# bjack205/altro

Measured on AMD Instinct MI355X. Metric: iLQR backward+forward sweeps/sec (N knotpoints x batch), higher is better.
Workload: dtype f64

## Files before the change

### altro_amd/__init__.py

```python
import ctypes as C
import os

import numpy as np

_HERE = os.path.dirname(os.path.abspath(__file__))
LIB_PATH = os.path.join(_HERE, "lib", "libaltro_hip.so")

F64, F32 = 0, 1
PLAN_AUTO, PLAN_GENERIC, PLAN_MFMA16, PLAN_LANE, PLAN_MFMA32 = 0, 1, 2, 3, 4
STORE_QBLOCKS = 0x1
LANE_FUSED = 0x4
F32_PURE = 0x2
TILE_USER_BLOCKS = 0x2
GENERIC_MATRIX_CORES = 0x8
TVLQR_SUCCESS = -1

C_ABI_SYMBOLS = [
    "altro_hip_version", "altro_hip_last_error", "altro_hip_device_count", "altro_hip_device_info", "altro_hip_device_pci_bus_id",
    "altro_hip_batch_create", "altro_hip_batch_create_dims", "altro_hip_batch_destroy", "altro_hip_batch_plan",
    "altro_hip_batch_device_bytes", "altro_hip_set_dynamics", "altro_hip_set_cost",
    "altro_hip_set_initial_state", "altro_hip_set_host_batch", "altro_hip_backward", "altro_hip_forward_ltv", "altro_hip_sweep",
    "altro_hip_synchronize", "altro_hip_get_K", "altro_hip_get_d", "altro_hip_get_P",
    "altro_hip_get_p", "altro_hip_get_x", "altro_hip_get_u", "altro_hip_get_y",
    "altro_hip_get_delta_V", "altro_hip_get_status", "altro_hip_get_qblocks",
    "altro_hip_stats_reduce", "altro_hip_comm_unique_id", "altro_hip_comm_create", "altro_hip_comm_create_all",
    "altro_hip_comm_destroy", "altro_hip_comm_rank", "altro_hip_comm_world", "altro_hip_comm_device", "altro_hip_stats_allreduce", "altro_hip_stats_allreduce_multi",
    "altro_hip_profile_enable", "altro_hip_profile_reset",
    "altro_hip_profile_get", "altro_hip_profile_get_range", "altro_hip_profile_dropped", "altro_hip_algorithmic_bytes",
    "altro_hip_set_model", "altro_hip_set_model_source", "altro_hip_model_row_layout", "altro_hip_set_tracking_cost", "altro_hip_set_quadratic_cost",
    "altro_hip_set_input_guess", "altro_hip_set_state_guess",
    "altro_hip_open_loop_rollout", "altro_hip_accept", "altro_hip_expand", "altro_hip_merit",
    "altro_hip_stationarity", "altro_hip_get_nominal", "altro_hip_get_expansion",
    "altro_hip_default_solve_options", "altro_hip_set_forms", "altro_hip_get_forms", "altro_hip_ilqr_solve", "altro_hip_last_solve_counts",
    "altro_hip_ilqr_solve_async", "altro_hip_ilqr_poll", "altro_hip_ilqr_wait",
    "altro_hip_linesearch_host",
    "altro_hip_add_linear_constraint", "altro_hip_add_user_constraint", "altro_hip_clear_constraints", "altro_hip_reset_duals",
    "altro_hip_get_duals", "altro_hip_feasibility",
    "altro_hip_shift_trajectory", "altro_hip_update_linear_costs", "altro_hip_get_knot",
    "altro_hip_set_pointer_mode",
]
CONE_EQUALITY, CONE_IDENTITY, CONE_INEQUALITY, CONE_SOC = 0, 1, 2, 3

FORM_NO_SPECULATION, FORM_NO_RUNAHEAD, FORM_NO_MERIT2, FORM_MERIT_LDS, FORM_MERIT_DPP_ALWAYS = 0x1, 0x2, 0x4, 0x8, 0x10
FORM_EXPAND_LDS, FORM_ALROWS_LDS, FORM_ROLLOUT_ROUNDS, FORM_SEQUENCED, FORM_MERIT_ONE_LAUNCH = 0x20, 0x40, 0x80, 0x100, 0x200
FORM_LANE_QUAD_OFF, FORM_LANE_QUAD_ON, FORM_GENERIC_LATE_Q_OFF, FORM_GENERIC_LATE_Q_ON, FORM_FUSED_CLOCK = 0x400, 0x800, 0x1000, 0x2000, 0x4000
FORM_AFFINE_EXACT = 0x8000
FORM_NO_COMPACTION = 0x10000
FORM_GENERIC_MERIT_LDS = 0x20000


def forms_from_env():
    e = os.environ
    off = lambda name: e.get(name) is not None and e[name].strip() not in ("",) and _atoi(e[name]) == 0
    f = 0
    if "ALTRO_HIP_NO_SPECULATION" in e: f |= FORM_NO_SPECULATION
    if "ALTRO_HIP_NO_RUNAHEAD" in e and not off("ALTRO_HIP_NO_RUNAHEAD"): f |= FORM_NO_RUNAHEAD
    if off("ALTRO_HIP_MERIT2"): f |= FORM_NO_MERIT2
    if off("ALTRO_HIP_MERIT_DPP"): f |= FORM_MERIT_LDS
    elif e.get("ALTRO_HIP_MERIT_DPP") is not None and _atoi(e["ALTRO_HIP_MERIT_DPP"]) == 2: f |= FORM_MERIT_DPP_ALWAYS
    if off("ALTRO_HIP_EXPAND_DPP"): f |= FORM_EXPAND_LDS
    if off("ALTRO_HIP_ALROWS_DPP"): f |= FORM_ALROWS_LDS
    if off("ALTRO_HIP_AFFINE"): f |= FORM_ROLLOUT_ROUNDS
    if off("ALTRO_HIP_FUSED") or "ALTRO_HIP_NO_FUSED" in e: f |= FORM_SEQUENCED
    if off("ALTRO_HIP_MERIT_SPLIT"): f |= FORM_MERIT_ONE_LAUNCH
    if "ALTRO_HIP_LANE_QUAD" in e: f |= FORM_LANE_QUAD_OFF if _atoi(e["ALTRO_HIP_LANE_QUAD"]) == 0 else FORM_LANE_QUAD_ON
    if "ALTRO_HIP_GENERIC_LATE_Q" in e: f |= FORM_GENERIC_LATE_Q_OFF if _atoi(e["ALTRO_HIP_GENERIC_LATE_Q"]) == 0 else FORM_GENERIC_LATE_Q_ON
    if "ALTRO_HIP_FUSED_CLOCK" in e: f |= FORM_FUSED_CLOCK
    if "ALTRO_HIP_AFFINE_EXACT" in e: f |= FORM_AFFINE_EXACT
    if "ALTRO_HIP_NO_COMPACTION" in e: f |= FORM_NO_COMPACTION
    return f


def _atoi(text):
    try:
        return int(text.strip() or 0)
    except ValueError:
        return 0

MODEL_LINEAR, MODEL_DOUBLE_INTEGRATOR, MODEL_PENDULUM, MODEL_BICYCLE, MODEL_USER, MODEL_QUADROTOR, MODEL_QUADROTOR13 = 0, 1, 2, 3, 4, 5, 6
MERIT_FN = C.CFUNCTYPE(None, C.c_double, C.POINTER(C.c_double), C.POINTER(C.c_double), C.c_void_p)


class SolveOptions(C.Structure):
    _fields_ = [("iterations_max", C.c_int), ("tol_stationarity", C.c_double),
                ("tol_primal_feasibility", C.c_double), ("tol_meritfun_gradient", C.c_double),
                ("use_backtracking_linesearch", C.c_int), ("penalty_initial", C.c_double),
                ("penalty_scaling", C.c_double), ("penalty_max", C.c_double), ("reg_initial", C.c_double),
                ("reg_retry_max", C.c_int), ("reg_scale", C.c_double), ("reg_min", C.c_double),
                ("reg_max", C.c_double), ("stop_when_running_at_most", C.c_int),
                ("forms", C.c_uint), ("fused_sweeps", C.c_int), ("decision_margin", C.c_double)]


class SolveResult(C.Structure):
    _fields_ = [("status", C.c_int), ("iterations", C.c_int), ("stationarity", C.c_double),
                ("final_alpha", C.c_double), ("final_phi", C.c_double), ("primal_feasibility", C.c_double),
                ("penalty", C.c_double), ("dual_updates", C.c_int), ("reg_retries", C.c_int)]


class PollRecord(C.Structure):
    _fields_ = [("result", SolveResult), ("u0", C.c_double * 4), ("done", C.c_int), ("reserved", C.c_int)]

# ... 62 lines not shown
        L.altro_hip_set_initial_state.argtypes = [vp, vp, i]
        L.altro_hip_set_host_batch.argtypes = [vp, i]
        L.altro_hip_backward.argtypes = [vp, d]
        L.altro_hip_forward_ltv.argtypes = [vp]
        L.altro_hip_sweep.argtypes = [vp, d]
        L.altro_hip_synchronize.argtypes = [vp]
        for g in ("K", "d", "P", "p", "x", "u", "y", "delta_V", "status", "qblocks"):
            getattr(L, "altro_hip_get_" + g).argtypes = [vp, vp]
        L.altro_hip_stats_reduce.argtypes = [vp, C.POINTER(Stats)]
        L.altro_hip_comm_unique_id.argtypes = [vp]
        L.altro_hip_comm_create.argtypes = [C.POINTER(vp), i, i, i, vp]
        L.altro_hip_comm_create_all.argtypes = [C.POINTER(vp), i, C.POINTER(i)]
        L.altro_hip_comm_destroy.argtypes = [vp]
        L.altro_hip_comm_destroy.restype = None
        for fn in ("rank", "world", "device"):
            getattr(L, "altro_hip_comm_" + fn).argtypes = [vp]
        L.altro_hip_stats_allreduce.argtypes = [vp, vp, C.POINTER(Stats)]
        L.altro_hip_stats_allreduce_multi.argtypes = [C.POINTER(vp), C.POINTER(vp), i, C.POINTER(Stats)]
        L.altro_hip_profile_enable.argtypes = [vp, i]
        L.altro_hip_profile_reset.argtypes = [vp]
        L.altro_hip_profile_get.argtypes = [vp, i, C.POINTER(i), C.POINTER(d), C.POINTER(C.c_char_p)]
        L.altro_hip_profile_get_range.argtypes = [vp, i, C.POINTER(d), C.POINTER(d)]
        L.altro_hip_profile_dropped.argtypes = [vp, i]
        L.altro_hip_algorithmic_bytes.argtypes = [vp, i]
        L.altro_hip_algorithmic_bytes.restype = d
        L.altro_hip_set_model.argtypes = [vp, i, C.c_float, i, d, d]
        L.altro_hip_set_model_source.argtypes = [vp, C.c_char_p, C.c_float]
        L.altro_hip_model_row_layout.argtypes = [vp]
        L.altro_hip_set_tracking_cost.argtypes = [vp, vp, vp, vp, vp, i, i]
        L.altro_hip_set_quadratic_cost.argtypes = [vp, vp, vp, vp, vp, vp, vp, i, i]
        L.altro_hip_set_input_guess.argtypes = [vp, vp, i, i]
        L.altro_hip_set_state_guess.argtypes = [vp, vp, i, i]
        for fn in ("open_loop_rollout", "accept", "expand"):
            getattr(L, "altro_hip_" + fn).argtypes = [vp]
        L.altro_hip_merit.argtypes = [vp, vp, i, i, vp, vp]
        L.altro_hip_stationarity.argtypes = [vp, vp]
        L.altro_hip_get_nominal.argtypes = [vp, vp, vp]
        L.altro_hip_get_expansion.argtypes = [vp, vp, vp, vp, vp]
        L.altro_hip_add_linear_constraint.argtypes = [vp, i, i, i, i, vp, vp, i]
        L.altro_hip_add_user_constraint.argtypes = [vp, i, i, i, i, i]
        L.altro_hip_clear_constraints.argtypes = [vp]
        L.altro_hip_reset_duals.argtypes = [vp, d]
        L.altro_hip_get_duals.argtypes = [vp, i, i, vp]
        L.altro_hip_feasibility.argtypes = [vp, vp]
        L.altro_hip_set_pointer_mode.argtypes = [vp, i]
        L.altro_hip_shift_trajectory.argtypes = [vp]
        L.altro_hip_update_linear_costs.argtypes = [vp, vp, vp, vp, i, i, i, i]
        L.altro_hip_get_knot.argtypes = [vp, i, vp, vp]
        L.altro_hip_default_solve_options.argtypes = [C.POINTER(SolveOptions)]
        L.altro_hip_default_solve_options.restype = None
        L.altro_hip_set_forms.argtypes = [vp, C.c_uint]
        L.altro_hip_get_forms.argtypes = [vp]
        L.altro_hip_get_forms.restype = C.c_uint
        L.altro_hip_ilqr_solve.argtypes = [vp, C.POINTER(SolveOptions), vp]
        L.altro_hip_last_solve_counts.argtypes = [vp, C.POINTER(i), C.POINTER(i)]
        L.altro_hip_ilqr_solve_async.argtypes = [vp, C.POINTER(SolveOptions)]
        L.altro_hip_ilqr_poll.argtypes = [vp, C.POINTER(i), C.POINTER(C.POINTER(PollRecord))]
        L.altro_hip_ilqr_wait.argtypes = [vp, vp]
        L.altro_hip_linesearch_host.argtypes = [MERIT_FN, vp, d, d, d, i, i, d, d, C.POINTER(i), C.POINTER(i),
                                                C.POINTER(d), C.POINTER(d)]
        L.altro_hip_linesearch_host.restype = d
        L.altro_hip_selftest_mfma_f64.argtypes = [i]
        L.altro_hip_selftest_mfma_f64.restype = d
        L.altro_hip_selftest_mfma_f32_4b.argtypes = [i]
        L.altro_hip_selftest_mfma_f32_4b.restype = d
        L.altro_hip_selftest_sincos.argtypes = [i, vp, i, vp, vp]
        L.altro_hip_selftest_sincos.restype = i
        _lib = L
    return _lib


def _check(rc):
    if rc != 0:
        raise AltroHipError("altro_hip error %d: %s" % (rc, lib().altro_hip_last_error().decode()))


def device_info(device=0):
    L = lib()
    name, pci = C.create_string_buffer(256), C.create_string_buffer(64)
    cus, ws = C.c_int(), C.c_int()
    _check(L.altro_hip_device_info(int(device), name, 256, C.byref(cus), C.byref(ws)))
    _check(L.altro_hip_device_pci_bus_id(int(device), pci, 64))
    return name.value.decode(), cus.value, pci.value.decode()


def _in(a):
    if a is None:
        return None, None
    a = np.ascontiguousarray(a, dtype=np.float64)
    return a, a.ctypes.data_as(C.c_void_p)


class Batch:

    def __init__(self, N, n, m, batch, dtype=F64, plan=PLAN_AUTO, flags=0, device=0, stream=None):
        self.L = lib()
        self.N, self.n, self.m, self.batch = N, n, m, batch
        self.h = C.c_void_p()
        _check(self.L.altro_hip_batch_create(C.byref(self.h), N, n, m, batch, dtype, plan, flags,
                                             device, stream))

    @property
    def plan(self):
        return self.L.altro_hip_batch_plan(self.h)

    @classmethod
# ... 202 lines not shown
        if rc < 0:
            _check(rc)
        return rc

    def add_user_constraint(self, k_first, k_last, cone, p, cid):
        rc = self.L.altro_hip_add_user_constraint(self.h, int(k_first), int(k_last), int(cone), int(p), int(cid))
        if rc < 0:
            _check(rc)
        return rc

    def clear_constraints(self):
        _check(self.L.altro_hip_clear_constraints(self.h))

    def reset_duals(self, penalty=1.0):
        _check(self.L.altro_hip_reset_duals(self.h, float(penalty)))

    def get_duals(self, k, slot, p):
        out = np.zeros((self.batch, p))
        _check(self.L.altro_hip_get_duals(self.h, int(k), int(slot), out.ctypes.data_as(C.c_void_p)))
        return out

    def feasibility(self):
        self._sync_forms()
        out = np.zeros(self.batch)
        _check(self.L.altro_hip_feasibility(self.h, out.ctypes.data_as(C.c_void_p)))
        return out

    def _solve_options(self, iterations_max=200, tol_stationarity=1e-4, tol_meritfun_gradient=1e-8,
                       use_backtracking=False, tol_primal_feasibility=1e-4, penalty_initial=1.0, penalty_scaling=10.0,
                       penalty_max=1e8, reg_initial=0.0, reg_retry_max=0, reg_scale=10.0, reg_min=1e-6, reg_max=1e8,
                       stop_when_running_at_most=0, forms=0, fused_sweeps=None, decision_margin=None):
        self._sync_forms()
        o = SolveOptions()
        self.L.altro_hip_default_solve_options(C.byref(o))
        o.forms = int(forms)
        if fused_sweeps is None and "ALTRO_HIP_FUSED_SWEEPS" in os.environ:
            fused_sweeps = _atoi(os.environ["ALTRO_HIP_FUSED_SWEEPS"]) or 1
        o.fused_sweeps = int(fused_sweeps or 0)
        if decision_margin is not None:
            o.decision_margin = float(decision_margin)
        o.tol_primal_feasibility = tol_primal_feasibility
        o.penalty_initial, o.penalty_scaling, o.penalty_max = penalty_initial, penalty_scaling, penalty_max
        o.reg_initial, o.reg_retry_max, o.reg_scale = reg_initial, reg_retry_max, reg_scale
        o.reg_min, o.reg_max = reg_min, reg_max
        o.stop_when_running_at_most = int(stop_when_running_at_most)
        o.iterations_max, o.tol_stationarity = iterations_max, tol_stationarity
        o.tol_meritfun_gradient, o.use_backtracking_linesearch = tol_meritfun_gradient, int(use_backtracking)
        return o

    def set_forms(self, forms):
        self._forms_user = int(forms)
        self._sync_forms()

    def _sync_forms(self):
        want = getattr(self, "_forms_user", 0) | forms_from_env()
        if want != getattr(self, "_forms_set", 0):
            _check(self.L.altro_hip_set_forms(self.h, want))
            self._forms_set = want

    @staticmethod
    def _results(rec, sweeps, merit_launches):
        return dict(status=rec["status"].copy(), iterations=rec["iterations"].copy(),
                    stationarity=rec["stationarity"].copy(), alpha=rec["final_alpha"].copy(), phi=rec["final_phi"].copy(),
                    feasibility=rec["primal_feasibility"].copy(), penalty=rec["penalty"].copy(),
                    dual_updates=rec["dual_updates"].copy(), reg_retries=rec["reg_retries"].copy(),
                    sweeps=sweeps, merit_launches=merit_launches)

    def ilqr_solve(self, **options):
        o = self._solve_options(**options)
        res = (SolveResult * self.batch)()
        _check(self.L.altro_hip_ilqr_solve(self.h, C.byref(o), res))
        sw, ml = C.c_int(), C.c_int()
        self.L.altro_hip_last_solve_counts(self.h, C.byref(sw), C.byref(ml))
        rec = np.frombuffer(res, dtype=np.dtype(SolveResult))
        return self._results(rec, sw.value, ml.value)

    def ilqr_solve_async(self, **options):
        o = self._solve_options(**options)
        _check(self.L.altro_hip_ilqr_solve_async(self.h, C.byref(o)))

    def poll(self):
        n, recs = C.c_int(), C.POINTER(PollRecord)()
        _check(self.L.altro_hip_ilqr_poll(self.h, C.byref(n), C.byref(recs)))
        buf = (PollRecord * self.batch).from_address(C.addressof(recs.contents))
        return n.value, np.frombuffer(buf, dtype=np.dtype(PollRecord))

    def wait(self):
        res = (SolveResult * self.batch)()
        _check(self.L.altro_hip_ilqr_wait(self.h, res))
        sw, ml = C.c_int(), C.c_int()
        self.L.altro_hip_last_solve_counts(self.h, C.byref(sw), C.byref(ml))
        return self._results(np.frombuffer(res, dtype=np.dtype(SolveResult)), sw.value, ml.value)


class Comm:

    @staticmethod
    def unique_id():
        buf = (C.c_char * COMM_ID_BYTES)()
        _check(lib().altro_hip_comm_unique_id(C.cast(buf, C.c_void_p)))
        return bytes(buf)

    def __init__(self, device, rank, world, uid):
        self.L = lib()
        self.c = C.c_void_p()
        assert len(uid) == COMM_ID_BYTES
# ... 36 lines not shown
```

### altro_amd/csrc/capi_core.hip

```cpp
#include "capi_internal.h"

namespace altro_hip {
namespace capi {

thread_local std::string g_last_error;

int fail(int code, const char* fmt, ...) {
  char buf[512];
  va_list ap;
  va_start(ap, fmt);
  vsnprintf(buf, sizeof(buf), fmt, ap);
  va_end(ap);
  g_last_error = buf;
  return code;
}

}
}

using namespace altro_hip;
using namespace altro_hip::capi;

namespace {

// ... 166 lines not shown
    }
    ALLOC(h->g_off, off.size() * sizeof(int64_t));
    ALLOC(h->g_nx, (size_t)(N + 1) * sizeof(int));
    ALLOC(h->g_nu, (size_t)(N + 1) * sizeof(int));
    if (!rc) {
      if (hipMemcpy(h->g_off, off.data(), off.size() * sizeof(int64_t), hipMemcpyHostToDevice) != hipSuccess ||
          hipMemcpy(h->g_nx, nx.data(), nx.size() * sizeof(int), hipMemcpyHostToDevice) != hipSuccess ||
          hipMemcpy(h->g_nu, nu.data(), nu.size() * sizeof(int), hipMemcpyHostToDevice) != hipSuccess)
        rc = fail(ALTRO_HIP_ERR_HIP, "table upload failed");
    }
  }
  {
    if (!rc) h->al_knots.assign((size_t)N + 1, AlKnotBig{});
    ALLOC(h->i_prob, B * sizeof(IlqrProb));
    ALLOC(h->i_alpha, B * 8);
    ALLOC(h->i_phi, B * 8 * ILQR_SPEC_TRIALS);
    ALLOC(h->i_spec_sel, B * sizeof(int));
    ALLOC(h->i_spec_refresh, B * sizeof(int));
    ALLOC(h->i_guard, B * sizeof(int));
    ALLOC(h->i_active_exact, B * sizeof(int));
    if (!rc && (hipMemsetAsync(h->i_guard, 0, B * sizeof(int), h->stream) != hipSuccess || hipMemsetAsync(h->i_active_exact, 0, B * sizeof(int), h->stream) != hipSuccess)) rc = fail(ALTRO_HIP_ERR_HIP, "memset failed");
    ALLOC(h->i_stat_done, B * sizeof(int));
    ALLOC(h->i_dphi, B * 8 * 2);
    ALLOC(h->i_active, B * sizeof(int));
    ALLOC(h->i_counters, (size_t)kCounterSlots * 8 * sizeof(int));
    if (!rc && hipMemsetAsync(h->i_counters, 0, (size_t)kCounterSlots * 8 * sizeof(int), h->stream) != hipSuccess) rc = fail(ALTRO_HIP_ERR_HIP, "memset failed");
    ALLOC(h->i_reg, B * 8);
    if (!rc) {
      std::vector<IlqrProb> pr((size_t)B);
      std::memset(pr.data(), 0, pr.size() * sizeof(IlqrProb));
      for (auto& q : pr) { q.rho = 1.0; q.rho_est = 1.0; q.status = 1; }
      if (hipMemcpy(h->i_prob, pr.data(), pr.size() * sizeof(IlqrProb), hipMemcpyHostToDevice) != hipSuccess)
        rc = fail(ALTRO_HIP_ERR_HIP, "control block upload failed");
    }
  }
#undef ALLOC
  if (!rc && (hipEventCreate(&h->ev0) != hipSuccess || hipEventCreate(&h->ev1) != hipSuccess))
    rc = fail(ALTRO_HIP_ERR_HIP, "hipEventCreate failed");
  if (rc) {
    altro_hip_batch_destroy(h);
    return rc;
  }
  *out = h;
  return 0;
}

int altro_hip_batch_create(altro_hip_batch** out, int N, int n, int m, int batch, int dtype, int plan,
                           unsigned flags, int device, void* stream) {
  return batch_create_impl(out, N, n, m, batch, dtype, plan, flags, device, stream, nullptr, nullptr);
}

extern "C++" {
namespace altro_hip { namespace capi {
int replan_empty_handle(altro_hip_batch* h, int plan) {
  if (!h->auto_plan || h->dyn_set || h->cost_set || h->model_set || h->lqr_cost_set || h->guess_set || !h->al_defs.empty() ||
      (h->x0_set && h->x0_host.empty()))
    return fail(ALTRO_HIP_ERR_UNSUPPORTED, "this handle runs plan %d; create it with plan %d (or call altro_hip_set_model before the dynamics, the cost, "
                                           "a guess or a constraint block reach a handle created with ALTRO_HIP_PLAN_AUTO)", h->plan, plan);
  altro_hip_batch* fresh = nullptr;
  int rc = batch_create_impl(&fresh, h->N, h->n, h->m, h->batch, h->dtype, plan, h->flags, h->device, h->user_stream ? (void*)h->stream : nullptr,
                             nullptr, nullptr);
  if (rc) return rc;
  fresh->dev_ptrs = h->dev_ptrs; fresh->host_batch = h->host_batch; fresh->forms = h->forms;
  const int prof = h->prof;
  std::vector<double> x0 = std::move(h->x0_host);
  const int x0_bz = h->x0_host_bz;
  std::swap(*h, *fresh);
  h->auto_plan = false;
  altro_hip_batch_destroy(fresh);
  if (prof && (rc = altro_hip_profile_enable(h, prof))) return rc;
  if (!x0.empty()) {
    const bool dp = h->dev_ptrs;
    h->dev_ptrs = false;
    rc = altro_hip_set_initial_state(h, x0.data(), x0_bz);
    h->dev_ptrs = dp;
  }
  return rc;
}
} }
}

int altro_hip_batch_create_dims(altro_hip_batch** out, int N, const int* nx, const int* nu, int batch, int dtype,
                                unsigned flags, int device, void* stream) {
  if (!out) return fail(ALTRO_HIP_ERR_BAD_ARGUMENT, "out == NULL");
  *out = nullptr;
  if (N <= 0 || !nx || !nu) return fail(ALTRO_HIP_ERR_BAD_ARGUMENT, "N must be positive, nx and nu non-null");
  int nmax = 0, mmax = 0;
  for (int k = 0; k <= N; ++k) {
    if (nx[k] <= 0 || nx[k] > kGenericMaxDim) return fail(ALTRO_HIP_ERR_UNSUPPORTED, "nx[%d] = %d outside [1, %d]", k, nx[k], kGenericMaxDim);
    nmax = std::max(nmax, nx[k]);
    if (k < N) {
      if (nu[k] <= 0 || nu[k] > kGenericMaxDim) return fail(ALTRO_HIP_ERR_UNSUPPORTED, "nu[%d] = %d outside [1, %d]", k, nu[k], kGenericMaxDim);
      mmax = std::max(mmax, nu[k]);
    }
  }
  return batch_create_impl(out, N, nmax, mmax, batch, dtype, ALTRO_HIP_PLAN_GENERIC, flags, device, stream, nx, nu);
}

void altro_hip_batch_destroy(altro_hip_batch* h) {
  if (!h) return;
  (void)hipSetDevice(h->device);
  if (h->stream) (void)hipStreamSynchronize(h->stream);
  void* ptrs[] = {h->x0, h->delta_V, h->status, h->m_in, h->m_cin, h->m_term, h->m_out, h->m_outn, h->m_xuy,
                  h->m_qblk, h->m_trash, h->g_off, h->g_nx, h->g_nu, h->stage,
                  h->l_in, h->l_term, h->l_out, h->l_outn, h->l_xuy, h->l_x0,
                  h->l_nom, h->l_cost, h->g_ws, h->i_prob, h->i_alpha, h->i_phi, h->i_dphi, h->i_active, h->i_counters,
                  h->al_d_knots, h->al_d_big, h->al_d_gsel, h->al_d_guser, h->g_stat_part, h->al_d_G, h->al_d_Gpad, h->al_d_g, h->al_d_z, h->i_reg, h->m_nom, h->m_costp,
                  h->i_cand_spec, h->i_spec_sel, h->i_spec_refresh, h->i_fused_list, h->i_guard, h->i_active_exact, h->i_stat_done, h->st_partial, h->st_red, h->i_merit_jk, h->i_spec_jac, h->i_results,
                  h->m_costd, h->m_costd_term, h->l_costq, h->i_sens, h->i_sens_alpha, h->i_aff_part, h->i_aff_on, h->g_xn, h->g_un, h->g_cQ, h->g_cR, h->g_cH, h->g_cq, h->g_cr, h->g_cc};
  for (void* p : ptrs) if (p) (void)hipFree(p);
  if (h->i_results_host) (void)hipHostFree(h->i_results_host);
  if (h->poll_host) (void)hipHostFree(h->poll_host);
  if (h->poll_count_host) (void)hipHostFree(h->poll_count_host);
  if (h->cnt_host) (void)hipHostFree(h->cnt_host);
  for (hipEvent_t e : h->cnt_ev) if (e) (void)hipEventDestroy(e);
  for (int a = 0; a < G_NUM; ++a) if (h->g_arr[a]) (void)hipFree(h->g_arr[a]);
  if (h->ev0) (void)hipEventDestroy(h->ev0);
  if (h->ev1) (void)hipEventDestroy(h->ev1);
  for (hipEvent_t e : h->prof_ev) if (e) (void)hipEventDestroy(e);
  if (h->own_stream && h->stream) (void)hipStreamDestroy(h->stream);
  delete h;
}

int altro_hip_batch_plan(const altro_hip_batch* h) { return h ? (h->g_tile ? (int)ALTRO_HIP_PLAN_MFMA32 : h->plan) : ALTRO_HIP_ERR_BAD_ARGUMENT; }
size_t altro_hip_batch_device_bytes(const altro_hip_batch* h) { return h ? h->device_bytes : 0; }

int altro_hip_set_dynamics(altro_hip_batch* h, const double* A, const double* B, const double* f,
                           int kz, int bz) {
  int rc = check(h);
  if (rc) return rc;
  h->expansion_current = false;
  if (!A || !B) return fail(ALTRO_HIP_ERR_BAD_ARGUMENT, "A and B are required");
  const int n = h->n, m = h->m, N = h->N;
  h->has_f = f ? 1 : 0;
  if (h->plan == ALTRO_HIP_PLAN_MFMA16) {
    DevSrc dA, dB, df;
    const int nkh = kz ? 1 : N;
    rc = put_src(h, A, n * n, nkh, kz, bz, &dA);
    if (!rc) rc = put_src(h, B, n * m, nkh, kz, bz, &dB);
    if (!rc) rc = put_src(h, f, n, nkh, kz, bz, &df);
    if (!rc) rc = mfma16_pack_launch(h, MSEG_Z, dA.s, dB.s);
    if (!rc) rc = mfma16_pack_launch(h, MSEG_F, df.s, SrcArr{nullptr, 0, 0, 0});
    if (!rc) HIP_TRY(hipStreamSynchronize(h->stream));
  } else if (h->plan == ALTRO_HIP_PLAN_LANE) {
    const LaneSizes z = lane_sizes(n, m);
    const int nkh = kz ? 1 : N;
    auto pk = [&](const double* src, int len, int off) -> int { return lane_pack(h, h->l_in, 0, z.e_in, src, len, off, 0, N, 0, nkh, kz, bz); };
    rc = pk(A, n * n, 0);
    if (!rc) rc = pk(B, n * m, n * n);
    if (!rc) rc = pk(f, n, n * n + n * m);
  } else {
    if (h->ragged && kz) return fail(ALTRO_HIP_ERR_BAD_ARGUMENT, "k_stride_zero needs uniform dimensions");
    auto set = [&](int arr, const double* src, int blk) -> int {
      return h->ragged ? generic_set(h, arr, src, (int)h->g_bstride[arr], 1, 0, bz) : generic_set(h, arr, src, blk, N, kz, bz);
    };
    rc = set(G_A, A, n * n);
    if (!rc) rc = set(G_B, B, n * m);
    if (!rc) {
      if (f) rc = set(G_f, f, n);
      else HIP_TRY(hipMemsetAsync(h->g_arr[G_f], 0, (size_t)h->batch * h->g_bstride[G_f] * h->esz, h->stream));
    }
  }
  if (!rc) { HIP_TRY(hipStreamSynchronize(h->stream)); h->dyn_set = true; }
  return rc;
}

int altro_hip_set_cost(altro_hip_batch* h, const double* Q, const double* R, const double* H,
                       const double* q, const double* r, int is_diag, int kz, int bz) {
  int rc = check(h);
  if (rc) return rc;
  h->expansion_current = false;
  if (!Q || !R || !q || !r) return fail(ALTRO_HIP_ERR_BAD_ARGUMENT, "Q, R, q, r are required");
  if (!is_diag && !H) return fail(ALTRO_HIP_ERR_BAD_ARGUMENT, "H is required for a dense cost");
  h->ilqr_linear = false;
  const int n = h->n, m = h->m, N = h->N;
  Dims d{n, m};
  h->is_diag = is_diag ? 1 : 0;
  const int nkQ = kz ? 2 : N + 1;
  const int nkR = kz ? 1 : N;
  if (h->plan == ALTRO_HIP_PLAN_MFMA16) {
    DevSrc dQ, dR, dH, dq, dr;
    rc = put_src(h, Q, d.Q(is_diag), nkQ, kz, bz, &dQ);
    if (!rc) rc = put_src(h, R, d.R(is_diag), nkR, kz, bz, &dR);
    if (!rc && !is_diag) rc = put_src(h, H, d.H(), nkR, kz, bz, &dH);
    if (!rc) rc = put_src(h, q, n, nkQ, kz, bz, &dq);
    if (!rc) rc = put_src(h, r, m, nkR, kz, bz, &dr);
    SrcArr none{nullptr, 0, 0, 0};
    SrcArr tQ = dQ.s, tq = dq.s;
    if (kz) { tQ.p += d.Q(is_diag); tq.p += n; }
    if (!rc) rc = mfma16_pack_launch(h, MSEG_Q, dQ.s, none);
    if (!rc) rc = mfma16_pack_launch(h, MSEG_TERM_Q, tQ, none);
    if (!rc) rc = mfma16_pack_launch(h, MSEG_HR, dH.s, dR.s);
    if (!rc) rc = mfma16_pack_launch(h, MSEG_QR, dq.s, dr.s);
    if (!rc) rc = mfma16_pack_launch(h, MSEG_TERM_q, tq, none);
    if (!rc) HIP_TRY(hipStreamSynchronize(h->stream));
  } else if (h->plan == ALTRO_HIP_PLAN_LANE) {
    const LaneSizes z = lane_sizes(n, m);
    const int oQ = n * n + n * m + n, oR = oQ + n * n, oH = oR + m * m, oq = oH + m * n, or_ = oq + n;
    auto pk = [&](void* dst, int E, const double* src, int len, int off, int diag, int nk, int k_src0,
                  int nk_host, int src_off = 0) -> int {
      return lane_pack(h, dst, 0, E, src, len, off, diag, nk, k_src0, nk_host, kz, bz, src_off);
    };
    const int kt = kz ? 0 : N;
    rc = pk(h->l_in, z.e_in, Q, d.Q(is_diag), oQ, is_diag ? n : 0, N, 0, nkQ);
    if (!rc) rc = pk(h->l_in, z.e_in, R, d.R(is_diag), oR, is_diag ? m : 0, N, 0, nkR);
    if (!rc) rc = pk(h->l_in, z.e_in, is_diag ? nullptr : H, d.H(), oH, 0, N, 0, nkR);
    if (!rc) rc = pk(h->l_in, z.e_in, q, n, oq, 0, N, 0, nkQ);
    if (!rc) rc = pk(h->l_in, z.e_in, r, m, or_, 0, N, 0, nkR);
    if (!rc) rc = pk(h->l_term, z.e_term, Q, d.Q(is_diag), 0, is_diag ? n : 0, 1, kt, nkQ, kz ? d.Q(is_diag) : 0);
    if (!rc) rc = pk(h->l_term, z.e_term, q, n, n * n, 0, 1, kt, nkQ, kz ? n : 0);
  } else if (h->ragged) {
    if (kz) return fail(ALTRO_HIP_ERR_BAD_ARGUMENT, "k_stride_zero needs uniform dimensions");
    {
      std::vector<int64_t> off((size_t)(N + 1) * G_NUM);
      HIP_TRY(hipStreamSynchronize(h->stream));
      HIP_TRY(hipMemcpy(off.data(), h->g_off, off.size() * sizeof(int64_t), hipMemcpyDeviceToHost));
      int64_t aq = 0, ar = 0;
      for (int k = 0; k <= N; ++k) {
        off[(size_t)k * G_NUM + G_Q] = aq; off[(size_t)k * G_NUM + G_R] = ar;
        aq += is_diag ? h->nxv[k] : h->nxv[k] * h->nxv[k];
        if (k < N) ar += is_diag ? h->nuv[k] : h->nuv[k] * h->nuv[k];
      }
      h->g_bstride[G_Q] = aq; h->g_bstride[G_R] = ar;
      HIP_TRY(hipMemcpy(h->g_off, off.data(), off.size() * sizeof(int64_t), hipMemcpyHostToDevice));
    }
    auto whole = [&](int arr, const double* src) -> int {
      if (!src) { HIP_TRY(hipMemsetAsync(h->g_arr[arr], 0, (size_t)h->batch * h->g_bstride[arr] * h->esz, h->stream)); return 0; }
      return generic_set(h, arr, src, (int)h->g_bstride[arr], 1, 0, bz);
    };
    rc = whole(G_Q, Q);
// ... 248 lines not shown
```

### altro_amd/csrc/capi_ilqr.hip

```cpp
#include "capi_internal.h"

#include <cstring>

using namespace altro_hip;
using namespace altro_hip::capi;

namespace altro_hip {
namespace capi {

static AlInput al_input(const altro_hip_batch* h) {
  return AlInput{h->plan, h->n, h->m, h->N, h->batch, h->dtype == ALTRO_HIP_F64 ? sizeof(double) : sizeof(float), h->ragged, h->nxv, h->nuv,
                 h->al_defs, h->al_knots, h->al_G, h->al_g};
}
static int al_copy(altro_hip_batch* h, void** dst, const void* src, size_t bytes) {
  if (const int rc = dmalloc(h, dst, bytes)) return rc;
  HIP_TRY(hipMemcpy(*dst, src, bytes, hipMemcpyHostToDevice));
  return 0;
}
static int al_copy_pool(altro_hip_batch* h, void** dst, const std::vector<double>& pool) {
  if (h->dtype == ALTRO_HIP_F64) return al_copy(h, dst, pool.data(), pool.size() * sizeof(double));
  const std::vector<float> f = al_pool_as<float>(pool);
  return al_copy(h, dst, f.data(), f.size() * sizeof(float));
}
static int al_upload_tables(altro_hip_batch* h) {
// ... 69 lines not shown
bool ensure_spares(altro_hip_batch* h, int count, size_t bytes_each) {
  if (h->spare_count >= count) return true;
  if (h->spare_failed > 0 && count >= h->spare_failed) return false;
  void* fresh = nullptr;
  if (hipMalloc(&fresh, (size_t)count * bytes_each) != hipSuccess) { (void)hipGetLastError(); h->spare_failed = count; return false; }
  if (h->i_cand_spec) { (void)hipStreamSynchronize(h->stream); (void)hipFree(h->i_cand_spec); h->device_bytes -= (size_t)h->spare_count * bytes_each; }
  h->i_cand_spec = fresh;
  h->spare_count = count;
  h->device_bytes += (size_t)count * bytes_each;
  return true;
}
void merit_split_prepare(altro_hip_batch* h) {
  if (h->merit_split >= 0) return;
  h->merit_split = form(h, ALTRO_HIP_FORM_MERIT_ONE_LAUNCH) ? 0 : 1;
  if (!h->merit_split) return;
  const size_t jk = (size_t)spec_trials_cap(h) * (h->N + 1) * h->batch * h->esz;
  const size_t jac = ((size_t)h->N * (h->n * h->n + h->n * h->m + h->n + h->m) + h->n) * h->batch * h->esz;
  if (dmalloc(h, &h->i_merit_jk, jk) || dmalloc(h, &h->i_spec_jac, jac)) {
    (void)hipGetLastError();
    if (h->i_merit_jk) { (void)hipFree(h->i_merit_jk); h->i_merit_jk = nullptr; }
    h->merit_split = 0;
  }
}

template <typename T>
int ilqr_launch(altro_hip_batch* h, int which, IlqrArgs<T> a) {
  if (h->model.kind == MODEL_USER) return rtc_launch<T>(h, which, a);
  const int rc = ilqr_launch_kernel<T>(h->stream, which, h->model.kind, h->n, h->m, a);
  if (rc == 1) return fail(ALTRO_HIP_ERR_UNSUPPORTED, "no device model for (kind, n, m) = (%d, %d, %d)", h->model.kind, h->n, h->m);
  if (rc) return fail(ALTRO_HIP_ERR_HIP, "iLQR kernel launch failed");
  return 0;
}
template <typename S>
int wave_run(altro_hip_batch* h, int which, bool use_alpha, bool use_active, int want_deriv, double alpha_const, int mode) {
  IlqrWaveArgs<S> a;
  a.al = al_table<S>(h);
  a.mode = mode;
  const bool user_al = a.al.enabled && h->al_sum.has_user;
  if (user_al && (h->forms & (ALTRO_HIP_FORM_MERIT_LDS | ALTRO_HIP_FORM_ALROWS_LDS | ALTRO_HIP_FORM_EXPAND_LDS)))
    return fail(ALTRO_HIP_ERR_UNSUPPORTED, "constraint blocks from source on plan MFMA16 run in the row-layout kernels only: the LDS comparison forms "
                                           "(ALTRO_HIP_FORM_MERIT_LDS, _ALROWS_LDS, _EXPAND_LDS) do not evaluate them");
  a.penalty_scaling = h->expand_penalty_scaling; a.penalty_max = h->expand_penalty_max;
  if (which == IK_STATIONARITY || which == IK_DUAL)
    a.mode = form(h, ALTRO_HIP_FORM_ALROWS_LDS) ? 0 : STAT_NO_FEAS;
  if (which == IK_EXPAND && form(h, ALTRO_HIP_FORM_EXPAND_LDS) && !h->cost_dense) a.mode |= EXPAND_LDS;
  a.costd = (const S*)h->m_costd; a.costd_term = (const S*)h->m_costd_term; a.cost_dense = h->cost_dense ? 1 : 0;
  if (h->model_set) {
    a.mp = h->model;
    if (which == IK_EXPAND && (a.mode & EXPAND_GRADIENT) && !(a.mode & EXPAND_NEXT)) a.mode |= EXPAND_DYN;
  }
  if (which == IK_MERIT)
    a.mode = form(h, ALTRO_HIP_FORM_MERIT_LDS) ? 0 : form(h, ALTRO_HIP_FORM_MERIT_DPP_ALWAYS) ? 3 : 2;
  a.dyn = (const S*)h->m_in; a.dyn_bs = h->m_st.in_bs; a.dyn_ks = h->m_st.in_ks;
  a.cin = (S*)h->m_cin; a.cin_bs = h->m_st.cin_bs; a.cin_ks = h->m_st.cin_ks;
  a.term = (S*)h->m_term; a.out = (const S*)h->m_out; a.out_bs = h->m_st.out_bs; a.out_ks = h->m_st.out_ks;
  a.outn = (const S*)h->m_outn; a.nom = (S*)h->m_nom; a.cand = (S*)h->m_xuy; a.xuy_bs = h->m_st.xuy_bs;
  a.xuy_ks = h->m_st.xuy_ks; a.costp = (const S*)h->m_costp; a.x0 = (const S*)h->x0;
  a.alpha = use_alpha ? h->i_alpha : nullptr; a.active = use_active ? h->i_active : nullptr;
  a.phi = h->i_phi; a.dphi = h->i_dphi; a.prob = h->i_prob; a.N = h->N; a.batch = h->batch;
  a.want_derivative = want_deriv; a.alpha_const = alpha_const;
  a.cand_spec = (S*)h->i_cand_spec; a.spec_trials = h->i_cand_spec ? h->spec_trials : 1; a.spec_sel = h->i_spec_sel;
  a.spec_pre = h->i_cand_spec ? h->spec_pre : 0;
  a.spec_stride = (int64_t)h->batch * (h->N + 1) * MF_XUY;
  a.ls_beta = h->spec_beta; a.ls_max_iters = h->spec_max_iters;
  a.skip = which == IK_STATIONARITY ? h->stat_skip : nullptr;
  if constexpr (sizeof(S) == 8) {
    if (h->aff_enabled && !h->model_set) {
      if (h->aff_store && (which == IK_MERIT2 || which == IK_MERIT)) {
        a.sens = (double*)h->i_sens; a.sens_alpha = (double*)h->i_sens_alpha;
      } else if (which == IK_MERIT && h->aff_round && a.mode >= 2 && !a.spec_pre) {
        a.sens = (double*)h->i_sens; a.sens_alpha = (double*)h->i_sens_alpha;
        a.aff = 1; a.aff_part = (double*)h->i_aff_part; a.aff_on = (int*)h->i_aff_on;
      }
    }
  }
  if (h->model_set && h->model.kind == MODEL_USER) {
    if constexpr (sizeof(S) == 8) {
      if (which == IK_ROLLOUT || which == IK_MERIT || which == IK_MERIT2) return rtc_tile_launch(h, which, a);
      if (which == IK_EXPAND && (a.mode & EXPAND_DYN)) {
        const int rcm = rtc_tile_launch(h, IK_EXPAND, a);
        if (rcm) return rcm;
      }
      if (user_al && (which == IK_EXPAND || which == IK_DUAL)) return rtc_tile_al_launch(h, which, a);
      if (user_al && which == IK_STATIONARITY) {
        a.mp.kind = MODEL_LINEAR;
        a.mode |= STAT_FEAS_USER;
        const int rcs = ilqr_wave_launch_kernel<S>(h->stream, which, a);
        if (rcs) return fail(ALTRO_HIP_ERR_HIP, "iLQR kernel launch failed");
        return rtc_tile_al_launch(h, which, a);
      }
    }
    a.mp.kind = MODEL_LINEAR;
  }
  const int rc = ilqr_wave_launch_kernel<S>(h->stream, which, a);
  if (rc == 1) return fail(ALTRO_HIP_ERR_UNSUPPORTED, "operation %d is not available on plan MFMA16", which);
  if (rc) return fail(ALTRO_HIP_ERR_HIP, "iLQR kernel launch failed");
  return 0;
}
struct GenSizes { int64_t sx, su, sQ, sR, sH; };
GenSizes gen_sizes(const altro_hip_batch* h) {
  GenSizes z{0, 0, 0, 0, 0};
  for (int k = 0; k <= h->N; ++k) {
    const int64_t nk = h->ragged ? h->nxv[k] : h->n, mk = k < h->N ? (h->ragged ? h->nuv[k] : h->m) : 0;
    z.sx += nk; z.su += mk; z.sQ += nk * nk; z.sR += mk * mk; z.sH += mk * nk;
  }
  return z;
}
// ... 27 lines not shown
  a.alpha = use_alpha ? h->i_alpha : nullptr; a.active = use_active ? h->i_active : nullptr; a.alpha_const = alpha_const;
  a.phi = h->i_phi; a.dphi = h->i_dphi; a.prob = h->i_prob;
  a.N = N; a.n = n; a.m = m; a.batch = h->batch; a.want_derivative = want_deriv; a.mode = mode;
  a.off = h->g_off; a.nx = h->g_nx; a.nu = h->g_nu;
  const GenSizes gs = gen_sizes(h);
  a.sx = gs.sx; a.su = gs.su; a.sQ = gs.sQ; a.sR = gs.sR; a.sH = gs.sH;
  a.al = al_table<T>(h);
  a.row32 = (sizeof(T) == 8 && row32_eligible(h)) ? 1 : 0;
  a.row32m = (sizeof(T) == 8 && row32_model_eligible(h)) ? 1 : 0;
  if ((a.row32 || a.row32m) && which == IK_STATIONARITY && N > 32) {
    const size_t need = (size_t)((N + 31) / 32) * h->batch * 2 * sizeof(double);
    if (h->g_stat_part_bytes < need) {
      if (h->g_stat_part) { (void)hipFree(h->g_stat_part); h->g_stat_part = nullptr; h->g_stat_part_bytes = 0; }
      if (hipMalloc((void**)&h->g_stat_part, need) == hipSuccess) h->g_stat_part_bytes = need;
      else { (void)hipGetLastError(); h->g_stat_part = nullptr; }
    }
    a.stat_part = h->g_stat_part;
  }
  if (h->model_set) {
    a.mp = h->model;
    if (which == IK_EXPAND && (a.mode & EXPAND_GRADIENT)) a.mode |= EXPAND_DYN;
  }
  if constexpr (sizeof(T) == 8) {
    if (h->model_set && h->model.kind == MODEL_USER) {
      const bool user_al = a.al.enabled && a.al.guser;
      if (which == IK_ROLLOUT || which == IK_MERIT || (which == IK_MERIT2 && a.row32m)) return rtc_gen_launch(h, which, a);
      if (user_al && (which == IK_STATIONARITY || which == IK_DUAL)) return rtc_gen_al_launch(h, which, a);
      if (which == IK_EXPAND) {
        IlqrGenArgs<T> ac = a;
        ac.mp.kind = MODEL_LINEAR;
        if (user_al) {
          const int rc0 = rtc_gen_al_launch(h, which, ac);
          if (rc0) return rc0;
        } else {
          const int rc0 = ilqr_generic_launch<T>(h->stream, which, ac);
          if (rc0) return fail(ALTRO_HIP_ERR_HIP, "iLQR kernel launch failed");
        }
        return (a.mode & EXPAND_DYN) ? rtc_gen_launch(h, which, a) : 0;
      }
    }
  }
  const int rc = ilqr_generic_launch<T>(h->stream, which, a);
  if (rc == 1) return fail(ALTRO_HIP_ERR_UNSUPPORTED, "operation %d is not available on plan GENERIC", which);
  if (rc) return fail(ALTRO_HIP_ERR_HIP, "iLQR kernel launch failed");
  return 0;
}
int ilqr_run(altro_hip_batch* h, int which, bool use_alpha, bool use_active, int want_deriv, double alpha_const, int mode) {
  int rc = al_upload(h);
  if (rc) return rc;
  if (h->plan == ALTRO_HIP_PLAN_GENERIC)
    return h->dtype == ALTRO_HIP_F64 ? gen_run<double>(h, which, use_alpha, use_active, want_deriv, alpha_const, mode)
                                     : gen_run<float>(h, which, use_alpha, use_active, want_deriv, alpha_const, mode);
  if (h->plan == ALTRO_HIP_PLAN_MFMA16) {
    rc = h->dtype == ALTRO_HIP_F64 ? wave_run<double>(h, which, use_alpha, use_active, want_deriv, alpha_const, mode)
                                   : wave_run<float>(h, which, use_alpha, use_active, want_deriv, alpha_const, mode);
    if (which == IK_MERIT) h->expansion_current = !rc && want_deriv && !use_active && h->spec_trials == 1 && !h->spec_pre && h->al_defs.empty();
    else if (which == IK_ROLLOUT || which == IK_SHIFT || which == IK_SPEC_SELECT || which == IK_MERIT2 || which == IK_DUAL) h->expansion_current = false;
    return rc;
  }
  if (which == IK_MERIT) merit_split_prepare(h);
  if (h->dtype == ALTRO_HIP_F64) {
    auto a = ilqr_args<double>(h, use_alpha, use_active, want_deriv, alpha_const);
    a.mode = mode;
    return ilqr_launch<double>(h, which, a);
  }
  auto a = ilqr_args<float>(h, use_alpha, use_active, want_deriv, alpha_const);
  a.mode = mode;
  return ilqr_launch<float>(h, which, a);
}

struct CostUpload { int field; const double* src; int nk_host; };
int cost_fields_set(altro_hip_batch* h, bool dense, const CostUpload* up, int count, int kz, int bz) {
  LoopShape s = loop_shape(h);
  s.cost_dense = dense;
  const int N = h->N;
  int rc = 0;
  for (int pass = 0; pass < 2; ++pass)
    for (int i = 0; i < count && !rc; ++i) {
      const FieldRef r0 = loop_field(s, up[i].field, 0), rN = loop_field(s, up[i].field, N);
      const bool zero_array = !up[i].src && r0.kind == LK_AOS;
      if (pass == 0 && zero_array) HIP_TRY(hipMemsetAsync(loop_buffer(h, r0.buf), 0, (size_t)h->batch * r0.bs * h->esz, h->stream));
      else if (pass == 0) rc = field_set(h, s, up[i].field, 0, s.ragged && rN.buf != LB_NONE ? N + 1 : N, up[i].src, kz, bz, up[i].nk_host);
      else if (!zero_array && !s.ragged && rN.buf != LB_NONE) rc = field_set(h, s, up[i].field, N, 1, up[i].src, 1, bz, up[i].nk_host, (kz ? 1 : N) * rN.len);
    }
  return rc;
}
int generic_cost_def(altro_hip_batch* h, const double* Q, const double* R, const double* H, const double* q, const double* r,
                     const double* c, int kz, int bz) {
  const int N = h->N;
  const int nkx = kz ? 2 : N + 1, nku = kz ? 1 : N;
  const size_t B = h->batch, E = h->esz;
  const GenSizes gs = gen_sizes(h);
  int rc = 0;
  {
    struct { void** p; size_t bytes; bool zero; } want[] = {
        {&h->g_cQ, B * gs.sQ * E, false}, {&h->g_cR, B * gs.sR * E, false}, {&h->g_cH, B * gs.sH * E, false},
        {&h->g_cq, B * gs.sx * E, false}, {&h->g_cr, B * gs.su * E, false}, {&h->g_cc, B * (N + 1) * E, false},
        {&h->g_xn, B * gs.sx * E, true},  {&h->g_un, B * gs.su * E, true}};
    for (auto& w : want) {
      if (*w.p) continue;
      if ((rc = dmalloc(h, w.p, w.bytes))) return rc;
      if (w.zero) HIP_TRY(hipMemsetAsync(*w.p, 0, w.bytes, h->stream));
    }
  }
  if (h->ragged && kz) return fail(ALTRO_HIP_ERR_BAD_ARGUMENT, "k_stride_zero needs uniform dimensions");
  const CostUpload up[] = {{LF_COST_Q, Q, nkx}, {LF_COST_R, R, nku}, {LF_COST_H, H, nku}, {LF_COST_q, q, nkx}, {LF_COST_r, r, nku}, {LF_COST_c, c, nkx}};
// ... 408 lines not shown
      return fail(ALTRO_HIP_ERR_BAD_ARGUMENT, "knot points %d and %d differ in dimension: one constraint block takes one [x; u] size "
                                              "(register it per range, like ALTROSolver::SetConstraint per index)", k_first, ad.k);
    default: break;
  }
  const int w = ad.w;
  AlDef d{cone, p, g_per_problem ? 1 : 0, (int)h->al_G.size(), 0, user, w};
  h->al_G.insert(h->al_G.end(), G, G + (size_t)p * w);
  h->al_g.emplace_back(g, g + (size_t)p * (g_per_problem ? h->batch : 1));
  const int id = (int)h->al_defs.size();
  h->al_defs.push_back(d);
  for (int k = k_first; k <= k_last; ++k) {
    AlKnotBig& kn = h->al_knots[k];
    kn.def[kn.ncon++] = id;
  }
  h->al_dirty = true;
  return id;
}
int altro_hip_add_linear_constraint(altro_hip_batch* h, int k_first, int k_last, int cone, int p, const double* G,
                                    const double* g, int g_per_problem) {
  return add_block(h, k_first, k_last, cone, p, G, g, g_per_problem, 0);
}
int altro_hip_add_user_constraint(altro_hip_batch* h, int k_first, int k_last, int cone, int p, int id) {
  int rc = loop_entry(h);
  if (rc) return rc;
  const bool gen = h->plan == ALTRO_HIP_PLAN_GENERIC;
  const bool tile = h->plan == ALTRO_HIP_PLAN_MFMA16;
  if ((h->plan != ALTRO_HIP_PLAN_LANE && !gen && !tile) || h->model.kind != MODEL_USER || !h->rtc_has_constraints)
    return fail(ALTRO_HIP_ERR_NOT_SET, "altro_hip_set_model_source must come first, with a source that defines "
                                       "altro_user_constraint and altro_user_constraint_jacobian (plans LANE and GENERIC / MFMA32)");
  if (id < 0) return fail(ALTRO_HIP_ERR_BAD_ARGUMENT, "constraint id %d", id);
  const AlAdmit ad = al_admit(al_input(h), k_first, k_last, cone, p, id + 1);
  if (ad.limit == AL_LIMIT_USER_CONE) return fail(ALTRO_HIP_ERR_BAD_ARGUMENT, "unknown cone %d", cone);
  if (ad.limit == AL_LIMIT_USER_ROWS && tile)
    return fail(ALTRO_HIP_ERR_UNSUPPORTED, "a constraint block from source has 1 .. %d rows on plan MFMA16 (%s: one slot; got %d): "
                                           "ALTRO_HIP_PLAN_GENERIC takes 32", ad.pmax, cone == CONE_SOC ? "AL_MAXSOC" : "AL_MAXP", p);
  if (ad.limit == AL_LIMIT_USER_ROWS)
    return fail(ALTRO_HIP_ERR_UNSUPPORTED, "a constraint block from source has 1 .. %d rows on plan GENERIC (GEN_USER_MAXROWS; got %d)", ad.pmax, p);
  if (ad.limit == AL_LIMIT_USER_KNOT && tile)
    return fail(ALTRO_HIP_ERR_UNSUPPORTED, "at most %d constraint blocks from source per knot point on plan MFMA16 (AL_TILE_USER_MAXC; k = %d "
                                           "would have %d): ALTRO_HIP_PLAN_GENERIC takes 32 rows of them", ad.cmax, ad.k, ad.count);
  if (ad.limit == AL_LIMIT_USER_KNOT)
    return fail(ALTRO_HIP_ERR_UNSUPPORTED, "at most %d rows of constraint blocks from source per knot point on plan GENERIC "
                                           "(GEN_USER_MAXROWS; k = %d would have %d)", ad.cmax, ad.k, ad.count);
  std::vector<double> G((size_t)std::max(p, 0) * (h->n + h->m), 0.0), g((size_t)std::max(p, 0), 0.0);
  return add_block(h, k_first, k_last, cone, p, G.data(), g.data(), 0, id + 1);
}
int altro_hip_clear_constraints(altro_hip_batch* h) {
  int rc = loop_entry(h, true);
  if (rc) return rc;
  h->expansion_current = false;
  h->al_defs.clear(); h->al_G.clear(); h->al_g.clear();
  h->al_knots.assign((size_t)h->N + 1, AlKnotBig{});
  h->al_dirty = true;
  return al_upload(h);
}
int altro_hip_reset_duals(altro_hip_batch* h, double penalty) {
  int rc = loop_entry(h, true);
  if (rc) return rc;
  h->expansion_current = false;
  if (!(penalty > 0.0)) return fail(ALTRO_HIP_ERR_BAD_ARGUMENT, "penalty must be positive");
  if ((rc = al_upload(h))) return rc;
  const size_t E = h->dtype == ALTRO_HIP_F64 ? 8 : 4;
  if (h->al_d_z) HIP_TRY(hipMemsetAsync(h->al_d_z, 0, (size_t)h->al_rows * h->batch * E, h->stream));
  std::vector<IlqrProb> pr(h->batch);
  HIP_TRY(hipStreamSynchronize(h->stream));
  HIP_TRY(hipMemcpy(pr.data(), h->i_prob, pr.size() * sizeof(IlqrProb), hipMemcpyDeviceToHost));
  for (auto& q : pr) { q.rho = penalty; q.rho_est = penalty; }
  HIP_TRY(hipMemcpy(h->i_prob, pr.data(), pr.size() * sizeof(IlqrProb), hipMemcpyHostToDevice));
  return 0;
}
int altro_hip_get_duals(altro_hip_batch* h, int k, int slot, double* z) {
  int rc = loop_entry(h, true);
  if (rc) return rc;
  if ((rc = al_upload(h))) return rc;
  if (k < 0 || k > h->N || slot < 0 || slot >= h->al_knots[k].ncon || !z)
    return fail(ALTRO_HIP_ERR_BAD_ARGUMENT, "no constraint block %d at knot point %d", slot, k);
  const AlKnotBig& kn = h->al_knots[k];
  const int p = h->al_defs[kn.def[slot]].p;
  const int64_t B = h->batch;
  HIP_TRY(hipStreamSynchronize(h->stream));
  auto fetch = [&](auto t) -> int {
    std::vector<decltype(t)> v((size_t)p * B);
    HIP_TRY(hipMemcpy(v.data(), (const decltype(t)*)h->al_d_z + (size_t)kn.z_off[slot] * B, v.size() * sizeof(t), hipMemcpyDeviceToHost));
    for (int64_t b = 0; b < B; ++b)
      for (int r = 0; r < p; ++r) z[(size_t)b * p + r] = v[(size_t)r * B + b];
    return 0;
  };
  return h->dtype == ALTRO_HIP_F64 ? fetch(double{}) : fetch(float{});
}

}
int altro_hip::capi::ilqr_gather_results(altro_hip_batch* h, altro_hip_solve_result* results) {
  static_assert(sizeof(IlqrResult) == sizeof(altro_hip_solve_result), "IlqrResult mirrors altro_hip_solve_result");
  static_assert(sizeof(IlqrPollRec) == sizeof(altro_hip_poll_record), "IlqrPollRec mirrors altro_hip_poll_record");
  int rc;
  const size_t bytes = (size_t)h->batch * sizeof(IlqrResult);
  if (!h->i_results) {
    if ((rc = dmalloc(h, &h->i_results, bytes))) return rc;
    if (hipHostMalloc(&h->i_results_host, bytes, hipHostMallocDefault) != hipSuccess) { (void)hipGetLastError(); h->i_results_host = nullptr; }
  }
  if (ilqr_launch_results(h->stream, h->i_prob, (IlqrResult*)h->i_results, h->batch)) return fail(ALTRO_HIP_ERR_HIP, "results kernel launch failed");
  void* stage = h->i_results_host ? h->i_results_host : (void*)results;
  HIP_TRY(hipMemcpyAsync(stage, h->i_results, bytes, hipMemcpyDeviceToHost, h->stream));
  HIP_TRY(hipStreamSynchronize(h->stream));
  if (stage != (void*)results) std::memcpy(results, stage, bytes);
  return 0;
}
// ... 14 lines not shown
  return 0;
}
int altro_hip_ilqr_wait(altro_hip_batch* h, altro_hip_solve_result* results) {
  int rc = loop_entry(h, true);
  if (rc) return rc;
  if (!h->poll_host) return fail(ALTRO_HIP_ERR_NOT_SET, "altro_hip_ilqr_solve_async has not been called");
  HIP_TRY(hipStreamSynchronize(h->stream));
  if (h->async_pending) {
    h->async_pending = false;
    int c4[4];
    HIP_TRY(hipMemcpy(c4, h->i_counters, sizeof(c4), hipMemcpyDeviceToHost));
    h->last_sweeps = c4[3];
    h->last_merit_launches = 0;
  }
  if (results) return ilqr_gather_results(h, results);
  return 0;
}


void altro_hip_default_solve_options(altro_hip_solve_options* o) {
  if (!o) return;
  o->iterations_max = 200;
  o->tol_stationarity = 1e-4;
  o->tol_primal_feasibility = 1e-4;
  o->tol_meritfun_gradient = 1e-8;
  o->use_backtracking_linesearch = 0;
  o->penalty_initial = 1.0;
  o->penalty_scaling = 10.0;
  o->penalty_max = 1e8;
  o->reg_initial = 0.0;
  o->reg_retry_max = 0;
  o->reg_scale = 10.0;
  o->reg_min = 1e-6;
  o->reg_max = 1e8;
  o->stop_when_running_at_most = 0;
  o->forms = 0;
  o->fused_sweeps = 0;
  o->decision_margin = 0.0;
}
int altro_hip_set_forms(altro_hip_batch* h, unsigned forms) {
  int rc = check(h);
  if (rc) return rc;
  if ((forms & ALTRO_HIP_FORM_LANE_QUAD_OFF) && (forms & ALTRO_HIP_FORM_LANE_QUAD_ON))
    return fail(ALTRO_HIP_ERR_BAD_ARGUMENT, "ALTRO_HIP_FORM_LANE_QUAD_OFF and _ON exclude each other");
  if ((forms & ALTRO_HIP_FORM_GENERIC_LATE_Q_OFF) && (forms & ALTRO_HIP_FORM_GENERIC_LATE_Q_ON))
    return fail(ALTRO_HIP_ERR_BAD_ARGUMENT, "ALTRO_HIP_FORM_GENERIC_LATE_Q_OFF and _ON exclude each other");
  if (((h->forms ^ forms) & ALTRO_HIP_FORM_MERIT_ONE_LAUNCH) && h->merit_split >= 0) {
    HIP_TRY(hipStreamSynchronize(h->stream));
    if (h->i_merit_jk) { (void)hipFree(h->i_merit_jk); h->i_merit_jk = nullptr; }
    if (h->i_spec_jac) { (void)hipFree(h->i_spec_jac); h->i_spec_jac = nullptr; }
    h->merit_split = -1;
  }
  h->forms = forms;
  return 0;
}
unsigned altro_hip_get_forms(const altro_hip_batch* h) { return h ? h->forms : 0u; }
int altro_hip_last_solve_counts(const altro_hip_batch* h, int* sweeps, int* merit_launches) {
  if (!h) return fail(ALTRO_HIP_ERR_BAD_ARGUMENT, "null handle");
  if (sweeps) *sweeps = h->last_sweeps;
  if (merit_launches) *merit_launches = h->last_merit_launches;
  return 0;
}
int altro_hip_get_nominal(altro_hip_batch* h, double* x, double* u) {
  int rc = loop_entry(h, true);
  if (rc) return rc;
  if (h->plan == ALTRO_HIP_PLAN_MFMA16 && !h->m_nom) return fail(ALTRO_HIP_ERR_NOT_SET, "altro_hip_set_tracking_cost has not been called");
  if (h->plan == ALTRO_HIP_PLAN_GENERIC && !h->g_xn) return fail(ALTRO_HIP_ERR_NOT_SET, "no cost has been set for the iLQR loop");
  const LoopShape s = loop_shape(h);
  if (x && (rc = field_get(h, s, LF_NOM_X, 0, h->N + 1, x))) return rc;
  if (u) rc = field_get(h, s, LF_NOM_U, 0, h->N, u);
  return rc;
}
int altro_hip_get_expansion(altro_hip_batch* h, double* A, double* B, double* lx, double* lu) {
  int rc = loop_entry(h);
  if (rc) return rc;
  const int n = h->n, m = h->m, N = h->N;
  if (h->plan == ALTRO_HIP_PLAN_MFMA16) {
    if (h->dev_ptrs) return fail(ALTRO_HIP_ERR_UNSUPPORTED, "altro_hip_get_expansion on plan MFMA16 writes host arrays");
    const int64_t B_ = h->batch;
    std::vector<double> raw;
    auto fetch = [&](const void* src, int64_t bs, int64_t ks, int off, int block, int nk) -> int {
      raw.assign((size_t)B_ * nk * block, 0.0);
      return aos_get(h, raw.data(), src, off, bs, ks, block, nk);
    };
    if (A || B) {
      if ((rc = fetch(h->m_in, h->m_st.in_bs, h->m_st.in_ks, MF_OFF_Z, 192, N))) return rc;
      for (int64_t b = 0; b < B_; ++b)
        for (int k = 0; k < N; ++k) {
          const double* zr = raw.data() + ((size_t)b * N + k) * 192;
          if (A) for (int j = 0; j < n; ++j) for (int i = 0; i < n; ++i) A[((size_t)b * N + k) * n * n + i + (size_t)n * j] = zr[i * 16 + j];
          if (B) for (int j = 0; j < m; ++j) for (int i = 0; i < n; ++i) B[((size_t)b * N + k) * n * m + i + (size_t)n * j] = zr[i * 16 + MF_N + j];
        }
    }
    if (lx || lu) {
      if ((rc = fetch(h->m_cin, h->m_st.cin_bs, h->m_st.cin_ks, MF_OFF_QR, 16, N))) return rc;
      for (int64_t b = 0; b < B_; ++b)
        for (int k = 0; k < N; ++k) {
          const double* qr = raw.data() + ((size_t)b * N + k) * 16;
          if (lx) for (int i = 0; i < n; ++i) lx[((size_t)b * (N + 1) + k) * n + i] = qr[i];
          if (lu) for (int i = 0; i < m; ++i) lu[((size_t)b * N + k) * m + i] = qr[MF_N + i];
        }
      if (lx) {
        if ((rc = fetch(h->m_term, MF_TERM, 0, MF_TERM_q, MF_N, 1))) return rc;
        for (int64_t b = 0; b < B_; ++b)
          for (int i = 0; i < n; ++i) lx[((size_t)b * (N + 1) + N) * n + i] = raw[(size_t)b * MF_N + i];
      }
    }
    return 0;
  }
  if (h->plan == ALTRO_HIP_PLAN_GENERIC) {
    auto get = [&](double* dst, int arr, int blk, int nk) -> int { return dst ? generic_get(h, arr, dst, blk, nk) : 0; };
    rc = get(A, G_A, n * n, N);
    if (!rc) rc = get(B, G_B, n * m, N);
    if (!rc) rc = get(lx, G_q, n, N + 1);
    if (!rc) rc = get(lu, G_r, m, N);
    return rc;
  }
  const LaneSizes z = lane_sizes(n, m);
  const int oq = 2 * n * n + 2 * n * m + m * m + n, orr = oq + n;
  auto get = [&](double* dst, int off, int len, int nk, bool with_term, int off_term) -> int {
    if (!dst) return 0;
    return lane_get(h, dst, h->l_in, 0, with_term ? h->l_term : nullptr, z.e_in, off, off_term, len, nk, N);
  };
  rc = get(A, 0, n * n, N, false, 0);
  if (!rc) rc = get(B, n * n, n * m, N, false, 0);
  if (!rc) rc = get(lx, oq, n, N + 1, true, n * n);
  if (!rc) rc = get(lu, orr, m, N, false, 0);
  return rc;
}

double altro_hip_linesearch_host(altro_hip_merit_fn f, void* ctx, double alpha0, double phi0, double dphi0,
                                 int try_cubic_first, int use_backtracking, double c1, double c2,
                                 int* status, int* iters, double* phi, double* dphi) {
  LsOptions o = ls_default_options();
  o.try_cubic_first = try_cubic_first; o.use_backtracking = use_backtracking; o.c1 = c1; o.c2 = c2;
  LsState s;
  bool need = ls_begin(s, o, alpha0, phi0, dphi0);
  while (need) {
    double p = 0.0, dp = 0.0;
    f(s.alpha, &p, s.want_derivative ? &dp : nullptr, ctx);
    need = ls_feed(s, o, p, dp);
  }
  if (status) *status = s.status;
  if (iters) *iters = s.n_iters;
  if (phi) *phi = s.phi;
  if (dphi) *dphi = s.dphi;
  return s.alpha;
}
// ... 3 lines not shown
```

### altro_amd/csrc/capi_internal.h

```cpp
#pragma once
#include "altro_hip/altro_hip.h"

#include <hip/hip_runtime.h>
#include <hip/hip_ext.h>

#include <algorithm>
#include <cstdarg>
#include <cstdio>
#include <cstdlib>
#include <cstring>
#include <string>
#include <vector>

#include "kernels/pack.hip"
#include "kernels/tvlqr_generic.hip"
#include "kernels/tvlqr_lane.hip"
#include "kernels/ilqr_types.h"
#include "kernels/ilqr_generic.hip"
#include "kernels/mfma16_layout.h"
#include "linesearch_sm.h"
#include "al_tables.h"
#include "loop_fields.h"
#include "rtc_unit.h"

namespace altro_hip {
namespace capi {

int fail(int code, const char* fmt, ...);

#define HIP_TRY(expr)                                                                         \
  do {                                                                                        \
    hipError_t e_ = (expr);                                                                   \
    if (e_ != hipSuccess)                                                                     \
      return ::altro_hip::capi::fail(ALTRO_HIP_ERR_HIP, "%s failed: %s (%s:%d)", #expr, hipGetErrorString(e_), \
                  __FILE__, __LINE__);                                                        \
  } while (0)

constexpr size_t kStageBytes = size_t(256) << 20;

}
}

using namespace altro_hip;

struct altro_hip_batch {
  int N = 0, n = 0, m = 0, batch = 0, dtype = 0, plan = 0, device = 0;
  unsigned flags = 0;
  unsigned forms = 0;
  hipStream_t stream = nullptr;
  bool own_stream = false;
  size_t esz = 8;
  void* x0 = nullptr;
  void* delta_V = nullptr;
  int* status = nullptr;
  bool dyn_set = false, cost_set = false, x0_set = false, backward_done = false, forward_done = false;
  int has_f = 0, is_diag = 0;
  int host_batch = 0;
  bool dev_ptrs = false;
  void* g_arr[G_NUM] = {};
  int64_t g_bstride[G_NUM] = {};
  void *i_sens = nullptr, *i_sens_alpha = nullptr, *i_aff_part = nullptr, *i_aff_on = nullptr;
  bool aff_failed = false;
  bool aff_enabled = false, aff_round = false, aff_store = false;
  bool g_tile = false;
  bool g_mfma = false;
  bool ragged = false;
  std::vector<int> nxv, nuv;
  int64_t* g_off = nullptr;
  int* g_nx = nullptr;
  int* g_nu = nullptr;
  void *m_in = nullptr, *m_cin = nullptr, *m_term = nullptr, *m_out = nullptr, *m_outn = nullptr, *m_xuy = nullptr,
       *m_qblk = nullptr, *m_trash = nullptr;
  Mfma16Strides m_st{};
  void *l_in = nullptr, *l_term = nullptr, *l_out = nullptr, *l_outn = nullptr, *l_xuy = nullptr,
       *l_x0 = nullptr;
  void *l_nom = nullptr, *l_cost = nullptr;
  IlqrProb* i_prob = nullptr;
  double *i_alpha = nullptr, *i_phi = nullptr, *i_dphi = nullptr;
  int *i_active = nullptr, *i_counters = nullptr;
  int* cnt_host = nullptr;
  int* cnt_host_dev = nullptr;
  hipEvent_t cnt_ev[16] = {};
  void* i_cand_spec = nullptr;
  void* poll_host = nullptr; int* poll_count_host = nullptr;
  bool async_request = false, async_pending = false;
  bool rtc_row32_ok = false;
  bool rtc_has_constraints = false;
  void* rtc = nullptr;
  std::string rtc_source;
  int rtc_ck = 0;
  int x0_stride = 0;
  int spare_count = 0;
  int spare_failed = 0;
  int *i_spec_sel = nullptr, *i_spec_refresh = nullptr;
  int* i_fused_list = nullptr;
  int fused_resident = 0;
  int *i_guard = nullptr, *i_active_exact = nullptr;
  int* i_stat_done = nullptr;
  const int* stat_skip = nullptr;
  void *i_merit_jk = nullptr, *i_spec_jac = nullptr;
  int merit_split = -1;
  void *i_results = nullptr, *i_results_host = nullptr;
  void* g_ws = nullptr;
  bool fwd_quad = false;
  bool bwd_quad = false;
  int spec_trials = 1;
  int spec_pre = 0;
  bool spec_no_memory = false;
  double spec_beta = 0.5;
  int spec_max_iters = 25;
  ModelParams model{MODEL_LINEAR, 0.0f, 0, 2.7, 1.5};
  bool model_set = false, lqr_cost_set = false, guess_set = false;
  std::vector<double> x0_host;
  int x0_host_bz = 0;
  bool auto_plan = false;
  bool user_stream = false;
  std::vector<AlDef> al_defs;
  std::vector<AlKnotBig> al_knots;
  std::vector<double> al_G;
  std::vector<std::vector<double>> al_g;
  int al_rows = 0;
  capi::AlSummary al_sum;
  bool al_dirty = false;
  AlKnot* al_d_knots = nullptr;
  AlKnotBig* al_d_big = nullptr;
  void *al_d_G = nullptr, *al_d_g = nullptr, *al_d_z = nullptr;
  void* al_d_Gpad = nullptr;
  double* g_stat_part = nullptr; size_t g_stat_part_bytes = 0;
  int* al_d_gsel = nullptr;
  int* al_d_guser = nullptr;
  double expand_penalty_scaling = 10.0, expand_penalty_max = 1e8;
  const int* bwd_active = nullptr;
  const double* bwd_reg = nullptr;
  void *m_nom = nullptr, *m_costp = nullptr;
  bool ilqr_linear = false;
  void *m_costd = nullptr, *m_costd_term = nullptr, *l_costq = nullptr;
  bool cost_dense = false;
  bool expansion_current = false;
  void *g_xn = nullptr, *g_un = nullptr, *g_cQ = nullptr, *g_cR = nullptr, *g_cH = nullptr, *g_cq = nullptr, *g_cr = nullptr, *g_cc = nullptr;
  double* i_reg = nullptr;
  void* stage = nullptr;
  size_t stage_bytes = 0;
  size_t device_bytes = 0;
  double *st_partial = nullptr, *st_red = nullptr;
  bool solve_done = false;
  int prof = 0;
  std::vector<hipEvent_t> prof_ev;
  std::vector<int> prof_slot;
  int prof_n = 0;
  double prof_min[2] = {0, 0}, prof_max[2] = {0, 0};
  hipEvent_t ev0 = nullptr, ev1 = nullptr;
  hipEvent_t launch_ev0 = nullptr, launch_ev1 = nullptr;
  int last_sweeps = 0, last_merit_launches = 0;
  int prof_launches[2] = {0, 0};
  int prof_dropped[2] = {0, 0};
  double prof_ms[2] = {0, 0};
};

namespace altro_hip {
namespace capi {

inline bool form(const altro_hip_batch* h, unsigned bit) { return (h->forms & bit) != 0; }

inline int dmalloc(altro_hip_batch* h, void** p, size_t bytes) {
  hipError_t e = hipMalloc(p, bytes ? bytes : 16);
  if (e != hipSuccess) {
    *p = nullptr;
    return fail(ALTRO_HIP_ERR_OUT_OF_MEMORY, "hipMalloc(%zu bytes) failed: %s", bytes,
                hipGetErrorString(e));
  }
  h->device_bytes += bytes;
  return 0;
}

inline int check(altro_hip_batch* h) {
  if (!h) return fail(ALTRO_HIP_ERR_BAD_ARGUMENT, "null handle");
  hipError_t e = hipSetDevice(h->device);
  if (e != hipSuccess) return fail(ALTRO_HIP_ERR_HIP, "hipSetDevice(%d): %s", h->device, hipGetErrorString(e));
  return 0;
}

inline int loop_entry(altro_hip_batch* h, bool takes_varying_dims = false) {
  int rc = check(h);
  if (rc) return rc;
  if (h->ragged && !takes_varying_dims)
    return fail(ALTRO_HIP_ERR_UNSUPPORTED, "this call needs uniform dimensions; a handle with per-knot-point dimensions (altro_hip_batch_create_dims) "
                                           "takes altro_hip_set_dynamics / _set_quadratic_cost / _set_tracking_cost / _update_linear_costs / _set_initial_state / "
                                           "_set_input_guess / _set_state_guess / _add_linear_constraint, the iLQR loop calls and their getters, all with packed "
                                           "[batch][k][block_k] arrays");
  return 0;
}

inline int ensure_stage(altro_hip_batch* h, size_t bytes) {
  if (h->stage_bytes >= bytes) return 0;
  if (h->stage) (void)hipFree(h->stage);
  h->stage = nullptr;
  h->stage_bytes = 0;
  hipError_t e = hipMalloc(&h->stage, bytes);
  if (e != hipSuccess)
    return fail(ALTRO_HIP_ERR_OUT_OF_MEMORY, "staging hipMalloc(%zu) failed: %s", bytes,
                hipGetErrorString(e));
  h->stage_bytes = bytes;
  return 0;
}

inline int grid_for(int64_t total, int block = 256) {
  int64_t g = (total + block - 1) / block;
  return (int)std::min<int64_t>(std::max<int64_t>(g, 1), 256 * 32);
}

struct Dims {
  int n, m;
  int A() const { return n * n; }
  int B() const { return n * m; }
  int Q(int diag) const { return diag ? n : n * n; }
  int R(int diag) const { return diag ? m : m * m; }
// ... 125 lines not shown
  });
}

inline int aos_get(altro_hip_batch* h, double* host, const void* base, int64_t off, int64_t src_bs, int64_t src_ks, int block, int nk) {
  return h->dtype == ALTRO_HIP_F64 ? aos_get<double>(h, host, (const double*)base + off, src_bs, src_ks, block, nk)
                                   : aos_get<float>(h, host, (const float*)base + off, src_bs, src_ks, block, nk);
}
inline int generic_get(altro_hip_batch* h, int arr, double* host, int block, int nk) {
  return h->dtype == ALTRO_HIP_F64 ? generic_get<double>(h, arr, host, block, nk) : generic_get<float>(h, arr, host, block, nk);
}

inline int mfma16_get(altro_hip_batch* h, int what, double* host, int block, int nk) {
  return download_chunks(h, host, block, nk, [&](double* dst, int b0, int nb) {
    const int64_t total = (int64_t)nb * nk * block;
    if (h->dtype == ALTRO_HIP_F64)
      hipLaunchKernelGGL(mfma16_unpack_kernel<double>, dim3(grid_for(total)), dim3(256), 0, h->stream, dst, what,
                         (const double*)h->m_out, (const double*)h->m_outn, (const double*)h->m_xuy,
                         (const double*)h->m_qblk, h->m_st, h->N, b0, nb, h->n, h->m);
    else
      hipLaunchKernelGGL(mfma16_unpack_kernel<float>, dim3(grid_for(total)), dim3(256), 0, h->stream, dst, what,
                         (const float*)h->m_out, (const float*)h->m_outn, (const float*)h->m_xuy,
                         (const float*)h->m_qblk, h->m_st, h->N, b0, nb, h->n, h->m);
    hipError_t e = hipGetLastError();
    if (e != hipSuccess) return fail(ALTRO_HIP_ERR_HIP, "mfma16_unpack launch: %s", hipGetErrorString(e));
    return 0;
  });
}

struct DevSrc {
  void* dev = nullptr;
  SrcArr s{nullptr, 0, 0, 0};
  ~DevSrc() { if (dev) (void)hipFree(dev); }
};
inline int put_src(altro_hip_batch* h, const double* src, int blk, int nk_host, int k_zero, int b_zero,
            DevSrc* out) {
  if (!src) return 0;
  const size_t per_b = (size_t)nk_host * blk;
  const int tiled = (!b_zero && h->host_batch > 0 && h->host_batch < h->batch) ? h->host_batch : 0;
  const size_t bytes = (size_t)(b_zero ? 1 : (tiled ? tiled : h->batch)) * per_b * sizeof(double);
  if (h->dev_ptrs) {
    out->s = SrcArr{src, b_zero ? 0 : (int64_t)per_b, k_zero ? 0 : (int64_t)blk, tiled};
    return 0;
  }
  if (hipMalloc(&out->dev, bytes) != hipSuccess)
    return fail(ALTRO_HIP_ERR_OUT_OF_MEMORY, "hipMalloc(%zu) failed", bytes);
  if (hipMemcpyAsync(out->dev, src, bytes, hipMemcpyHostToDevice, h->stream) != hipSuccess)
    return fail(ALTRO_HIP_ERR_HIP, "H2D copy failed");
  out->s = SrcArr{(const double*)out->dev, b_zero ? 0 : (int64_t)per_b, k_zero ? 0 : (int64_t)blk, tiled};
  return 0;
}
inline int mfma16_pack_launch(altro_hip_batch* h, int seg, SrcArr s0, SrcArr s1, void* cin = nullptr, void* term = nullptr,
                              int is_diag = -1) {
  const int64_t total = (int64_t)h->batch * h->N * 192;
  if (!cin) cin = h->m_cin;
  if (!term) term = h->m_term;
  if (is_diag < 0) is_diag = h->is_diag;
  if (h->dtype == ALTRO_HIP_F64)
    hipLaunchKernelGGL(mfma16_pack_kernel<double>, dim3(grid_for(total)), dim3(256), 0, h->stream, (double*)h->m_in,
                       (double*)cin, (double*)term, h->m_st, seg, s0, s1, is_diag, h->N, 0, h->batch, h->n, h->m);
  else
    hipLaunchKernelGGL(mfma16_pack_kernel<float>, dim3(grid_for(total)), dim3(256), 0, h->stream, (float*)h->m_in,
                       (float*)cin, (float*)term, h->m_st, seg, s0, s1, is_diag, h->N, 0, h->batch, h->n, h->m);
  hipError_t e = hipGetLastError();
  if (e != hipSuccess) return fail(ALTRO_HIP_ERR_HIP, "mfma16_pack launch: %s", hipGetErrorString(e));
  return 0;
}

#define LANE_SHAPES(X)                                                                                   \
  X(1, 1) X(2, 1) X(3, 1) X(4, 1) X(5, 1) X(6, 1) X(1, 2) X(2, 2) X(3, 2) X(4, 2) X(5, 2) X(6, 2) X(1, 3) \
  X(2, 3) X(3, 3) X(4, 3) X(5, 3) X(6, 3)
inline bool lane_supported(int n, int m) {
#define X(N_, M_) if (n == N_ && m == M_) return true;
  LANE_SHAPES(X)
#undef X
  return false;
}
struct LaneSizes { int e_in, e_term, e_out, e_xuy; };
inline LaneSizes lane_sizes(int n, int m) {
  return LaneSizes{2 * n * n + 2 * n * m + m * m + 2 * n + m, n * n + n, m * n + m + n * n + n, 2 * n + m};
}
template <typename T>
inline int lane_pack(altro_hip_batch* h, T* dst_base, int E, const double* host, int len, int dst_off,
              int diag_n, int nk, int k_src0, int nk_host, int kz, int bz, int src_off = 0) {
  DevSrc d;
  int rc = put_src(h, host, len, nk_host, kz, bz, &d);
  if (rc) return rc;
  LaneSeg s{d.s.p ? d.s.p + src_off : nullptr, d.s.bs, d.s.ks, len, dst_off, diag_n, d.s.bmod};
  const int dlen = diag_n > 0 ? diag_n * diag_n : len;
  const int64_t total = (int64_t)h->batch * nk * dlen;
  hipLaunchKernelGGL(lane_pack_kernel<T>, dim3(grid_for(total)), dim3(256), 0, h->stream, dst_base, E, s,
                     nk, k_src0, h->batch);
  if (hipGetLastError() != hipSuccess) return fail(ALTRO_HIP_ERR_HIP, "lane_pack launch failed");
  HIP_TRY(hipStreamSynchronize(h->stream));
  return 0;
}
template <typename T>
inline int lane_get(altro_hip_batch* h, double* host, const void* src, const void* src_term, int E, int off,
             int off_term, int len, int nk, int nk_main) {
  return download_chunks(h, host, len, nk, [&](double* dst, int b0, int nb) {
    const int64_t total = (int64_t)nb * nk * len;
    hipLaunchKernelGGL(lane_unpack_kernel<T>, dim3(grid_for(total)), dim3(256), 0, h->stream, dst,
                       (const T*)src, (const T*)src_term, E, off, 0, off_term, len, nk, nk_main, b0, nb,
                       h->batch);
    if (hipGetLastError() != hipSuccess) return fail(ALTRO_HIP_ERR_HIP, "lane_unpack launch failed");
    return 0;
  });
}

inline int lane_pack(altro_hip_batch* h, void* base, int64_t off, int E, const double* host, int len, int dst_off, int diag_n, int nk,
                     int k_src0, int nk_host, int kz, int bz, int src_off = 0) {
  return h->dtype == ALTRO_HIP_F64 ? lane_pack<double>(h, (double*)base + off, E, host, len, dst_off, diag_n, nk, k_src0, nk_host, kz, bz, src_off)
                                   : lane_pack<float>(h, (float*)base + off, E, host, len, dst_off, diag_n, nk, k_src0, nk_host, kz, bz, src_off);
}
inline int lane_get(altro_hip_batch* h, double* host, const void* base, int64_t off, const void* src_term, int E, int rec_off, int off_term,
                    int len, int nk, int nk_main) {
// ... 73 lines not shown
```

### altro_amd/csrc/capi_tvlqr.hip

```cpp
#include "capi_internal.h"
#include "models.h"

#include "kernels/tvlqr_mfma16.hip"
#include "kernels/tvlqr_mfma16_f32.hip"
#include "kernels/tvlqr_mfma16_f32x4.hip"
#include "kernels/tvlqr_mfma16_fwd_f32x4.hip"

using namespace altro_hip;
using namespace altro_hip::capi;

#define PROF_LAUNCH(kernel, grid, block, lds, stream, ...) \
  hipExtLaunchKernelGGL(kernel, grid, block, lds, stream, h->launch_ev0, h->launch_ev1, 0, __VA_ARGS__)

namespace {

template <typename T>
int lane_launch(altro_hip_batch* h, bool backward, double reg) {
  LaneArgs<T> a{(const T*)h->l_in, (const T*)h->l_term, (T*)h->l_out, (T*)h->l_outn, (const T*)h->l_x0,
                (T*)h->l_xuy, (T*)h->delta_V, h->status, h->N, h->batch, (T)reg, backward ? h->bwd_active : nullptr,
                backward ? h->bwd_reg : nullptr};
  const dim3 grid(8 * (((h->batch + 63) / 64 + 7) / 8)), block(64);
  const bool fused = (h->flags & ALTRO_HIP_LANE_FUSED) != 0;
  const bool quad_on = form(h, ALTRO_HIP_FORM_LANE_QUAD_ON) ? true : form(h, ALTRO_HIP_FORM_LANE_QUAD_OFF) ? false : h->batch <= 12288;
  const bool q42 = h->n == 4 && h->m == 2, q21 = h->n == 2 && h->m == 1;
// ... 45 lines not shown
  a.x0_stride = h->n;
  a.delta_V = (T*)h->delta_V;
  a.status = h->status;
  a.N = h->N;
  a.batch = h->batch;
  a.nmax = h->n;
  a.mmax = h->m;
  a.reg = (T)reg;
  a.is_diag = h->is_diag;
  a.store_q = (h->flags & ALTRO_HIP_STORE_QBLOCKS) ? 1 : 0;
  a.want_y = 1;
  a.no_f = h->ilqr_linear ? 1 : 0;
  if (h->bwd_reg) { a.active = h->bwd_active; a.reg_pp = h->bwd_reg; }
  return a;
}

struct ProfScope {
  altro_hip_batch* h;
  int slot, idx = -1;
  static void add(altro_hip_batch* h, int slot, float ms) {
    h->prof_min[slot] = h->prof_launches[slot] ? std::min(h->prof_min[slot], (double)ms) : (double)ms;
    h->prof_max[slot] = std::max(h->prof_max[slot], (double)ms);
    h->prof_ms[slot] += ms;
    h->prof_launches[slot] += 1;
  }
  ProfScope(altro_hip_batch* h_, int slot_) : h(h_), slot(slot_) {
    h->launch_ev0 = nullptr; h->launch_ev1 = nullptr;
    if (h->prof == 1) { h->launch_ev0 = h->ev0; h->launch_ev1 = h->ev1; }
    else if (h->prof == 2) {
      if (2 * (h->prof_n + 1) <= (int)h->prof_ev.size()) {
        idx = h->prof_n++;
        h->prof_slot[idx] = slot;
        h->launch_ev0 = h->prof_ev[2 * idx]; h->launch_ev1 = h->prof_ev[2 * idx + 1];
      } else {
        h->prof_dropped[slot] += 1;
      }
    }
  }
  ~ProfScope() {
    if (h->prof == 1 && h->launch_ev1) {
      (void)hipEventSynchronize(h->ev1);
      float ms = 0.f;
      if (hipEventElapsedTime(&ms, h->ev0, h->ev1) == hipSuccess) add(h, slot, ms);
    }
    h->launch_ev0 = nullptr; h->launch_ev1 = nullptr;
  }
};


template <typename S>
Mfma16Args<S> mfma16_args(altro_hip_batch* h, double reg) {
  Mfma16Args<S> a;
  a.in = (const S*)h->m_in;
  a.cin = (const S*)h->m_cin;
  a.cin_bs = h->m_st.cin_bs; a.cin_ks = h->m_st.cin_ks;
  a.in_bs = h->m_st.in_bs; a.in_ks = h->m_st.in_ks; a.out_bs = h->m_st.out_bs; a.out_ks = h->m_st.out_ks;
  a.xuy_bs = h->m_st.xuy_bs; a.xuy_ks = h->m_st.xuy_ks;
  a.term = (const S*)h->m_term; a.out = (S*)h->m_out; a.outn = (S*)h->m_outn; a.qblk = (S*)h->m_qblk;
  a.trash = (S*)h->m_trash; a.x0 = (const S*)h->x0; a.xuy = (S*)h->m_xuy; a.delta_V = (S*)h->delta_V;
  a.status = h->status; a.N = h->N; a.batch = h->batch; a.reg = reg; a.has_f = h->has_f && !h->ilqr_linear;
  a.active = h->bwd_active; a.reg_pp = h->bwd_reg;
  return a;
}
template <typename S>
void mfma16_launch_backward(altro_hip_batch* h, double reg, bool sq) {
  auto a = mfma16_args<S>(h, reg);
  const dim3 grid(mf_grid(h->batch)), block(64);
  if (sq && a.has_f) PROF_LAUNCH((mfma16_backward_kernel<true, true, S>), grid, block, 0, h->stream, a);
  else if (sq) PROF_LAUNCH((mfma16_backward_kernel<true, false, S>), grid, block, 0, h->stream, a);
  else if (a.has_f) PROF_LAUNCH((mfma16_backward_kernel<false, true, S>), grid, block, 0, h->stream, a);
  else PROF_LAUNCH((mfma16_backward_kernel<false, false, S>), grid, block, 0, h->stream, a);
}

template <typename S>
void mfma16_launch_forward(altro_hip_batch* h, const Mfma16Args<S>& a) {
  PROF_LAUNCH((mfma16_forward_kernel<S, 3>), dim3(mf_grid(h->batch)), dim3(64), 0, h->stream, a);
}

}

namespace altro_hip {
namespace capi {

int launch_backward(altro_hip_batch* h, double reg) {
  ProfScope ps(h, 0);
  if (h->plan == ALTRO_HIP_PLAN_MFMA16) {
    const bool sq = (h->flags & ALTRO_HIP_STORE_QBLOCKS) != 0;
    if (h->dtype == ALTRO_HIP_F64) mfma16_launch_backward<double>(h, reg, sq);
    else if (sq || !(h->flags & ALTRO_HIP_F32_PURE)) mfma16_launch_backward<float>(h, reg, sq);
    else {
      auto a = mfma16_args<float>(h, reg);
      if (h->batch % 4 == 0) {
        const dim3 grid(mf_grid(h->batch / 4));
        if (a.has_f) PROF_LAUNCH((mfma16_backward_f32x4_kernel<true, 2, 2>), grid, dim3(64), 0, h->stream, a);
        else PROF_LAUNCH((mfma16_backward_f32x4_kernel<false, 2, 2>), grid, dim3(64), 0, h->stream, a);
      } else if (a.has_f) PROF_LAUNCH((mfma16_backward_f32_kernel<true, 3>), dim3(mf_grid(h->batch)), dim3(64), 0, h->stream, a);
      else PROF_LAUNCH((mfma16_backward_f32_kernel<false, 3>), dim3(mf_grid(h->batch)), dim3(64), 0, h->stream, a);
    }
  } else if (h->plan == ALTRO_HIP_PLAN_LANE) {
    return h->dtype == ALTRO_HIP_F64 ? lane_launch<double>(h, true, reg) : lane_launch<float>(h, true, reg);
  } else if (h->g_tile && !h->is_diag) {
    int rc = tile32_launch_backward(h, reg);
    if (rc) return rc;
  } else {
    const bool f64 = h->dtype == ALTRO_HIP_F64;
    const size_t lds4 = f64 ? generic_backward_lds_bytes<double>(h->n, h->m) : generic_backward_lds_bytes<float>(h->n, h->m);
    const size_t lds3 = f64 ? generic_backward_lds_bytes<double>(h->n, h->m, true) : generic_backward_lds_bytes<float>(h->n, h->m, true);
    const auto per_cu = [](size_t lds) { return (int)std::min<size_t>(16, (160 * 1024) / std::max<size_t>(lds, 1)); };
    const int cus = 256;
    bool late_q = lds4 > kGenericLdsLimit ? lds3 <= kGenericLdsLimit
                                          : (per_cu(lds3) > per_cu(lds4) && (int64_t)h->batch > (int64_t)cus * per_cu(lds4));
    if (form(h, ALTRO_HIP_FORM_GENERIC_LATE_Q_ON)) late_q = lds3 <= kGenericLdsLimit;
    else if (form(h, ALTRO_HIP_FORM_GENERIC_LATE_Q_OFF)) late_q = false;
    const size_t lds = late_q ? lds3 : lds4;
    const bool big = lds > kGenericLdsLimit;
    if (big && !h->g_ws) {
      int rc = dmalloc(h, &h->g_ws, (size_t)h->batch * ((lds + 15) / 16 * 16));
      if (rc) return rc;
    }
    if (f64) {
      auto a = generic_args<double>(h, reg);
      a.ws = (double*)h->g_ws; a.ws_stride = (int64_t)((lds + 15) / 16 * 16 / sizeof(double));
      const dim3 grid(h->batch), blk(64);
      if (h->g_mfma) {
        if (big) PROF_LAUNCH((generic_backward_kernel<double, true, true>), grid, blk, 0, h->stream, a);
        else if (late_q) PROF_LAUNCH((generic_backward_kernel<double, false, true, true>), grid, blk, lds, h->stream, a);
        else PROF_LAUNCH((generic_backward_kernel<double, false, true>), grid, blk, lds, h->stream, a);
      } else if (big) PROF_LAUNCH((generic_backward_kernel<double, true>), grid, blk, 0, h->stream, a);
      else if (late_q) PROF_LAUNCH((generic_backward_kernel<double, false, false, true>), grid, blk, lds, h->stream, a);
      else PROF_LAUNCH((generic_backward_kernel<double, false>), grid, blk, lds, h->stream, a);
    } else {
      auto a = generic_args<float>(h, reg);
      a.ws = (float*)h->g_ws; a.ws_stride = (int64_t)((lds + 15) / 16 * 16 / sizeof(float));
      if (big) PROF_LAUNCH((generic_backward_kernel<float, true>), dim3(h->batch), dim3(64), 0, h->stream, a);
      else if (late_q) PROF_LAUNCH((generic_backward_kernel<float, false, false, true>), dim3(h->batch), dim3(64), lds, h->stream, a);
      else PROF_LAUNCH((generic_backward_kernel<float, false>), dim3(h->batch), dim3(64), lds, h->stream, a);
    }
// ... 160 lines not shown
```

### altro_amd/csrc/kernels/ilqr_merit2_dpp.hip

```cpp
#pragma once

namespace altro_hip {

constexpr int MD_ZLD = 18;
constexpr int MD_OUT0 = 12 * MD_ZLD;
constexpr int MD_F0 = MD_OUT0 + MF_OUT;
constexpr int MD_NOM0 = MD_F0 + 12;
constexpr int MD_CP0 = MD_NOM0 + MF_NOM;
constexpr int MD_IMG = MD_CP0 + MF_COSTP;
constexpr int MD_IMG_DENSE = MD_CP0 + MF_COST;
static_assert(MF_DYN % 2 == 0 && MF_OUT % 2 == 0 && MF_NOM % 2 == 0 && MF_COSTP % 2 == 0 && MD_IMG % 2 == 0, "records move as pairs");

typedef double md_d2 __attribute__((ext_vector_type(2)));
typedef float md_f2 __attribute__((ext_vector_type(2)));
template <typename S> struct md_pair_of;
template <> struct md_pair_of<double> { typedef md_d2 type; };
template <> struct md_pair_of<float> { typedef md_f2 type; };
template <typename S>
__device__ __forceinline__ md_d2 md_ld(const S* __restrict__ p, int pair) {
  const typename md_pair_of<S>::type v = *reinterpret_cast<const typename md_pair_of<S>::type*>(p + 2 * pair);
  return md_d2{(double)v[0], (double)v[1]};
}
template <bool DENSE = false>
struct MeritPairRegs { md_d2 z[3], f, o[3], nm, cp[DENSE ? 3 : 1]; };
// ... 533 lines not shown
        tile_model_step<MK, true>(a.mp, w, jr, xn, cR);
      } else {
        tile_model_step<MK, false>(a.mp, w, jr, xn, cR);
#pragma unroll
        for (int c = 0; c < 16; ++c) cR[c] = 0.0;
      }
      md_rows16(zacc, zacc2, s2, t2, w, dw, cR);
      if (DUAL && kStat && cand && isx) {
#pragma unroll
        for (int c = 0; c < 16; ++c) L[jr * MD_ZLD + c] = cR[c];
      }
      if (live && wqr && isx) {
        S* zd = const_cast<S*>(a.dyn) + (size_t)b * a.dyn_bs + (size_t)kc * a.dyn_ks;
#pragma unroll
        for (int c = 0; c < 16; ++c) zd[MF_OFF_Z + j * 16 + c] = (S)cR[c];
        zd[MF_OFF_F + j] = S(0);
      }
    } else {
#pragma unroll
      for (int c = 0; c < 16; ++c) cR[c] = L[jr * MD_ZLD + c];
      md_rows16(zacc, zacc2, s2, t2, w, dw, cR);
      xn = (zacc + s2) + L[MD_F0 + jr];
    }
    const double dxn = zacc2 + t2;
    double l;
    if constexpr (DENSE) {
      double cW[16];
#pragma unroll
      for (int c = 0; c < 16; ++c) cW[c] = L[rw[c]];
      double g = 0.0;
      md_chain16(g, w, cW);
      if (live) {
        J += 0.5 * (w * g) + cl * w;
        if (j == 0) J += L[MD_CP0 + MF_COSTD_C];
      }
      l = g + cl;
    } else {
      if (live) {
        J += 0.5 * (w * (cq * w)) + cl * w;
        if (j == 0) J += L[MD_CP0 + 32];
      }
      l = __builtin_fma(cq, w, cl);
    }
    if (al) {
      if constexpr (FUSE) l -= colsum;
      else l -= alp_col(kc_s, j, jvr, Gdyn MD_UARGS(false));
      if (live) kc_s = kn_s;
    }
    if (live) dJ += l * dw;
    if (cand) {
      S* c = candb + (size_t)(live ? k : N) * a.xuy_ks;
      if (isx) c[j] = (S)x;
      c[12 + j] = (S)(isx ? y : uval);
      if (live && wqr) a.cin[(size_t)b * a.cin_bs + (size_t)kc * a.cin_ks + MF_OFF_QR + j] = (S)l;
    }
    if (live) { lprev = l; yprev = y; if (isx) { x = xn; dxda = dxn; } }
   }
  }
  if (!AFF || ke == N) {
    if constexpr (AFF) {
      const double xb = sensb[(size_t)N * sens_ks + jr], sv = sensb[(size_t)N * sens_ks + 12 + jr];
      x = isx ? xb + dalpha * sv : 0.0; dxda = isx ? sv : 0.0;
    }
    if (sens_out && isx) {
      double* sp_ = const_cast<double*>(sensb) + (size_t)N * sens_ks;
      sp_[j] = x; sp_[12 + j] = dxda;
    }
    const S* nm = a.nom + ((size_t)N * a.batch + b) * MF_NOM;
    const S* on = a.outn + (size_t)b * MF_TERM;
    S* c = candb + (size_t)N * a.xuy_ks;
    const double dxN = x - (double)nm[jr];
    double Qd = 0.0, q, gN = 0.0;
    if constexpr (DENSE) {
      const S* cT = a.costd_term + (size_t)b * MF_TERM;
      double cQ[12];
#pragma unroll
      for (int cc = 0; cc < 12; ++cc) cQ[cc] = (double)cT[jr * 12 + cc];
      q = (double)cT[144 + jr];
      md_col12(gN, isx ? x : 0.0, cQ);
      if (isx) {
        J += 0.5 * (x * gN) + q * x;
        if (j == 0) J += (double)a.costd[((size_t)N * a.batch + b) * MF_COST + MF_COSTD_C];
      }
    } else {
      const S* cp = a.costp + ((size_t)N * a.batch + b) * MF_COSTP;
      Qd = (double)cp[jr]; q = (double)cp[16 + jr];
      if (isx) {
        J += 0.5 * (x * (Qd * x)) + q * x;
        if (j == 0) J += (double)cp[32];
      }
    }
    if (al) {
      double Ja = 0.0, vv = 0.0;
#ifdef MD_USER_BLOCKS
      tile_user_eval_knot(*(const AlKnot ALTRO_CONST_AS*)(a.al.knots + N), isx ? x : 0.0, j, uimg_row);
#endif
      if constexpr (DUAL) {
        alp_rows<SOC, NC, FUSE>(kc_s, isx ? x : 0.0, rho, j, rowb, jvr, Ja, vv, Gdyn, zg, jr, &colsum MD_UARGS(true));
        Jal += Ja;
      } else {
        alp_rows<SOC, NC, FUSE>(kc_s, isx ? x : 0.0, rho, j, rowb, jvr, Jal, vv, Gdyn, zg, jr, &colsum MD_UARGS(true));
      }
      if (cand) viol = fmax(viol, vv);
    }
    double cP[13];
#pragma unroll
    for (int cc = 0; cc < 13; ++cc) cP[cc] = (double)on[jr * 13 + cc];
// ... 300 lines not shown
#pragma unroll
          for (int i = 0; i < 8; ++i) ai[i] = mk[i] * cC[i];
          md_outer_rows<0>(tile, ai);
          tile_counts = false;
        }
      }
    } else if constexpr (!BOUNDS) {
      double valv[AL_MAXSOC], zev[AL_MAXSOC], zpv[AL_MAXSOC];
      md_gather4(val, valv);
      md_gather4(ze, zev);
      soc_projection<double>(p, zev, zpv);
      double Jc[AL_MAXSOC * AL_MAXSOC];
      soc_jacobian<double>(p, zev, Jc);
#pragma unroll
      for (int r = 0; r < AL_MAXSOC; ++r) {
        double sj = 0.0;
#pragma unroll
        for (int q = 0; q < AL_MAXSOC; ++q) sj += Jc[q + r * AL_MAXSOC] * zpv[q];
        if (r < p && j == r) jv = sj;
      }
      if (grad) md_chain8(scol, jv, cC);
      if (hess) {
        double ai[8];
#pragma unroll
        for (int i = 0; i < 8; ++i) {
          double jr2 = 0.0;
          if (i < AL_MAXSOC) {
#pragma unroll
            for (int q = 0; q < AL_MAXSOC; ++q)
              if (q < p) jr2 += Jc[i + q * AL_MAXSOC] * cC[q];
          }
          ai[i] = (i < p) ? jr2 : 0.0;
        }
        md_outer_rows<0>(tile, ai);
        tile_counts = false;
        double Hp[AL_MAXSOC * AL_MAXSOC], hc[4];
        soc_hessian<double>(p, zev, zpv, Hp);
#pragma unroll
        for (int i = 0; i < AL_MAXSOC; ++i) {
          double hh = 0.0;
#pragma unroll
          for (int q = 0; q < AL_MAXSOC; ++q)
            if (q < p) hh += Hp[i + q * AL_MAXSOC] * cC[q];
          hc[i] = (i < p) ? hh : 0.0;
        }
        md_cross_rows<0>(tile, cC, hc);
      }
    }
  }
  if (!on) return;
  if (grad && on_g) {
    double l = DENSE ? gW + cl : cq * w + cl;
    l -= scol;
    if (!terminal) a.cin[(size_t)b * a.cin_bs + (size_t)k * a.cin_ks + MF_OFF_QR + j] = (S)l;
    else if (j < 12) a.term[(size_t)b * MF_TERM + 144 + j] = (S)l;
  }
  if (hess && on_h) {
    const bool diag_only = BOUNDS && (a.mode & EXPAND_DIAG) != 0;
#pragma unroll
    for (int r = 0; r < 16; ++r) {
      if (terminal && (r >= 12 || j >= 12)) continue;
      if (r < 12 && j >= 12) continue;
      if (!terminal && r < 12 && j < r) continue;
      if (diag_only && r != j) continue;
      double v = DENSE ? cW[r] : ((r == j) ? cq : 0.0);
      if constexpr (BOUNDS) v += rho * ((r == j) ? dacc : 0.0);
      else v += rho * tile[r];
      if (terminal) a.term[(size_t)b * MF_TERM + r * 12 + j] = (S)v;
      else if (r < 12) a.cin[(size_t)b * a.cin_bs + (size_t)k * a.cin_ks + MF_OFF_Q + mf_sym(r, j)] = (S)v;
      else a.cin[(size_t)b * a.cin_bs + (size_t)k * a.cin_ks + MF_OFF_HR + (r - 12) * 16 + j] = (S)v;
    }
  }
}

template <typename S>
__global__ __launch_bounds__(64) void wave_dual_update_dpp_kernel(IlqrWaveArgs<S> a) {
  const int lane = threadIdx.x, j = lane & 15;
  const int wpk = (a.batch + 3) >> 2;
  const int k = (int)(blockIdx.x / wpk), b0 = (int)(blockIdx.x % wpk) * 4, b_own = b0 + (lane >> 4);
  if (k > a.N || !a.al.enabled) return;
  const bool on = b_own < a.batch && a.prob[b_own < a.batch ? b_own : 0].dual != 0;
  const unsigned long long onm = __ballot(on);
  if (onm == 0ull) return;
  const int b = on ? b_own : b0 + (__builtin_ctzll(onm) >> 4);
  const bool terminal = k == a.N;
  const S* c = a.cand + (size_t)b * a.xuy_bs + (size_t)k * a.xuy_ks;
  const double w = j < 12 ? (double)c[j] : (terminal ? 0.0 : (double)c[12 + j]);
  double jvr[AL_TILE_MAXC], cost = 0.0, viol = 0.0;
#ifdef MD_USER_BLOCKS
  __shared__ double uimg[4][MD_UIMG_ROW];
  dpp_al_rows<S, true>(a.al, k, b, a.batch, w, terminal, a.prob[b].rho_est, j, jvr, cost, viol, on, uimg[lane >> 4]);
#else
  dpp_al_rows<S, true>(a.al, k, b, a.batch, w, terminal, a.prob[b].rho_est, j, jvr, cost, viol, on);
#endif
}
template <typename S>
__global__ __launch_bounds__(64) void wave_feasibility_dpp_kernel(IlqrWaveArgs<S> a) {
  const int lane = threadIdx.x, j = lane & 15;
  const int wpk = (a.batch + 3) >> 2;
  const int k = (int)(blockIdx.x / wpk), b0 = (int)(blockIdx.x % wpk) * 4, b_own = b0 + (lane >> 4);
  if (k > a.N) return;
  bool on = b_own < a.batch;
  if (on && a.active && !a.active[b_own]) on = false;
  if (on && a.skip && a.skip[b_own]) on = false;
  const unsigned long long onm = __ballot(on);
  if (onm == 0ull) return;
  const int b = on ? b_own : b0 + (__builtin_ctzll(onm) >> 4);
  const bool terminal = k == a.N;
  const S* c = a.cand + (size_t)b * a.xuy_bs + (size_t)k * a.xuy_ks;
  const double w = j < 12 ? (double)c[j] : (terminal ? 0.0 : (double)c[12 + j]);
  double jvr[AL_TILE_MAXC], cost = 0.0, viol = 0.0;
#ifdef MD_USER_BLOCKS
  __shared__ double uimg[4][MD_UIMG_ROW];
  dpp_al_rows<S>(a.al, k, b, a.batch, w, terminal, a.prob[b].rho, j, jvr, cost, viol, false, uimg[lane >> 4]);
#else
  dpp_al_rows<S>(a.al, k, b, a.batch, w, terminal, a.prob[b].rho, j, jvr, cost, viol);
#endif
#pragma unroll
  for (int o = 8; o > 0; o >>= 1) viol = fmax(viol, __shfl_xor(viol, o, 64));
  if (j == 0 && on && viol > 0.0)
    atomicMax(reinterpret_cast<unsigned long long*>(&a.prob[b].feasibility), (unsigned long long)__double_as_longlong(viol));
// ... 5 lines not shown
```

### altro_amd/csrc/kernels/ilqr_mfma16.hip

```cpp
#pragma once
#include "../rtc_compat.h"

#include "ilqr_types.h"
#include "mfma16_layout.h"
#include "al_lane.hip"

namespace altro_hip {

__device__ __forceinline__ double wave_sum(double v) {
#pragma unroll
  for (int o = 32; o > 0; o >>= 1) v += __shfl_xor(v, o, 64);
  return v;
}
__device__ __forceinline__ double wave_max(double v) {
#pragma unroll
  for (int o = 32; o > 0; o >>= 1) v = fmax(v, __shfl_xor(v, o, 64));
  return v;
}

template <typename S, int ROW0 = 48>
__device__ __forceinline__ void wave_al_rows(const AlTable<S>& t, int k, int b, int64_t B, const double* xs, const double* us,
                                             bool terminal, double rho_est, int lane, double* jv, double* Jm, double* Hm,
                                             double& cost, double& viol, bool dual_update) {
  int zshift;
// ... 85 lines not shown
  int zshift;
  const AlKnot ALTRO_CONST_AS& kn = al_knot<S>(t, k, zshift);
  double s = 0.0;
#pragma unroll
  for (int c = 0; c < AL_TILE_MAXC; ++c)
    if (c < kn.ncon) {
      const int p = kn.p[c];
      const S* G = t.G + kn.G_off[c];
      for (int i = 0; i < p; ++i) s += (double)G[i + e * p] * w[c * AL_MAXP + i];
    }
  return s;
}

template <typename S>
__global__ __launch_bounds__(64) void wave_rollout_kernel(IlqrWaveArgs<S> a) {
  constexpr int ZLD = 17;
  __shared__ double zimg[12 * ZLD + 12], xs[12], us[4];
  const int b = mf_problem(blockIdx.x, a.batch), lane = threadIdx.x;
  if (b >= a.batch) return;
  if (a.active && !a.active[b]) return;
  const int N = a.N;
  const int i = lane < 12 ? lane : 11;
  const bool init = (a.mode & ROLLOUT_INIT) != 0;
  const int e16 = lane & 15;
  const S* __restrict__ dynb = a.dyn + (size_t)b * a.dyn_bs;
  S* __restrict__ candb = a.cand + (size_t)b * a.xuy_bs;
  double x = (double)a.x0[(size_t)b * 12 + i];
  double zr[3], fr, ur, cq = 0.0, cl = 0.0;
  auto load = [&](int k) {
    const S* z = dynb + (size_t)k * a.dyn_ks;
#pragma unroll
    for (int c = 0; c < 3; ++c) zr[c] = (double)z[MF_OFF_Z + c * 64 + lane];
    fr = (double)z[MF_OFF_F + i];
    ur = (double)candb[(size_t)k * a.xuy_ks + 24 + (lane & 3)];
    if (init) {
      const S* cp = a.costp + ((size_t)k * a.batch + b) * MF_COSTP;
      cq = (double)cp[e16]; cl = (double)cp[16 + e16];
    }
  };
  load(0);
  for (int k = 0; k < N; ++k) {
    __syncthreads();
#pragma unroll
    for (int c = 0; c < 3; ++c) zimg[(4 * c + (lane >> 4)) * ZLD + (lane & 15)] = zr[c];
    zimg[12 * ZLD + i] = fr;
    if (lane < 4) us[lane] = ur;
    if (lane < 12) { xs[lane] = x; candb[(size_t)k * a.xuy_ks + lane] = (S)x; }
    const double cqk = cq, clk = cl;
    load(k + 1 < N ? k + 1 : N - 1);
    __syncthreads();
    if (init && lane < 16) {
      const double z = (double)(S)(lane < 12 ? x : us[lane - 12]);
      a.nom[((size_t)k * a.batch + b) * MF_NOM + lane] = (S)z;
      a.cin[(size_t)b * a.cin_bs + (size_t)k * a.cin_ks + MF_OFF_QR + lane] = (S)(cqk * z + clk);
    }
    double acc = 0.0;
#pragma unroll
    for (int j = 0; j < 12; ++j) acc += zimg[i * ZLD + j] * xs[j];
    double acc2 = 0.0;
#pragma unroll
    for (int cc = 0; cc < 4; ++cc) acc2 += zimg[i * ZLD + 12 + cc] * us[cc];
    x = (acc + acc2) + zimg[12 * ZLD + i];
  }
  if (lane < 12) a.cand[(size_t)b * a.xuy_bs + (size_t)a.N * a.xuy_ks + lane] = (S)x;
  if (init && lane < 16) {
    const S* cp = a.costp + ((size_t)N * a.batch + b) * MF_COSTP;
    const double z = (double)(S)x;
    a.nom[((size_t)N * a.batch + b) * MF_NOM + lane] = lane < 12 ? (S)z : S(0);
    if (lane < 12) a.term[(size_t)b * MF_TERM + 144 + lane] = (S)((double)cp[lane] * z + (double)cp[16 + lane]);
  }
}

template <typename S>
__global__ void wave_accept_kernel(IlqrWaveArgs<S> a) {
  const int64_t total = (int64_t)a.batch * (a.N + 1) * 16;
  for (int64_t t = blockIdx.x * (int64_t)blockDim.x + threadIdx.x; t < total; t += (int64_t)gridDim.x * blockDim.x) {
    const int e = (int)(t % 16);
    const int64_t r = t / 16;
    const int b = (int)(r % a.batch);
    const int k = (int)(r / a.batch);
    if (a.active && !a.active[b]) continue;
    const S* c = a.cand + (size_t)b * a.xuy_bs + (size_t)k * a.xuy_ks;
    S v = S(0);
    if (e < 12) v = c[e];
    else if (k < a.N) v = c[24 + e - 12];
    a.nom[((size_t)k * a.batch + b) * MF_NOM + e] = v;
  }
}

template <typename S>
__global__ __launch_bounds__(64) void wave_spec_select_kernel(IlqrWaveArgs<S> a) {
  const int b = blockIdx.x;
  if (b >= a.batch) return;
  const int sl = a.spec_sel[b];
  if (sl <= 0) return;
  const int total = (a.N + 1) * 28;
  const S* __restrict__ src = a.cand_spec + (size_t)(sl - 1) * a.spec_stride + (size_t)b * a.xuy_bs;
  S* __restrict__ dst = a.cand + (size_t)b * a.xuy_bs;
  for (int t = threadIdx.x; t < total; t += 64) {
    const int k = t / 28, e = t - 28 * k;
    const size_t off = (size_t)k * a.xuy_ks + e;
    dst[off] = src[off];
  }
}

template <typename S>
__global__ void wave_expand_grad_kernel(IlqrWaveArgs<S> a) {
  const int64_t total = (int64_t)(a.N + 1) * a.batch * 16;
  for (int64_t t = blockIdx.x * (int64_t)blockDim.x + threadIdx.x; t < total; t += (int64_t)gridDim.x * blockDim.x) {
    const int e = (int)(t & 15);
    const int b = (int)((t >> 4) % a.batch);
    const int k = (int)((t >> 4) / a.batch);
    if (a.active && !a.active[b]) continue;
    const bool terminal = k == a.N;
    if (terminal && e >= 12) continue;
    const S* c = a.cand + (size_t)b * a.xuy_bs + (size_t)k * a.xuy_ks;
    const S* cp = a.costp + ((size_t)k * a.batch + b) * MF_COSTP;
    const double z = (double)c[e < 12 ? e : 12 + e];
    const double l = (double)cp[e] * z + (double)cp[16 + e];
    if (terminal) a.term[(size_t)b * MF_TERM + 144 + e] = (S)l;
    else a.cin[(size_t)b * a.cin_bs + (size_t)k * a.cin_ks + MF_OFF_QR + e] = (S)l;
  }
}

template <typename S>
__global__ void wave_expand_grad_dense_kernel(IlqrWaveArgs<S> a) {
  const int64_t total = (int64_t)(a.N + 1) * a.batch * 16;
  for (int64_t t = blockIdx.x * (int64_t)blockDim.x + threadIdx.x; t < total; t += (int64_t)gridDim.x * blockDim.x) {
    const int e = (int)(t & 15);
    const int b = (int)((t >> 4) % a.batch);
    const int k = (int)((t >> 4) / a.batch);
    if (a.active && !a.active[b]) continue;
    const bool terminal = k == a.N;
    if (terminal && e >= 12) continue;
    const S* c = a.cand + (size_t)b * a.xuy_bs + (size_t)k * a.xuy_ks;
    double acc = 0.0, lin;
    if (!terminal) {
      const S* cd = a.costd + ((size_t)k * a.batch + b) * MF_COST;
#pragma unroll
      for (int cc = 0; cc < 16; ++cc) {
        const double wv = (double)cd[e < 12 ? (cc < 12 ? MF_OFF_Q + mf_sym(e, cc) : MF_OFF_HR + (cc - 12) * 16 + e) : MF_OFF_HR + (e - 12) * 16 + cc];
        acc = __builtin_fma((double)c[cc < 12 ? cc : 12 + cc], wv, acc);
      }
      lin = (double)cd[MF_OFF_QR + e];
    } else {
      const S* cT = a.costd_term + (size_t)b * MF_TERM;
#pragma unroll
      for (int cc = 0; cc < 12; ++cc) acc = __builtin_fma((double)c[cc], (double)cT[e * 12 + cc], acc);
      lin = (double)cT[144 + e];
    }
    const double l = acc + lin;
    if (terminal) a.term[(size_t)b * MF_TERM + 144 + e] = (S)l;
    else a.cin[(size_t)b * a.cin_bs + (size_t)k * a.cin_ks + MF_OFF_QR + e] = (S)l;
  }
}

template <typename S>
__global__ __launch_bounds__(64) void wave_expand_kernel(IlqrWaveArgs<S> a) {
  __shared__ double xs[12], us[4], jv[AL_TILE_MAXC * AL_MAXP], Jm[AL_TILE_MAXC * 64], Hm[AL_TILE_MAXC * 16];
  const int lane = threadIdx.x;
  const int64_t wk = blockIdx.x;
  const int b = (int)(wk % a.batch), k = (int)(wk / a.batch);
  if (k > a.N) return;
  if (a.active && !a.active[b]) return;
  const bool terminal = k == a.N;
  const bool grad = (a.mode & EXPAND_GRADIENT) != 0, hess = (a.mode & EXPAND_HESSIAN) != 0;
  const S* c = a.cand + (size_t)b * a.xuy_bs + (size_t)k * a.xuy_ks;
  const S* cp = a.costp + ((size_t)k * a.batch + b) * MF_COSTP;
  if (lane < 12) xs[lane] = (double)c[lane];
  if (lane >= 12 && lane < 16) us[lane - 12] = terminal ? 0.0 : (double)c[24 + lane - 12];
  __syncthreads();
  const bool al = a.al.enabled != 0;
  if (al) {
    double cost = 0.0, viol = 0.0;
    wave_al_rows<S>(a.al, k, b, a.batch, xs, us, terminal, a.prob[b].rho_est, lane, jv, Jm, Hm, cost, viol, false);
  }
  __syncthreads();
  if (grad && lane < 16) {
    const int e = lane;
    if (e < 12) {
      double lx = (double)cp[e] * xs[e] + (double)cp[16 + e];
      if (al) lx -= wave_al_col<S>(a.al, k, e, jv);
      if (!terminal) a.cin[(size_t)b * a.cin_bs + (size_t)k * a.cin_ks + MF_OFF_QR + e] = (S)lx;
      else a.term[(size_t)b * MF_TERM + 144 + e] = (S)lx;
    } else if (!terminal) {
      double lu = (double)cp[e] * us[e - 12] + (double)cp[16 + e];
      if (al) lu -= wave_al_col<S>(a.al, k, e, jv);
      a.cin[(size_t)b * a.cin_bs + (size_t)k * a.cin_ks + MF_OFF_QR + e] = (S)lu;
    }
  }
  if (hess && al) {
    const double rho = a.prob[b].rho;
    int zshift;
    const AlKnot ALTRO_CONST_AS& kn = al_knot<S>(a.al, k, zshift);
    for (int t = lane; t < 256; t += 64) {
      const int r = t / 16, cc = t % 16;
      if (terminal && (r >= 12 || cc >= 12)) continue;
      if (r < 12 && cc >= 12) continue;
      if (!terminal && r < 12 && cc < r) continue;
      double v = (r == cc) ? (double)cp[r] : 0.0;
      double s = 0.0;
      for (int cidx = 0; cidx < kn.ncon; ++cidx) {
        const int p = kn.p[cidx];
        const S* G = a.al.G + kn.G_off[cidx];
        const double* Jc = Jm + cidx * 64;
        if (kn.cone[cidx] != CONE_SOC && kn.sel[cidx]) {
          if (r == cc)
            for (int i = 0; i < p; ++i) {
              const int code = kn.sidx[cidx][i];
              if ((code < 0 ? -code : code) - 1 != r) continue;
              const double jg = Jc[i * 8 + i] * (code < 0 ? -1.0 : 1.0);
              s += jg * jg;
            }
        } else if (kn.cone[cidx] != CONE_SOC) {
          for (int i = 0; i < p; ++i) {
            const double jii = Jc[i * 8 + i];
            double jr = 0.0, jc = 0.0;
            jr += jii * (double)G[i + r * p]; jc += jii * (double)G[i + cc * p];
            s += jr * jc;
          }
        } else {
          for (int i = 0; i < p; ++i) {
            double jr = 0.0, jc = 0.0;
            for (int q = 0; q < p; ++q) { jr += Jc[i * 8 + q] * (double)G[q + r * p]; jc += Jc[i * 8 + q] * (double)G[q + cc * p]; }
            s += jr * jc;
          }
        }
        if (kn.cone[cidx] == CONE_SOC) {
          const double* Hc = Hm + cidx * 16;
          for (int i = 0; i < p; ++i) {
            double hc = 0.0;
            for (int q = 0; q < p; ++q) hc += Hc[i * 4 + q] * (double)G[q + cc * p];
            s += (double)G[i + r * p] * hc;
          }
        }
      }
      v += rho * s;
      if (terminal) a.term[(size_t)b * MF_TERM + r * 12 + cc] = (S)v;
      else if (r < 12) a.cin[(size_t)b * a.cin_bs + (size_t)k * a.cin_ks + MF_OFF_Q + mf_sym(r, cc)] = (S)v;
      else a.cin[(size_t)b * a.cin_bs + (size_t)k * a.cin_ks + MF_OFF_HR + (r - 12) * 16 + cc] = (S)v;
    }
  }
}

template <typename S>
__global__ __launch_bounds__(64) void wave_dual_update_kernel(IlqrWaveArgs<S> a) {
  __shared__ double xs[12], us[4], jv[AL_TILE_MAXC * AL_MAXP], Jm[AL_TILE_MAXC * 64], Hm[AL_TILE_MAXC * 16];
  const int lane = threadIdx.x;
  const int64_t wk = blockIdx.x;
  const int b = (int)(wk % a.batch), k = (int)(wk / a.batch);
  if (k > a.N || !a.al.enabled) return;
  if (!a.prob[b].dual) return;
  const bool terminal = k == a.N;
  const S* c = a.cand + (size_t)b * a.xuy_bs + (size_t)k * a.xuy_ks;
  if (lane < 12) xs[lane] = (double)c[lane];
  if (lane >= 12 && lane < 16) us[lane - 12] = terminal ? 0.0 : (double)c[24 + lane - 12];
  __syncthreads();
  double cost = 0.0, viol = 0.0;
  wave_al_rows<S>(a.al, k, b, a.batch, xs, us, terminal, a.prob[b].rho_est, lane, jv, nullptr, nullptr, cost, viol, true);
}

constexpr int MW_ZLD = 17;
constexpr int MW_OUT0 = 12 * MW_ZLD;
constexpr int MW_F0 = MW_OUT0 + MF_OUT;
constexpr int MW_NOM0 = MW_F0 + 12;
constexpr int MW_CP0 = MW_NOM0 + 16;
constexpr int MW_IMG = MW_CP0 + MF_COSTP;
struct MeritWaveRegs { double z[3], o[3], f, nm, cp; };
template <typename S>
__device__ __forceinline__ void merit_wave_load(MeritWaveRegs& r, const S* __restrict__ z, const S* __restrict__ o,
                                                const S* __restrict__ nm, const S* __restrict__ cp, int lane) {
#pragma unroll
  for (int c = 0; c < 3; ++c) r.z[c] = (double)z[MF_OFF_Z + c * 64 + lane];
#pragma unroll
  for (int c = 0; c < 2; ++c) r.o[c] = (double)o[c * 64 + lane];
  r.o[2] = (double)o[128 + (lane & 15)];
  r.f = (double)z[MF_OFF_F + (lane < 12 ? lane : 11)];
  r.nm = (double)nm[lane & 15];
  r.cp = (double)cp[lane < MF_COSTP ? lane : MF_COSTP - 1];
}
__device__ __forceinline__ void merit_wave_stage(const MeritWaveRegs& r, double* __restrict__ L, int lane) {
#pragma unroll
  for (int c = 0; c < 3; ++c) L[c * 4 * MW_ZLD + (lane >> 4) * MW_ZLD + (lane & 15)] = r.z[c];
#pragma unroll
  for (int c = 0; c < 2; ++c) L[MW_OUT0 + c * 64 + lane] = r.o[c];
  L[MW_OUT0 + 128 + (lane & 15)] = r.o[2];
  L[MW_F0 + (lane < 12 ? lane : 11)] = r.f;
  L[MW_NOM0 + (lane & 15)] = r.nm;
  L[MW_CP0 + (lane < MF_COSTP ? lane : MF_COSTP - 1)] = r.cp;
}

// ... 78 lines not shown
#pragma unroll
    for (int j = 0; j < 12; ++j) {
      const double rj = img[ra[j]];
      acc += rj * vec[vbase + j];
      acc2 += rj * das[j];
    }
    const double aff = img[ra[12]];
    double uval = 0.0, duval = 0.0;
    if (is_u) {
      const double d = -aff;
      uval = img[MW_NOM0 + 12 + ia] + (-acc + alpha * d);
      duval = -acc2 + d;
      us[ia] = uval; dus[ia] = duval;
      crec[24 + ia] = uval;
      const double Rd = img[MW_CP0 + 12 + ia], rr = img[MW_CP0 + 28 + ia];
      if (live) J += 0.5 * (uval * (Rd * uval)) + rr * uval;
    }
    if (is_y) crec[12 + i] = acc + aff;
    __syncthreads();
    double xn = 0.0, dxn = 0.0;
    if (is_x) {
      double s2 = 0.0, t2 = 0.0;
#pragma unroll
      for (int cc = 0; cc < 4; ++cc) { const double bic = img[i * MW_ZLD + 12 + cc]; s2 += bic * us[cc]; t2 += bic * dus[cc]; }
      xn = (acc + s2) + img[MW_F0 + i];
      dxn = acc2 + t2;
      const double Qd = img[MW_CP0 + i], q = img[MW_CP0 + 16 + i];
      if (live) {
        J += 0.5 * (x * (Qd * x)) + q * x;
        if (lane == 0) J += img[MW_CP0 + 32];
      }
    }
    if (al) {
      double Jal = 0.0;
      wave_al_rows<S>(a.al, kc, b, a.batch, xs, us, false, rho, lane, jv, nullptr, nullptr, Jal, viol, false);
      if (live) J += Jal;
    }
    __syncthreads();
    if (deriv && lane < 16) {
      const int e = lane;
      const double pt = e < 12 ? x : us[e - 12];
      double l = img[MW_CP0 + e] * pt + img[MW_CP0 + 16 + e];
      if (al) l -= wave_al_col<S>(a.al, kc, e, jv);
      qrec[e] = l;
      if (live) dJ += l * (e < 12 ? dxda : dus[e - 12]);
    }
    __syncthreads();
    {
      S* c = candb + (size_t)(live ? k : N) * a.xuy_ks;
      c[l27] = (S)crec[l27];
      if (deriv) {
        S* ci = a.cin + (size_t)b * a.cin_bs + (size_t)kc * a.cin_ks;
        const double qv = qrec[sub];
        if (live && store) ci[MF_OFF_QR + sub] = (S)qv;
      }
    }
    if (is_x && live) { x = xn; dxda = dxn; }
   }
  }
  __syncthreads();
  {
    const S* nm = a.nom + ((size_t)N * a.batch + b) * MF_NOM;
    const S* cp = a.costp + ((size_t)N * a.batch + b) * MF_COSTP;
    const S* on = a.outn + (size_t)b * MF_TERM;
    S* c = candb + (size_t)N * a.xuy_ks;
    if (is_u) c[24 + ia] = S(0);
    if (is_x) {
      xs[lane] = x;
      dxs[lane] = x - (double)nm[lane];
      c[lane] = (S)x;
      const double Qd = (double)cp[i], q = (double)cp[16 + i];
      J += 0.5 * (x * (Qd * x)) + q * x;
      if (lane == 0) J += (double)cp[32];
    }
    __syncthreads();
    if (al) wave_al_rows<S>(a.al, N, b, a.batch, xs, us, true, rho, lane, jv, nullptr, nullptr, J, viol, false);
    if (is_y) {
      double s = 0.0;
#pragma unroll
      for (int j = 0; j < 12; ++j) s += (double)on[i * 13 + j] * dxs[j];
      c[12 + i] = (S)(s + (double)on[i * 13 + 12]);
    }
    __syncthreads();
    if (deriv && is_x) {
      double lx = (double)cp[i] * x + (double)cp[16 + i];
      if (al) lx -= wave_al_col<S>(a.al, N, i, jv);
      if (store) a.term[(size_t)b * MF_TERM + 144 + i] = (S)lx;
      dJ += lx * dxda;
    }
  }
  const double phi = wave_sum(J), dphi = wave_sum(dJ);
  if (lane == 0) {
    a.phi[(size_t)trial * a.batch + b] = phi;
    if (deriv) a.dphi[(size_t)trial * a.batch + b] = dphi;
    if (al) a.prob[b].rho_est = rho;
  }
}

__device__ __forceinline__ double half_sum(double v) {
#pragma unroll
  for (int o = 16; o > 0; o >>= 1) v += __shfl_xor(v, o, 64);
  return v;
}

template <typename S>
__global__ __launch_bounds__(64) void wave_stationarity_kernel(IlqrWaveArgs<S> a) {
  const int b = mf_problem(blockIdx.x, a.batch), lane = threadIdx.x;
  if (b >= a.batch) return;
  if (a.active && !a.active[b]) return;
  if (a.skip && a.skip[b]) return;
  const int N = a.N;
  const int j = lane & 15;
  double res = 0.0;
  for (int k = lane >> 4; k < N; k += 4) {
    const S* z = a.dyn + (size_t)b * a.dyn_bs + (size_t)k * a.dyn_ks;
    const S* ci = a.cin + (size_t)b * a.cin_bs + (size_t)k * a.cin_ks;
    const S* c = a.cand + (size_t)b * a.xuy_bs + (size_t)k * a.xuy_ks;
    const S* cn = a.cand + (size_t)b * a.xuy_bs + (size_t)(k + 1) * a.xuy_ks;
    double s = 0.0;
#pragma unroll
    for (int i = 0; i < 12; ++i) s += (double)z[i * 16 + j] * (double)cn[12 + i];
    const double g = (double)ci[MF_OFF_QR + j] + s;
    res = fmax(res, fabs(j < 12 ? g - (double)c[12 + j] : g));
  }
  if (lane < 12)
    res = fmax(res, fabs((double)a.term[(size_t)b * MF_TERM + 144 + lane] -
                         (double)a.cand[(size_t)b * a.xuy_bs + (size_t)N * a.xuy_ks + 12 + lane]));
  res = wave_max(res);
  double viol = 0.0;
  const bool feas_here = (a.mode & STAT_NO_FEAS) == 0;
  if (a.al.enabled && feas_here) {
    __shared__ double xs[12], us[4], jv[AL_TILE_MAXC * AL_MAXP], Jm[AL_TILE_MAXC * 64], Hm[AL_TILE_MAXC * 16];
    const double rho = a.prob[b].rho;
    for (int k = 0; k <= N; ++k) {
      const S* c = a.cand + (size_t)b * a.xuy_bs + (size_t)k * a.xuy_ks;
      __syncthreads();
      if (lane < 12) xs[lane] = (double)c[lane];
      if (lane >= 12 && lane < 16) us[lane - 12] = k < N ? (double)c[24 + lane - 12] : 0.0;
      __syncthreads();
      double cost = 0.0;
      wave_al_rows<S>(a.al, k, b, a.batch, xs, us, k == N, rho, lane, jv, nullptr, nullptr, cost, viol, false);
    }
    viol = wave_max(viol);
  }
  if (lane == 0) { a.prob[b].stationarity = res; a.prob[b].feasibility = viol; }
}

template <typename S>
__global__ void wave_shift_kernel(IlqrWaveArgs<S> a) {
  const int64_t total = (int64_t)a.batch * 16;
  for (int64_t t = blockIdx.x * (int64_t)blockDim.x + threadIdx.x; t < total; t += (int64_t)gridDim.x * blockDim.x) {
    const int e = (int)(t % 16);
    const int b = (int)(t / 16);
    const int el = e < 12 ? e : 24 + (e - 12);
    const int kend = e < 12 ? a.N : a.N - 1;
    S* c = a.cand + (size_t)b * a.xuy_bs + el;
    for (int k = 0; k < kend; ++k) c[(size_t)k * a.xuy_ks] = c[(size_t)(k + 1) * a.xuy_ks];
  }
}

}
```

### altro_amd/csrc/kernels/ilqr_types.h

```cpp
#pragma once
#include "../rtc_compat.h"

#include "../linesearch_sm.h"
#include "../models.h"
#include "al_types.h"
#include "mfma16_layout.h"

namespace altro_hip {

struct IlqrProb {
  int running;
  int iterations;
  int status;
  int ls_failed;
  double phi0, dphi0, alpha, stationarity;
  int ls_iters, evaluating;
  LsState ls;
  double rho, rho_est, feasibility;
  int dual, n_dual_updates;
  int reg_retries;
};

template <typename T>
struct IlqrArgs {
// ... 52 lines not shown
  int stat_inline = 0;
  int* stat_done = nullptr;
  int* guard = nullptr;
  int* active_exact = nullptr;
  int aff_fed = 0;
  int aff_exact = 0;
  double decision_margin = 0.0;
  int batch;
  int iter;
  int iterations_max;
  double tol_stationarity, tol_meritfun_gradient, tol_primal_feasibility;
  double penalty_initial, penalty_scaling, penalty_max;
  int al_enabled;
  double* reg;
  const int* bwd_status;
  double reg_initial, reg_scale, reg_min, reg_max;
  LsOptions ls;
};


template <typename S>
struct IlqrWaveArgs {
  const S* dyn;   int64_t dyn_bs, dyn_ks;
  S* cin;         int64_t cin_bs, cin_ks;
  S* term;
  const S* out;   int64_t out_bs, out_ks;
  const S* outn;
  S* nom;
  S* cand;        int64_t xuy_bs, xuy_ks;
  const S* costp;
  const S* x0;
  const double* alpha;
  const int* active;
  S* cand_spec; int64_t spec_stride; int spec_trials; int spec_pre; double ls_beta; int ls_max_iters;
  const int* spec_sel;
  double* phi;
  double* dphi;
  IlqrProb* prob;
  int N, batch, want_derivative;
  double alpha_const;
  AlTable<S> al;
  int mode;
  double penalty_scaling = 10.0, penalty_max = 1e8;
  const int* skip = nullptr;
  const S* costd = nullptr;
  const S* costd_term = nullptr;
  int cost_dense = 0;
  ModelParams mp{MODEL_LINEAR, 0.0f, 0, 2.7, 1.5};
  double* sens = nullptr;
  double* sens_alpha = nullptr;
  double* aff_part = nullptr;
  int* aff_on = nullptr;
  int aff = 0;
};
constexpr int ROLLOUT_INIT = 4;

template <typename S>
int ilqr_wave_launch_kernel(hipStream_t stream, int which, const IlqrWaveArgs<S>& a);
template <typename S>
int ilqr_wave_launch_model(hipStream_t stream, int which, const IlqrWaveArgs<S>& a);
bool ilqr_tile_model_supported(int kind, int n, int m);
template <typename S>
int ilqr_wave_launch_wide(hipStream_t stream, int which, const IlqrWaveArgs<S>& a);

constexpr int ILQR_SPEC_TRIALS = 8;
enum IlqrKernel { IK_ROLLOUT, IK_ACCEPT, IK_EXPAND, IK_MERIT, IK_STATIONARITY, IK_DUAL, IK_SHIFT, IK_SPEC_SELECT,
                  IK_MERIT2  };
enum IlqrLoopKernel { ILK_LOOP_INIT, ILK_LS_BEGIN, ILK_LS_FEED, ILK_FINISH_ITER, ILK_MARK_RUNNING, ILK_SET_PENALTY,
                      ILK_PENALTY_UPDATE, ILK_REG_RETRY };

template <typename T>
struct LaneArgs;
constexpr int ILQR_FUSED_PHASES = 12;
struct IlqrResult {
  int status, iterations;
  double stationarity, final_alpha, final_phi, primal_feasibility, penalty;
  int dual_updates, reg_retries;
};
struct IlqrPollRec {
  IlqrResult result;
  double u0[4];
  int done, reserved;
};
struct IlqrFusedArgs {
  int first_iter;
  int max_sweeps;
  int reg_retry_max;
  int use_reg;
  int* counters;
  unsigned long long* clk;
  int prologue;
  IlqrPollRec* poll = nullptr;
  int* poll_count = nullptr;
  const int* list = nullptr;
  int list_count = 0;
  int group = 0;
  int* run_flags = nullptr;
};
template <typename T, int G>
int ilqr_launch_fused_g(hipStream_t stream, int kind, int n, int m, const IlqrArgs<T>& a, const IlqrLoopArgs& la,
                        const LaneArgs<T>& ba, const IlqrFusedArgs& fa);
inline int ilqr_fused_group(int batch) { return batch <= 8 * 256 ? 8 : batch <= 16 * 256 ? 16 : 32; }
template <typename T>
inline int ilqr_launch_fused(hipStream_t stream, int kind, int n, int m, const IlqrArgs<T>& a, const IlqrLoopArgs& la,
                             const LaneArgs<T>& ba, const IlqrFusedArgs& fa) {
  const int G = fa.list ? fa.group : ilqr_fused_group(a.batch);
// ... 19 lines not shown
```

### altro_amd/csrc/kernels/mfma16_layout.h

```cpp
#pragma once

namespace altro_hip {

constexpr int MF_N = 12, MF_M = 4;
constexpr int MF_TRI = 78;
constexpr int MF_DYN = 204;
constexpr int MF_COST = 160;
constexpr int MF_IN = MF_DYN + MF_COST;
constexpr int MF_OUT = 144;
constexpr int MF_TERM = 156;
constexpr int MF_OFF_Z = 0, MF_OFF_F = 192;
constexpr int MF_OFF_Q = 0, MF_OFF_HR = 80, MF_OFF_QR = 144;
constexpr int MF_OFF_P = 52, MF_OFF_p = 130, MF_OFF_PAD = 142;
constexpr int MF_QB = 256 + 16;
constexpr int MF_TERM_q = 144;
constexpr int MF_XUY = 28;
constexpr int MF_XUY_X = 0, MF_XUY_Y = 12, MF_XUY_U = 24;
constexpr int MF_NOM = 16;
constexpr int MF_NOM_X = 0, MF_NOM_U = 12;
constexpr int MF_COSTP = 36;
constexpr int MF_COSTP_QD = 0, MF_COSTP_RD = 12, MF_COSTP_q = 16, MF_COSTP_r = 28, MF_COSTP_c = 32;
constexpr int MF_COSTD_C = 78;

__host__ __device__ constexpr int mf_tri_row(int i) { return 12 * i - (i * (i - 1)) / 2; }
__host__ __device__ constexpr int mf_sym(int i, int j) {
  return i <= j ? mf_tri_row(i) + (j - i) : mf_tri_row(j) + (i - j);
}
static_assert(mf_sym(11, 11) == MF_TRI - 1, "packed triangle size");
static_assert(MF_COST % 8 == 0 && MF_OUT % 8 == 0, "records are whole 64-byte lines");

constexpr int MF_XCDS = 8;
__host__ __device__ constexpr int mf_grid(int batch) { return MF_XCDS * ((batch + MF_XCDS - 1) / MF_XCDS); }
__host__ __device__ constexpr int mf_problem(int block, int batch) {
  return (block % MF_XCDS) * ((batch + MF_XCDS - 1) / MF_XCDS) + block / MF_XCDS;
}

}
```

### altro_amd/csrc/kernels/pack.hip

```cpp
#pragma once
#include <hip/hip_runtime.h>
#include <stdint.h>

#include "mfma16_layout.h"

namespace altro_hip {

struct SrcArr {
  const double* p;
  int64_t bs, ks;
  int bmod;
};
__device__ __forceinline__ int64_t src_b(const SrcArr& s, int b) { return s.bmod > 0 ? (b % s.bmod) : b; }

template <typename T>
__global__ void expand_copy_kernel(T* dst, int64_t dst_bs, int64_t dst_ks, SrcArr src, int block,
                                   int nk, int b0, int nb) {
  const int64_t total = (int64_t)nb * nk * block;
  for (int64_t t = blockIdx.x * (int64_t)blockDim.x + threadIdx.x; t < total;
       t += (int64_t)gridDim.x * blockDim.x) {
    const int e = (int)(t % block);
    const int k = (int)((t / block) % nk);
    const int b = (int)(t / ((int64_t)block * nk));
    dst[(int64_t)(b0 + b) * dst_bs + (int64_t)k * dst_ks + e] =
        (T)src.p[(src.bmod > 0 ? src_b(src, b0 + b) : (int64_t)b) * src.bs + (int64_t)k * src.ks + e];
  }
}

template <typename T>
__global__ void gather_copy_kernel(double* out, int64_t out_bs, int64_t out_ks, const T* src,
                                   int64_t src_bs, int64_t src_ks, int block, int nk, int b0, int nb) {
  const int64_t total = (int64_t)nb * nk * block;
  for (int64_t t = blockIdx.x * (int64_t)blockDim.x + threadIdx.x; t < total;
       t += (int64_t)gridDim.x * blockDim.x) {
    const int e = (int)(t % block);
    const int k = (int)((t / block) % nk);
    const int b = (int)(t / ((int64_t)block * nk));
    out[(int64_t)b * out_bs + (int64_t)k * out_ks + e] =
        (double)src[(int64_t)(b0 + b) * src_bs + (int64_t)k * src_ks + e];
  }
}

struct Mfma16Strides { int64_t in_bs, in_ks, out_bs, out_ks, xuy_bs, xuy_ks, cin_bs, cin_ks; };

enum Mfma16Seg { MSEG_Z = 0, MSEG_F, MSEG_Q, MSEG_HR, MSEG_QR, MSEG_TERM_Q, MSEG_TERM_q };

template <typename S>
__global__ void mfma16_pack_kernel(S* in, S* cin, S* term, Mfma16Strides st, int seg, SrcArr s0,
                                   SrcArr s1, int is_diag, int N, int b0, int nb, int n, int m) {
  int len, base;
  switch (seg) {
    case MSEG_Z: len = 192; base = MF_OFF_Z; break;
    case MSEG_F: len = 12; base = MF_OFF_F; break;
    case MSEG_Q: len = MF_TRI; base = MF_OFF_Q; break;
    case MSEG_HR: len = 64; base = MF_OFF_HR; break;
    case MSEG_QR: len = 16; base = MF_OFF_QR; break;
    case MSEG_TERM_Q: len = 144; base = 0; break;
    default: len = 12; base = 144; break;
  }
  const bool terminal = (seg == MSEG_TERM_Q || seg == MSEG_TERM_q);
  const int nk = terminal ? 1 : N;
  const int64_t total = (int64_t)nb * nk * len;
  for (int64_t t = blockIdx.x * (int64_t)blockDim.x + threadIdx.x; t < total;
       t += (int64_t)gridDim.x * blockDim.x) {
    const int e = (int)(t % len);
    const int k = terminal ? N : (int)((t / len) % nk);
    const int b = (int)(t / ((int64_t)len * nk));
    const double* p0 = s0.p ? s0.p + src_b(s0, b0 + b) * s0.bs + (int64_t)k * s0.ks : nullptr;
    const double* p1 = s1.p ? s1.p + src_b(s1, b0 + b) * s1.bs + (int64_t)k * s1.ks : nullptr;
    double v = 0.0;
    switch (seg) {
      case MSEG_Z: {
        const int c = e / 64, l = e % 64, col = l & 15, row = (l >> 4) + 4 * c;
        if (row < n) {
          if (col < 12) v = col < n ? p0[row + n * col] : 0.0;
          else v = col - 12 < m ? p1[row + n * (col - 12)] : 0.0;
        }
      } break;
      case MSEG_F: v = (p0 && e < n) ? p0[e] : 0.0; break;
      case MSEG_Q: {
        int row = 0, rem = e;
        while (rem >= 12 - row) { rem -= 12 - row; ++row; }
        const int jj = row + rem;
        if (jj < n) v = is_diag ? (row == jj ? p0[row] : 0.0) : p0[row + n * jj];
      } break;
      case MSEG_TERM_Q: {
        const int row = e / 12, jj = e % 12;
        if (row < n && jj < n) v = is_diag ? (row == jj ? p0[row] : 0.0) : p0[row + n * jj];
      } break;
      case MSEG_HR: {
        const int g = e / 16, jj = e % 16;
        if (g >= m) v = (jj == 12 + g) ? 1.0 : 0.0;
        else if (jj < 12) v = (is_diag || !p0 || jj >= n) ? 0.0 : p0[g + m * jj];
        else if (jj - 12 < m) v = is_diag ? (g == jj - 12 ? p1[g] : 0.0) : p1[g + m * (jj - 12)];
      } break;
      case MSEG_QR: v = (e < 12) ? (e < n ? p0[e] : 0.0) : (e - 12 < m ? p1[e - 12] : 0.0); break;
      default: v = e < n ? p0[e] : 0.0; break;
    }
    if (terminal) term[(int64_t)(b0 + b) * MF_TERM + base + e] = (S)v;
    else if (seg == MSEG_Z || seg == MSEG_F) in[(int64_t)(b0 + b) * st.in_bs + (int64_t)k * st.in_ks + base + e] = (S)v;
    else cin[(int64_t)(b0 + b) * st.cin_bs + (int64_t)k * st.cin_ks + base + e] = (S)v;
  }
}

enum Mfma16Get { MGET_K = 0, MGET_d, MGET_P, MGET_p, MGET_x, MGET_u, MGET_y, MGET_QBLK };

template <typename S>
__global__ void mfma16_unpack_kernel(double* dst, int what, const S* out, const S* outn,
                                     const S* xuy, const S* qblk, Mfma16Strides st, int N,
                                     int b0, int nb, int n, int m) {
  int len, nk;
  switch (what) {
    case MGET_K: len = m * n; nk = N; break;
    case MGET_d: len = m; nk = N; break;
    case MGET_P: len = n * n; nk = N + 1; break;
    case MGET_p: len = n; nk = N + 1; break;
    case MGET_x: len = n; nk = N + 1; break;
    case MGET_u: len = m; nk = N; break;
    case MGET_y: len = n; nk = N + 1; break;
    default: len = n * n + m * m + m * n + n + m; nk = N; break;
  }
  const int64_t total = (int64_t)nb * nk * len;
  for (int64_t t = blockIdx.x * (int64_t)blockDim.x + threadIdx.x; t < total;
       t += (int64_t)gridDim.x * blockDim.x) {
    const int e = (int)(t % len);
    const int k = (int)((t / len) % nk);
    const int b = b0 + (int)(t / ((int64_t)len * nk));
    const S* o = (k < N) ? out + (int64_t)b * st.out_bs + (int64_t)k * st.out_ks : nullptr;
    const S* pn = outn + (int64_t)b * MF_TERM;
    const S* xr = xuy ? xuy + (int64_t)b * st.xuy_bs + (int64_t)k * st.xuy_ks : nullptr;
    double v;
    switch (what) {
      case MGET_K: v = (double)o[(e % m) * 13 + (e / m)]; break;
      case MGET_d: v = -(double)o[e * 13 + 12]; break;
      case MGET_P:
        v = (k < N) ? (double)o[MF_OFF_P + mf_sym(e % n, e / n)] : (double)pn[(e % n) * 13 + (e / n)];
        break;
      case MGET_p: v = (k < N) ? (double)o[MF_OFF_p + e] : (double)pn[e * 13 + 12]; break;
      case MGET_x: v = xr[e]; break;
      case MGET_y: v = xr[12 + e]; break;
      case MGET_u: v = xr[24 + e]; break;
      default: {
        const S* q = qblk + ((int64_t)b * N + k) * MF_QB;
        const int oxx = n * n, ouu = oxx + m * m, oux = ouu + m * n, ox = oux + n;
        if (e < oxx) v = q[(e % n) * 16 + (e / n)];
        else if (e < ouu) { int t2 = e - oxx; v = q[(12 + t2 % m) * 16 + 12 + t2 / m]; }
        else if (e < oux) { int t2 = e - ouu; v = q[(12 + t2 % m) * 16 + t2 / m]; }
        else if (e < ox) v = q[256 + (e - oux)];
        else v = q[256 + 12 + (e - ox)];
      } break;
    }
    dst[t] = v;
  }
}
// ... 3 lines not shown
```

### altro_amd/csrc/kernels/tvlqr_mfma16.hip

```cpp
#pragma once
#include <hip/hip_runtime.h>
#include <stdint.h>

#include "mfma16_layout.h"

namespace altro_hip {

typedef double f64x4 __attribute__((ext_vector_type(4)));

__device__ __forceinline__ f64x4 mfma_f64_16x16x4(double a, double b, f64x4 c) {
  return __builtin_amdgcn_mfma_f64_16x16x4f64(a, b, c, 0, 0, 0);
}

template <int CTRL>
__device__ __forceinline__ double dpp_mov_f64(double v) {
  union { double d; int i[2]; } in, out;
  in.d = v;
  out.i[0] = __builtin_amdgcn_update_dpp(in.i[0], in.i[0], CTRL, 0xf, 0xf, false);
  out.i[1] = __builtin_amdgcn_update_dpp(in.i[1], in.i[1], CTRL, 0xf, 0xf, false);
  return out.d;
}
__device__ __forceinline__ double row16_allreduce(double v) {
  v += dpp_mov_f64<0xB1>(v);
  v += dpp_mov_f64<0x4E>(v);
  v += dpp_mov_f64<0x141>(v);
  v += dpp_mov_f64<0x140>(v);
  return v;
}
__device__ __forceinline__ double dpp_col12_dup(double v) {
  union { double d; int i[2]; } in, out;
  in.d = v;
  out.i[0] = __builtin_amdgcn_update_dpp(in.i[0], in.i[0], 0x00, 0xf, 0x8, false);
  out.i[1] = __builtin_amdgcn_update_dpp(in.i[1], in.i[1], 0x00, 0xf, 0x8, false);
  return out.d;
}
__device__ __forceinline__ double group4_allreduce(double v) {
  v += __shfl_xor(v, 16, 64);
  v += __shfl_xor(v, 32, 64);
  return v;
}

template <typename S>
struct Mfma16Args {
  const S* in;
  int64_t in_bs, in_ks, out_bs, out_ks, xuy_bs, xuy_ks, cin_bs, cin_ks;
  const S* cin;
  const S* term;
  S* out;
  S* outn;
  S* qblk;
  S* trash;
  const S* x0;
  S* xuy;
  S* delta_V;
  int* status;
  int N;
  int batch;
  double reg;
  int has_f;
  const int* active;
  const double* reg_pp;
};

template <typename S>
__device__ __forceinline__ double ld_stream(const S* p) {
  return (double)(*p);
}

constexpr int MF_PT_LD = 17;

struct Mfma16Knot {
  double z[3], q[3], hr, qr, f[3];
};
struct Mfma16QOff { int o[3]; };
__device__ __forceinline__ Mfma16QOff mfma16_q_offsets(int j, int g) {
  const int jq = (j < 12) ? j : 11;
  Mfma16QOff q;
#pragma unroll
  for (int r = 0; r < 3; ++r) q.o[r] = MF_OFF_Q + mf_sym(g + 4 * r, jq);
  return q;
}

template <bool HAS_F, typename S>
__device__ __forceinline__ void mfma16_load_knot(Mfma16Knot& kn, const S* __restrict__ rec,
                                                 const S* __restrict__ crec, int lane, int j, int g,
                                                 const Mfma16QOff& qo) {
#pragma unroll
  for (int c = 0; c < 3; ++c) kn.z[c] = ld_stream(&rec[MF_OFF_Z + c * 64 + lane]);
#pragma unroll
  for (int r = 0; r < 3; ++r) kn.q[r] = ld_stream(&crec[qo.o[r]]);
  kn.hr = ld_stream(&crec[MF_OFF_HR + lane]);
  kn.qr = ld_stream(&crec[MF_OFF_QR + j]);
  if (HAS_F) {
#pragma unroll
    for (int r = 0; r < 3; ++r) kn.f[r] = ld_stream(&rec[MF_OFF_F + g + 4 * r]);
  } else {
    kn.f[0] = kn.f[1] = kn.f[2] = 0.0;
  }
}

__device__ __forceinline__ double rsqrt_nr(double x) {
  const double y = __builtin_amdgcn_rsq(x);
  const double e = __builtin_fma(-x, y * y, 1.0);
  const double t = __builtin_fma(0.375, e, 0.5);
  return __builtin_fma(y * e, t, y);
}

template <bool STORE_Q, bool HAS_F, typename S>
__global__ __launch_bounds__(64, 4) void mfma16_backward_kernel(Mfma16Args<S> a) {
  __shared__ __attribute__((aligned(16))) double lds[64 + 16 + 2];
  __shared__ double ptile[12 * MF_PT_LD];
  const int lane = threadIdx.x;
  const int j = lane & 15, g = lane >> 4;
  const int b = mf_problem(blockIdx.x, a.batch);
  if (b >= a.batch) return;
  if (a.active && !a.active[b]) return;
  const int N = a.N;
  if (lane < 2) lds[80 + lane] = 0.0;
  int rhs_idx[4];
#pragma unroll
  for (int r = 0; r < 4; ++r) rhs_idx[r] = (j < 12) ? (r * 16 + j) : ((j == 12) ? (64 + 12 + r) : 80);
  const int qmine_idx = (j < 12) ? lane : ((j == 12) ? (64 + 12 + g) : 80);
  int qx_idx[3];
#pragma unroll
  for (int r = 0; r < 3; ++r) qx_idx[r] = (j == 12) ? (64 + g + 4 * r) : 80;
  const S* __restrict__ in = a.in + (size_t)b * a.in_bs;
  const S* __restrict__ cin = a.cin + (size_t)b * a.cin_bs;
  S* __restrict__ out = a.out + (size_t)b * a.out_bs;
  const bool col_ok = (j <= 12);
  const int jc = col_ok ? j : 12;
  S* __restrict__ trash = a.trash + (size_t)b * MF_OUT;
  const Mfma16QOff qo = mfma16_q_offsets(j, g);
  int p_off[3];
#pragma unroll
  for (int r = 0; r < 3; ++r) {
    const int row = g + 4 * r;
    p_off[r] = (j == 12) ? MF_OFF_p + row : ((j < 12 && j >= row) ? MF_OFF_P + mf_sym(row, j) : MF_OFF_PAD + (j > 12 ? 1 : 0));
  }

  int pt_wr[3], pt_rd[3];
#pragma unroll
  for (int r = 0; r < 3; ++r) {
    const int row = g + 4 * r;
    pt_wr[r] = row * MF_PT_LD + j;
    pt_rd[r] = (j < 12 && j < row) ? j * MF_PT_LD + row : pt_wr[r];
  }

  double Pt[3];
  {
    const S* term = a.term + (size_t)b * MF_TERM;
    S* on = a.outn + (size_t)b * MF_TERM;
#pragma unroll
    for (int r = 0; r < 3; ++r) {
      double v = 0.0;
      if (j < 12) v = (double)term[r * 48 + g * 12 + j];
      else if (j == 12) v = (double)term[144 + g + 4 * r];
      Pt[r] = v;
      if (col_ok) on[(g + 4 * r) * 13 + j] = (S)v;
    }
  }
  double dv0 = 0.0, dv1 = 0.0;
  int fail_k = -1;
  const double reg = a.reg_pp ? a.reg_pp[b] : a.reg;

  Mfma16Knot cur, nxt;
  mfma16_load_knot<HAS_F, S>(cur, in + (size_t)(N - 1) * a.in_ks, cin + (size_t)(N - 1) * a.cin_ks, lane, j, g, qo);
  __builtin_amdgcn_s_waitcnt(0x0F70);

  for (int k = N - 1; k >= 0; --k) {
    {
      const size_t kp = (k > 0) ? k - 1 : 0;
      mfma16_load_knot<HAS_F, S>(nxt, in + kp * a.in_ks, cin + kp * a.cin_ks, lane, j, g, qo);
    }

    f64x4 D1 = {0.0, 0.0, 0.0, 0.0};
#pragma unroll
    for (int c = 0; c < 3; ++c) D1 = mfma_f64_16x16x4(Pt[c], cur.z[c], D1);

    f64x4 G = {cur.q[0], cur.q[1], cur.q[2], cur.hr};
#pragma unroll
    for (int c = 0; c < 3; ++c) G = mfma_f64_16x16x4(cur.z[c], D1[c], G);

    double gv = D1[3] + cur.qr;
    if (HAS_F) {
      double s = cur.f[0] * D1[0] + cur.f[1] * D1[1] + cur.f[2] * D1[2];
      gv += group4_allreduce(s);
    }

    __syncthreads();
    lds[lane] = G[3];
    if (g == 0) lds[64 + j] = gv;
    __syncthreads();
    const double a00 = lds[0 * 16 + 12];
    const double a10 = lds[1 * 16 + 12], a11 = lds[1 * 16 + 13];
    const double a20 = lds[2 * 16 + 12], a21 = lds[2 * 16 + 13], a22 = lds[2 * 16 + 14];
    const double a30 = lds[3 * 16 + 12], a31 = lds[3 * 16 + 13], a32 = lds[3 * 16 + 14], a33 = lds[3 * 16 + 15];
    double rhs[4];
#pragma unroll
    for (int r = 0; r < 4; ++r) rhs[r] = lds[rhs_idx[r]];
    double quu_row[4];
#pragma unroll
    for (int c = 0; c < 4; ++c) quu_row[c] = lds[g * 16 + 12 + c];
    f64x4 Pn;
#pragma unroll
    for (int r = 0; r < 3; ++r) {
      const double qx = lds[qx_idx[r]];
      Pn[r] = (j < 12) ? G[r] : qx;
    }
    Pn[3] = 0.0;
    const double q_mine = lds[qmine_idx];

    const double x0 = a00 + reg;
    const double i0 = rsqrt_nr(x0);
    const double l10 = a10 * i0, l20 = a20 * i0, l30 = a30 * i0;
    const double x1 = (a11 + reg) - l10 * l10;
    const double i1 = rsqrt_nr(x1);
    const double l21 = (a21 - l20 * l10) * i1, l31 = (a31 - l30 * l10) * i1;
    const double x2 = (a22 + reg) - l20 * l20 - l21 * l21;
    const double i2 = rsqrt_nr(x2);
    const double l32 = (a32 - l30 * l20 - l31 * l21) * i2;
    const double x3 = (a33 + reg) - l30 * l30 - l31 * l31 - l32 * l32;
    const double i3 = rsqrt_nr(x3);
    const bool fail = !(x0 > 0.0) || !(x1 > 0.0) || !(x2 > 0.0) || !(x3 > 0.0);
    const bool was_alive = (fail_k < 0);
    if (was_alive && fail) fail_k = k;
    const bool alive = (fail_k < 0);
    const double y0 = rhs[0] * i0;
    const double y1 = (rhs[1] - l10 * y0) * i1;
    const double y2 = (rhs[2] - l20 * y0 - l21 * y1) * i2;
    const double y3 = (rhs[3] - l30 * y0 - l31 * y1 - l32 * y2) * i3;
    const double k3 = y3 * i3;
    const double k2 = (y2 - l32 * k3) * i2;
// ... 212 lines not shown
```

### include/altro_hip/altro_hip.h

```cpp
#ifndef ALTRO_HIP_H_
#define ALTRO_HIP_H_

#include <stddef.h>
#include <stdint.h>

#ifdef __cplusplus
extern "C" {
#endif

#define ALTRO_HIP_VERSION 300
#define ALTRO_HIP_TVLQR_SUCCESS (-1)

typedef struct altro_hip_batch altro_hip_batch;

typedef enum altro_hip_dtype {
  ALTRO_HIP_F64 = 0,
  ALTRO_HIP_F32 = 1
} altro_hip_dtype;

typedef enum altro_hip_error {
  ALTRO_HIP_OK = 0,
  ALTRO_HIP_ERR_NO_DEVICE = -1,
  ALTRO_HIP_ERR_BAD_ARGUMENT = -2,
  ALTRO_HIP_ERR_UNSUPPORTED = -3,
// ... 84 lines not shown
int altro_hip_merit(altro_hip_batch* h, const double* alpha, int alpha_is_uniform, int want_derivative,
                    double* phi, double* dphi);
int altro_hip_stationarity(altro_hip_batch* h, double* stationarity);
int altro_hip_get_nominal(altro_hip_batch* h, double* x, double* u);
int altro_hip_get_expansion(altro_hip_batch* h, double* A, double* B, double* lx, double* lu);

int altro_hip_add_linear_constraint(altro_hip_batch* h, int k_first, int k_last, int cone, int p,
                                    const double* G, const double* g, int g_per_problem);
int altro_hip_clear_constraints(altro_hip_batch* h);
int altro_hip_reset_duals(altro_hip_batch* h, double penalty);
int altro_hip_get_duals(altro_hip_batch* h, int k, int slot, double* z );
int altro_hip_feasibility(altro_hip_batch* h, double* out);

int altro_hip_shift_trajectory(altro_hip_batch* h);
int altro_hip_update_linear_costs(altro_hip_batch* h, const double* q, const double* r, const double* c,
                                  int k_first, int k_last, int kz, int bz);
int altro_hip_get_knot(altro_hip_batch* h, int k, double* x , double* u );

typedef struct altro_hip_solve_options {
  int iterations_max;
  double tol_stationarity;
  double tol_primal_feasibility;
  double tol_meritfun_gradient;
  int use_backtracking_linesearch;
  double penalty_initial;
  double penalty_scaling;
  double penalty_max;
  double reg_initial;
  int reg_retry_max;
  double reg_scale, reg_min, reg_max;
  int stop_when_running_at_most;
  unsigned forms;
  int fused_sweeps;
  double decision_margin;
} altro_hip_solve_options;
#define ALTRO_HIP_FORM_NO_SPECULATION 0x0001u
#define ALTRO_HIP_FORM_NO_RUNAHEAD 0x0002u
#define ALTRO_HIP_FORM_NO_MERIT2 0x0004u
#define ALTRO_HIP_FORM_MERIT_LDS 0x0008u
#define ALTRO_HIP_FORM_MERIT_DPP_ALWAYS 0x0010u
#define ALTRO_HIP_FORM_EXPAND_LDS 0x0020u
#define ALTRO_HIP_FORM_ALROWS_LDS 0x0040u
#define ALTRO_HIP_FORM_ROLLOUT_ROUNDS 0x0080u
#define ALTRO_HIP_FORM_SEQUENCED 0x0100u
#define ALTRO_HIP_FORM_MERIT_ONE_LAUNCH 0x0200u
#define ALTRO_HIP_FORM_LANE_QUAD_OFF 0x0400u
#define ALTRO_HIP_FORM_LANE_QUAD_ON 0x0800u
#define ALTRO_HIP_FORM_GENERIC_LATE_Q_OFF 0x1000u
#define ALTRO_HIP_FORM_GENERIC_LATE_Q_ON 0x2000u
#define ALTRO_HIP_FORM_AFFINE_EXACT 0x8000u
#define ALTRO_HIP_FORM_FUSED_CLOCK 0x4000u
#define ALTRO_HIP_FORM_NO_COMPACTION 0x10000u
#define ALTRO_HIP_FORM_GENERIC_MERIT_LDS 0x20000u
int altro_hip_set_forms(altro_hip_batch* h, unsigned forms);
unsigned altro_hip_get_forms(const altro_hip_batch* h);
typedef struct altro_hip_solve_result {
  int status;
  int iterations;
  double stationarity;
  double final_alpha;
  double final_phi;
  double primal_feasibility;
  double penalty;
  int dual_updates;
  int reg_retries;
} altro_hip_solve_result;
void altro_hip_default_solve_options(altro_hip_solve_options* opts);
int altro_hip_ilqr_solve(altro_hip_batch* h, const altro_hip_solve_options* opts,
                         altro_hip_solve_result* results);
int altro_hip_last_solve_counts(const altro_hip_batch* h, int* sweeps, int* merit_launches);

typedef struct altro_hip_poll_record {
  altro_hip_solve_result result;
  double u0[4];
  int done;
  int reserved;
} altro_hip_poll_record;
int altro_hip_ilqr_solve_async(altro_hip_batch* h, const altro_hip_solve_options* opts);
int altro_hip_ilqr_poll(altro_hip_batch* h, int* n_done, const altro_hip_poll_record** records);
int altro_hip_ilqr_wait(altro_hip_batch* h, altro_hip_solve_result* results);

typedef void (*altro_hip_merit_fn)(double alpha, double* phi, double* dphi, void* ctx);
double altro_hip_linesearch_host(altro_hip_merit_fn f, void* ctx, double alpha0, double phi0, double dphi0,
                                 int try_cubic_first, int use_backtracking, double c1, double c2,
                                 int* status, int* iters, double* phi, double* dphi);

typedef struct altro_hip_stats {
  int64_t problems;
  int64_t cholesky_failures;
  int64_t converged;
  int64_t iterations;
  double sum_cost;
  double sum_delta_V0;
  double sum_delta_V1;
  double max_stationarity;
  double max_feasibility;
  double max_abs_xN;
  int64_t non_finite;
} altro_hip_stats;
int altro_hip_stats_reduce(altro_hip_batch* h, altro_hip_stats* out);

typedef struct altro_hip_comm altro_hip_comm;
#define ALTRO_HIP_COMM_ID_BYTES 128
int altro_hip_comm_unique_id(void* id );
int altro_hip_comm_create(altro_hip_comm** out, int device, int rank, int world, const void* id);
int altro_hip_comm_create_all(altro_hip_comm** out , int ndev, const int* devices);
void altro_hip_comm_destroy(altro_hip_comm* c);
int altro_hip_comm_rank(const altro_hip_comm* c);
// ... 19 lines not shown
```

Measured before the change: 2.694 million.

## Add compact diagonal cost record layout for MFMA16 backward sweep

When costs are diagonal (no dense cost, no custom model, no partial AL constraints), the MFMA16 plan now stores per-knot cost data as a compact 32-element record (diag Q, diag R, q/r) instead of the full packed triangle plus Hr block. The backward kernel gets a template variant that reads this smaller record and rebuilds the sparse G tile in registers. Expansion, merit and pack kernels write into the compact layout, and a conversion kernel switches between forms when conditions change. The aim is to cut per-knot memory traffic in the bandwidth-bound backward sweep, at the cost of extra form-sync bookkeeping and a conversion launch whenever the form changes.

```diff
diff --git a/altro_amd/__init__.py b/altro_amd/__init__.py
--- a/altro_amd/__init__.py
+++ b/altro_amd/__init__.py
@@ -31,7 +31,7 @@
     "altro_hip_set_input_guess", "altro_hip_set_state_guess",
     "altro_hip_open_loop_rollout", "altro_hip_accept", "altro_hip_expand", "altro_hip_merit",
     "altro_hip_stationarity", "altro_hip_get_nominal", "altro_hip_get_expansion",
-    "altro_hip_default_solve_options", "altro_hip_set_forms", "altro_hip_get_forms", "altro_hip_ilqr_solve", "altro_hip_last_solve_counts",
+    "altro_hip_default_solve_options", "altro_hip_set_forms", "altro_hip_get_forms", "altro_hip_cost_record_form", "altro_hip_ilqr_solve", "altro_hip_last_solve_counts",
     "altro_hip_ilqr_solve_async", "altro_hip_ilqr_poll", "altro_hip_ilqr_wait",
     "altro_hip_linesearch_host",
     "altro_hip_add_linear_constraint", "altro_hip_add_user_constraint", "altro_hip_clear_constraints", "altro_hip_reset_duals",
@@ -47,6 +47,7 @@
 FORM_AFFINE_EXACT = 0x8000
 FORM_NO_COMPACTION = 0x10000
 FORM_GENERIC_MERIT_LDS = 0x20000
+FORM_COST_RECORD_DENSE = 0x40000
 
 
 def forms_from_env():
@@ -215,6 +216,7 @@
         L.altro_hip_set_forms.argtypes = [vp, C.c_uint]
         L.altro_hip_get_forms.argtypes = [vp]
         L.altro_hip_get_forms.restype = C.c_uint
+        L.altro_hip_cost_record_form.argtypes = [vp]
         L.altro_hip_ilqr_solve.argtypes = [vp, C.POINTER(SolveOptions), vp]
         L.altro_hip_last_solve_counts.argtypes = [vp, C.POINTER(i), C.POINTER(i)]
         L.altro_hip_ilqr_solve_async.argtypes = [vp, C.POINTER(SolveOptions)]
@@ -523,6 +525,13 @@
         self._forms_user = int(forms)
         self._sync_forms()
 
+    def cost_record_form(self):
+        self._sync_forms()
+        rc = self.L.altro_hip_cost_record_form(self.h)
+        if rc < 0:
+            _check(rc)
+        return rc
+
     def _sync_forms(self):
         want = getattr(self, "_forms_user", 0) | forms_from_env()
         if want != getattr(self, "_forms_set", 0):
diff --git a/altro_amd/csrc/capi_core.hip b/altro_amd/csrc/capi_core.hip
--- a/altro_amd/csrc/capi_core.hip
+++ b/altro_amd/csrc/capi_core.hip
@@ -242,6 +242,32 @@
 
 extern "C++" {
 namespace altro_hip { namespace capi {
+int cost_form_sync(altro_hip_batch* h, bool records_follow) {
+  if (h->plan != ALTRO_HIP_PLAN_MFMA16) return 0;
+  int rc = 0;
+  if (h->al_dirty && (rc = al_upload(h))) return rc;
+  const bool diag = h->is_diag && !h->cost_dense && !(h->flags & ALTRO_HIP_F32_PURE) && !h->model_set && !h->rtc && h->rtc_source.empty() &&
+                    (h->al_defs.empty() || h->al_sum.all_sel) && !form(h, ALTRO_HIP_FORM_COST_RECORD_DENSE);
+  const int want = diag ? COST_FORM_DIAG : COST_FORM_DENSE;
+  if (want == h->cin_form) return 0;
+  const size_t B = (size_t)h->batch, N = (size_t)h->N;
+  if (diag && !h->m_cind && (rc = dmalloc(h, &h->m_cind, B * N * MF_CDIAG * h->esz))) return rc;
+  if (!records_follow) {
+    const int64_t total = (int64_t)B * N * (diag ? MF_CDIAG : MF_COST);
+    const int64_t dg_ks = (int64_t)h->batch * MF_CDIAG;
+    if (h->dtype == ALTRO_HIP_F64)
+      hipLaunchKernelGGL(mfma16_cost_form_kernel<double>, dim3(grid_for(total)), dim3(256), 0, h->stream, (double*)h->m_cin, h->m_st.cin_bs,
+                         h->m_st.cin_ks, (double*)h->m_cind, (int64_t)MF_CDIAG, dg_ks, diag ? 1 : 0, h->N, h->batch);
+    else
+      hipLaunchKernelGGL(mfma16_cost_form_kernel<float>, dim3(grid_for(total)), dim3(256), 0, h->stream, (float*)h->m_cin, h->m_st.cin_bs,
+                         h->m_st.cin_ks, (float*)h->m_cind, (int64_t)MF_CDIAG, dg_ks, diag ? 1 : 0, h->N, h->batch);
+    hipError_t e = hipGetLastError();
+    if (e != hipSuccess) return fail(ALTRO_HIP_ERR_HIP, "mfma16_cost_form launch: %s", hipGetErrorString(e));
+  }
+  h->cin_form = want;
+  h->expansion_current = false;
+  return 0;
+}
 int replan_empty_handle(altro_hip_batch* h, int plan) {
   if (!h->auto_plan || h->dyn_set || h->cost_set || h->model_set || h->lqr_cost_set || h->guess_set || !h->al_defs.empty() ||
       (h->x0_set && h->x0_host.empty()))
@@ -291,7 +317,7 @@
   if (!h) return;
   (void)hipSetDevice(h->device);
   if (h->stream) (void)hipStreamSynchronize(h->stream);
-  void* ptrs[] = {h->x0, h->delta_V, h->status, h->m_in, h->m_cin, h->m_term, h->m_out, h->m_outn, h->m_xuy,
+  void* ptrs[] = {h->x0, h->delta_V, h->status, h->m_in, h->m_cin, h->m_cind, h->m_term, h->m_out, h->m_outn, h->m_xuy,
                   h->m_qblk, h->m_trash, h->g_off, h->g_nx, h->g_nu, h->stage,
                   h->l_in, h->l_term, h->l_out, h->l_outn, h->l_xuy, h->l_x0,
                   h->l_nom, h->l_cost, h->g_ws, h->i_prob, h->i_alpha, h->i_phi, h->i_dphi, h->i_active, h->i_counters,
@@ -366,6 +392,7 @@
   const int n = h->n, m = h->m, N = h->N;
   Dims d{n, m};
   h->is_diag = is_diag ? 1 : 0;
+  if (h->plan == ALTRO_HIP_PLAN_MFMA16 && (rc = cost_form_sync(h, true))) return rc;
   const int nkQ = kz ? 2 : N + 1;
   const int nkR = kz ? 1 : N;
   if (h->plan == ALTRO_HIP_PLAN_MFMA16) {
diff --git a/altro_amd/csrc/capi_ilqr.hip b/altro_amd/csrc/capi_ilqr.hip
--- a/altro_amd/csrc/capi_ilqr.hip
+++ b/altro_amd/csrc/capi_ilqr.hip
@@ -145,7 +145,10 @@
   if (which == IK_MERIT)
     a.mode = form(h, ALTRO_HIP_FORM_MERIT_LDS) ? 0 : form(h, ALTRO_HIP_FORM_MERIT_DPP_ALWAYS) ? 3 : 2;
   a.dyn = (const S*)h->m_in; a.dyn_bs = h->m_st.in_bs; a.dyn_ks = h->m_st.in_ks;
-  a.cin = (S*)h->m_cin; a.cin_bs = h->m_st.cin_bs; a.cin_ks = h->m_st.cin_ks;
+  {
+    const CostRecords cr = cost_records(h);
+    a.cin = (S*)cr.p; a.cin_bs = cr.bs; a.cin_ks = cr.ks; a.cin_diag = cr.diag; a.cin_qr = cr.qr;
+  }
   a.term = (S*)h->m_term; a.out = (const S*)h->m_out; a.out_bs = h->m_st.out_bs; a.out_ks = h->m_st.out_ks;
   a.outn = (const S*)h->m_outn; a.nom = (S*)h->m_nom; a.cand = (S*)h->m_xuy; a.xuy_bs = h->m_st.xuy_bs;
   a.xuy_ks = h->m_st.xuy_ks; a.costp = (const S*)h->m_costp; a.x0 = (const S*)h->x0;
@@ -279,6 +282,7 @@
     return h->dtype == ALTRO_HIP_F64 ? gen_run<double>(h, which, use_alpha, use_active, want_deriv, alpha_const, mode)
                                      : gen_run<float>(h, which, use_alpha, use_active, want_deriv, alpha_const, mode);
   if (h->plan == ALTRO_HIP_PLAN_MFMA16) {
+    if ((rc = cost_form_sync(h))) return rc;
     rc = h->dtype == ALTRO_HIP_F64 ? wave_run<double>(h, which, use_alpha, use_active, want_deriv, alpha_const, mode)
                                    : wave_run<float>(h, which, use_alpha, use_active, want_deriv, alpha_const, mode);
     if (which == IK_MERIT) h->expansion_current = !rc && want_deriv && !use_active && h->spec_trials == 1 && !h->spec_pre && h->al_defs.empty();
@@ -793,7 +797,9 @@
   h->al_defs.clear(); h->al_G.clear(); h->al_g.clear();
   h->al_knots.assign((size_t)h->N + 1, AlKnotBig{});
   h->al_dirty = true;
-  return al_upload(h);
+  rc = al_upload(h);
+  if (!rc && h->plan == ALTRO_HIP_PLAN_MFMA16) rc = cost_form_sync(h);
+  return rc;
 }
 int altro_hip_reset_duals(altro_hip_batch* h, double penalty) {
   int rc = loop_entry(h, true);
@@ -914,9 +920,16 @@
     h->merit_split = -1;
   }
   h->forms = forms;
-  return 0;
+  return h->plan == ALTRO_HIP_PLAN_MFMA16 ? cost_form_sync(h) : 0;
 }
 unsigned altro_hip_get_forms(const altro_hip_batch* h) { return h ? h->forms : 0u; }
+int altro_hip_cost_record_form(altro_hip_batch* h) {
+  int rc = check(h);
+  if (rc) return rc;
+  if (h->plan != ALTRO_HIP_PLAN_MFMA16) return 0;
+  if ((rc = cost_form_sync(h))) return rc;
+  return h->cin_form == COST_FORM_DIAG ? 1 : 0;
+}
 int altro_hip_last_solve_counts(const altro_hip_batch* h, int* sweeps, int* merit_launches) {
   if (!h) return fail(ALTRO_HIP_ERR_BAD_ARGUMENT, "null handle");
   if (sweeps) *sweeps = h->last_sweeps;
@@ -955,7 +968,9 @@
         }
     }
     if (lx || lu) {
-      if ((rc = fetch(h->m_cin, h->m_st.cin_bs, h->m_st.cin_ks, MF_OFF_QR, 16, N))) return rc;
+      if ((rc = cost_form_sync(h))) return rc;
+      const CostRecords cr = cost_records(h);
+      if ((rc = fetch(cr.p, cr.bs, cr.ks, cr.qr, 16, N))) return rc;
       for (int64_t b = 0; b < B_; ++b)
         for (int k = 0; k < N; ++k) {
           const double* qr = raw.data() + ((size_t)b * N + k) * 16;
diff --git a/altro_amd/csrc/capi_internal.h b/altro_amd/csrc/capi_internal.h
--- a/altro_amd/csrc/capi_internal.h
+++ b/altro_amd/csrc/capi_internal.h
@@ -72,6 +72,8 @@
   void *m_in = nullptr, *m_cin = nullptr, *m_term = nullptr, *m_out = nullptr, *m_outn = nullptr, *m_xuy = nullptr,
        *m_qblk = nullptr, *m_trash = nullptr;
   Mfma16Strides m_st{};
+  int cin_form = 0;
+  void* m_cind = nullptr;
   void *l_in = nullptr, *l_term = nullptr, *l_out = nullptr, *l_outn = nullptr, *l_xuy = nullptr,
        *l_x0 = nullptr;
   void *l_nom = nullptr, *l_cost = nullptr;
@@ -162,6 +164,14 @@
 
 inline bool form(const altro_hip_batch* h, unsigned bit) { return (h->forms & bit) != 0; }
 
+enum { COST_FORM_DENSE = 0, COST_FORM_DIAG = 1 };
+int cost_form_sync(altro_hip_batch* h, bool records_follow = false);
+struct CostRecords { void* p; int64_t bs, ks; int diag, qr; };
+inline CostRecords cost_records(const altro_hip_batch* h) {
+  if (h->cin_form == COST_FORM_DIAG) return CostRecords{h->m_cind, MF_CDIAG, (int64_t)h->batch * MF_CDIAG, 1, MF_CDIAG_QR};
+  return CostRecords{h->m_cin, h->m_st.cin_bs, h->m_st.cin_ks, 0, MF_OFF_QR};
+}
+
 inline int dmalloc(altro_hip_batch* h, void** p, size_t bytes) {
   hipError_t e = hipMalloc(p, bytes ? bytes : 16);
   if (e != hipSuccess) {
@@ -393,15 +403,21 @@
 inline int mfma16_pack_launch(altro_hip_batch* h, int seg, SrcArr s0, SrcArr s1, void* cin = nullptr, void* term = nullptr,
                               int is_diag = -1) {
   const int64_t total = (int64_t)h->batch * h->N * 192;
-  if (!cin) cin = h->m_cin;
+  Mfma16Strides st = h->m_st;
+  int cdiag = 0;
+  if (!cin) {
+    const CostRecords cr = cost_records(h);
+    cin = cr.p; st.cin_bs = cr.bs; st.cin_ks = cr.ks; cdiag = cr.diag;
+  }
   if (!term) term = h->m_term;
   if (is_diag < 0) is_diag = h->is_diag;
+  if (cdiag && !is_diag && (seg == MSEG_Q || seg == MSEG_HR)) return fail(ALTRO_HIP_ERR_HIP, "mfma16_pack: a dense cost cannot be packed into diagonal cost records");
   if (h->dtype == ALTRO_HIP_F64)
     hipLaunchKernelGGL(mfma16_pack_kernel<double>, dim3(grid_for(total)), dim3(256), 0, h->stream, (double*)h->m_in,
-                       (double*)cin, (double*)term, h->m_st, seg, s0, s1, is_diag, h->N, 0, h->batch, h->n, h->m);
+                       (double*)cin, (double*)term, st, seg, s0, s1, is_diag, h->N, 0, h->batch, h->n, h->m, cdiag);
   else
     hipLaunchKernelGGL(mfma16_pack_kernel<float>, dim3(grid_for(total)), dim3(256), 0, h->stream, (float*)h->m_in,
-                       (float*)cin, (float*)term, h->m_st, seg, s0, s1, is_diag, h->N, 0, h->batch, h->n, h->m);
+                       (float*)cin, (float*)term, st, seg, s0, s1, is_diag, h->N, 0, h->batch, h->n, h->m, cdiag);
   hipError_t e = hipGetLastError();
   if (e != hipSuccess) return fail(ALTRO_HIP_ERR_HIP, "mfma16_pack launch: %s", hipGetErrorString(e));
   return 0;
diff --git a/altro_amd/csrc/capi_tvlqr.hip b/altro_amd/csrc/capi_tvlqr.hip
--- a/altro_amd/csrc/capi_tvlqr.hip
+++ b/altro_amd/csrc/capi_tvlqr.hip
@@ -121,8 +121,9 @@
 Mfma16Args<S> mfma16_args(altro_hip_batch* h, double reg) {
   Mfma16Args<S> a;
   a.in = (const S*)h->m_in;
-  a.cin = (const S*)h->m_cin;
-  a.cin_bs = h->m_st.cin_bs; a.cin_ks = h->m_st.cin_ks;
+  const CostRecords cr = cost_records(h);
+  a.cin = (const S*)cr.p;
+  a.cin_bs = cr.bs; a.cin_ks = cr.ks; a.cin_diag = cr.diag; a.cin_qr = cr.qr;
   a.in_bs = h->m_st.in_bs; a.in_ks = h->m_st.in_ks; a.out_bs = h->m_st.out_bs; a.out_ks = h->m_st.out_ks;
   a.xuy_bs = h->m_st.xuy_bs; a.xuy_ks = h->m_st.xuy_ks;
   a.term = (const S*)h->m_term; a.out = (S*)h->m_out; a.outn = (S*)h->m_outn; a.qblk = (S*)h->m_qblk;
@@ -135,6 +136,13 @@
 void mfma16_launch_backward(altro_hip_batch* h, double reg, bool sq) {
   auto a = mfma16_args<S>(h, reg);
   const dim3 grid(mf_grid(h->batch)), block(64);
+  if (a.cin_diag) {
+    if (sq && a.has_f) PROF_LAUNCH((mfma16_backward_kernel<true, true, S, true>), grid, block, 0, h->stream, a);
+    else if (sq) PROF_LAUNCH((mfma16_backward_kernel<true, false, S, true>), grid, block, 0, h->stream, a);
+    else if (a.has_f) PROF_LAUNCH((mfma16_backward_kernel<false, true, S, true>), grid, block, 0, h->stream, a);
+    else PROF_LAUNCH((mfma16_backward_kernel<false, false, S, true>), grid, block, 0, h->stream, a);
+    return;
+  }
   if (sq && a.has_f) PROF_LAUNCH((mfma16_backward_kernel<true, true, S>), grid, block, 0, h->stream, a);
   else if (sq) PROF_LAUNCH((mfma16_backward_kernel<true, false, S>), grid, block, 0, h->stream, a);
   else if (a.has_f) PROF_LAUNCH((mfma16_backward_kernel<false, true, S>), grid, block, 0, h->stream, a);
@@ -152,6 +160,10 @@
 namespace capi {
 
 int launch_backward(altro_hip_batch* h, double reg) {
+  if (h->plan == ALTRO_HIP_PLAN_MFMA16) {
+    const int rcf = cost_form_sync(h);
+    if (rcf) return rcf;
+  }
   ProfScope ps(h, 0);
   if (h->plan == ALTRO_HIP_PLAN_MFMA16) {
     const bool sq = (h->flags & ALTRO_HIP_STORE_QBLOCKS) != 0;
diff --git a/altro_amd/csrc/kernels/ilqr_merit2_dpp.hip b/altro_amd/csrc/kernels/ilqr_merit2_dpp.hip
--- a/altro_amd/csrc/kernels/ilqr_merit2_dpp.hip
+++ b/altro_amd/csrc/kernels/ilqr_merit2_dpp.hip
@@ -609,7 +609,8 @@
       S* c = candb + (size_t)(live ? k : N) * a.xuy_ks;
       if (isx) c[j] = (S)x;
       c[12 + j] = (S)(isx ? y : uval);
-      if (live && wqr) a.cin[(size_t)b * a.cin_bs + (size_t)kc * a.cin_ks + MF_OFF_QR + j] = (S)l;
+      const int qr = MK != 0 ? MF_OFF_QR : a.cin_qr;
+      if (live && wqr) a.cin[(size_t)b * a.cin_bs + (size_t)kc * a.cin_ks + qr + j] = (S)l;
     }
     if (live) { lprev = l; yprev = y; if (isx) { x = xn; dxda = dxn; } }
    }
@@ -1016,7 +1017,7 @@
   if (grad && on_g) {
     double l = DENSE ? gW + cl : cq * w + cl;
     l -= scol;
-    if (!terminal) a.cin[(size_t)b * a.cin_bs + (size_t)k * a.cin_ks + MF_OFF_QR + j] = (S)l;
+    if (!terminal) a.cin[(size_t)b * a.cin_bs + (size_t)k * a.cin_ks + a.cin_qr + j] = (S)l;
     else if (j < 12) a.term[(size_t)b * MF_TERM + 144 + j] = (S)l;
   }
   if (hess && on_h) {
@@ -1031,6 +1032,9 @@
       if constexpr (BOUNDS) v += rho * ((r == j) ? dacc : 0.0);
       else v += rho * tile[r];
       if (terminal) a.term[(size_t)b * MF_TERM + r * 12 + j] = (S)v;
+      else if (a.cin_diag) {
+        if (r == j) a.cin[(size_t)b * a.cin_bs + (size_t)k * a.cin_ks + MF_CDIAG_H + r] = (S)v;
+      }
       else if (r < 12) a.cin[(size_t)b * a.cin_bs + (size_t)k * a.cin_ks + MF_OFF_Q + mf_sym(r, j)] = (S)v;
       else a.cin[(size_t)b * a.cin_bs + (size_t)k * a.cin_ks + MF_OFF_HR + (r - 12) * 16 + j] = (S)v;
     }
diff --git a/altro_amd/csrc/kernels/ilqr_mfma16.hip b/altro_amd/csrc/kernels/ilqr_mfma16.hip
--- a/altro_amd/csrc/kernels/ilqr_mfma16.hip
+++ b/altro_amd/csrc/kernels/ilqr_mfma16.hip
@@ -161,7 +161,7 @@
     if (init && lane < 16) {
       const double z = (double)(S)(lane < 12 ? x : us[lane - 12]);
       a.nom[((size_t)k * a.batch + b) * MF_NOM + lane] = (S)z;
-      a.cin[(size_t)b * a.cin_bs + (size_t)k * a.cin_ks + MF_OFF_QR + lane] = (S)(cqk * z + clk);
+      a.cin[(size_t)b * a.cin_bs + (size_t)k * a.cin_ks + a.cin_qr + lane] = (S)(cqk * z + clk);
     }
     double acc = 0.0;
 #pragma unroll
@@ -228,7 +228,7 @@
     const double z = (double)c[e < 12 ? e : 12 + e];
     const double l = (double)cp[e] * z + (double)cp[16 + e];
     if (terminal) a.term[(size_t)b * MF_TERM + 144 + e] = (S)l;
-    else a.cin[(size_t)b * a.cin_bs + (size_t)k * a.cin_ks + MF_OFF_QR + e] = (S)l;
+    else a.cin[(size_t)b * a.cin_bs + (size_t)k * a.cin_ks + a.cin_qr + e] = (S)l;
   }
 }
 
@@ -260,7 +260,7 @@
     }
     const double l = acc + lin;
     if (terminal) a.term[(size_t)b * MF_TERM + 144 + e] = (S)l;
-    else a.cin[(size_t)b * a.cin_bs + (size_t)k * a.cin_ks + MF_OFF_QR + e] = (S)l;
+    else a.cin[(size_t)b * a.cin_bs + (size_t)k * a.cin_ks + a.cin_qr + e] = (S)l;
   }
 }
 
@@ -290,12 +290,12 @@
     if (e < 12) {
       double lx = (double)cp[e] * xs[e] + (double)cp[16 + e];
       if (al) lx -= wave_al_col<S>(a.al, k, e, jv);
-      if (!terminal) a.cin[(size_t)b * a.cin_bs + (size_t)k * a.cin_ks + MF_OFF_QR + e] = (S)lx;
+      if (!terminal) a.cin[(size_t)b * a.cin_bs + (size_t)k * a.cin_ks + a.cin_qr + e] = (S)lx;
       else a.term[(size_t)b * MF_TERM + 144 + e] = (S)lx;
     } else if (!terminal) {
       double lu = (double)cp[e] * us[e - 12] + (double)cp[16 + e];
       if (al) lu -= wave_al_col<S>(a.al, k, e, jv);
-      a.cin[(size_t)b * a.cin_bs + (size_t)k * a.cin_ks + MF_OFF_QR + e] = (S)lu;
+      a.cin[(size_t)b * a.cin_bs + (size_t)k * a.cin_ks + a.cin_qr + e] = (S)lu;
     }
   }
   if (hess && al) {
@@ -346,6 +346,9 @@
       }
       v += rho * s;
       if (terminal) a.term[(size_t)b * MF_TERM + r * 12 + cc] = (S)v;
+      else if (a.cin_diag) {
+        if (r == cc) a.cin[(size_t)b * a.cin_bs + (size_t)k * a.cin_ks + MF_CDIAG_H + r] = (S)v;
+      }
       else if (r < 12) a.cin[(size_t)b * a.cin_bs + (size_t)k * a.cin_ks + MF_OFF_Q + mf_sym(r, cc)] = (S)v;
       else a.cin[(size_t)b * a.cin_bs + (size_t)k * a.cin_ks + MF_OFF_HR + (r - 12) * 16 + cc] = (S)v;
     }
@@ -530,7 +533,7 @@
       if (deriv) {
         S* ci = a.cin + (size_t)b * a.cin_bs + (size_t)kc * a.cin_ks;
         const double qv = qrec[sub];
-        if (live && store) ci[MF_OFF_QR + sub] = (S)qv;
+        if (live && store) ci[a.cin_qr + sub] = (S)qv;
       }
     }
     if (is_x && live) { x = xn; dxda = dxn; }
@@ -598,7 +601,7 @@
     double s = 0.0;
 #pragma unroll
     for (int i = 0; i < 12; ++i) s += (double)z[i * 16 + j] * (double)cn[12 + i];
-    const double g = (double)ci[MF_OFF_QR + j] + s;
+    const double g = (double)ci[a.cin_qr + j] + s;
     res = fmax(res, fabs(j < 12 ? g - (double)c[12 + j] : g));
   }
   if (lane < 12)
diff --git a/altro_amd/csrc/kernels/ilqr_types.h b/altro_amd/csrc/kernels/ilqr_types.h
--- a/altro_amd/csrc/kernels/ilqr_types.h
+++ b/altro_amd/csrc/kernels/ilqr_types.h
@@ -128,6 +128,7 @@
   double* aff_part = nullptr;
   int* aff_on = nullptr;
   int aff = 0;
+  int cin_diag = 0, cin_qr = MF_OFF_QR;
 };
 constexpr int ROLLOUT_INIT = 4;
 
diff --git a/altro_amd/csrc/kernels/mfma16_layout.h b/altro_amd/csrc/kernels/mfma16_layout.h
--- a/altro_amd/csrc/kernels/mfma16_layout.h
+++ b/altro_amd/csrc/kernels/mfma16_layout.h
@@ -11,6 +11,8 @@
 constexpr int MF_TERM = 156;
 constexpr int MF_OFF_Z = 0, MF_OFF_F = 192;
 constexpr int MF_OFF_Q = 0, MF_OFF_HR = 80, MF_OFF_QR = 144;
+constexpr int MF_CDIAG = 32;
+constexpr int MF_CDIAG_H = 0, MF_CDIAG_QR = 16;
 constexpr int MF_OFF_P = 52, MF_OFF_p = 130, MF_OFF_PAD = 142;
 constexpr int MF_QB = 256 + 16;
 constexpr int MF_TERM_q = 144;
@@ -28,6 +30,10 @@
 }
 static_assert(mf_sym(11, 11) == MF_TRI - 1, "packed triangle size");
 static_assert(MF_COST % 8 == 0 && MF_OUT % 8 == 0, "records are whole 64-byte lines");
+static_assert(MF_CDIAG == 32 && MF_CDIAG_H == 0 && MF_CDIAG_QR == MF_N + MF_M && MF_CDIAG == MF_CDIAG_QR + MF_N + MF_M,
+              "diagonal cost record: diag(Q) 12 | diag(R) 4 | [q r] 16");
+static_assert((MF_CDIAG * 8) % 256 == 0 && (MF_CDIAG * 4) % 128 == 0, "diagonal cost records are whole 128-byte lines in fp64 and fp32 storage");
+static_assert(MF_DYN + MF_CDIAG == 236, "elements the backward sweep reads per knot point with a diagonal cost record (tools/membench.hip)");
 
 constexpr int MF_XCDS = 8;
 __host__ __device__ constexpr int mf_grid(int batch) { return MF_XCDS * ((batch + MF_XCDS - 1) / MF_XCDS); }
diff --git a/altro_amd/csrc/kernels/pack.hip b/altro_amd/csrc/kernels/pack.hip
--- a/altro_amd/csrc/kernels/pack.hip
+++ b/altro_amd/csrc/kernels/pack.hip
@@ -47,14 +47,14 @@
 
 template <typename S>
 __global__ void mfma16_pack_kernel(S* in, S* cin, S* term, Mfma16Strides st, int seg, SrcArr s0,
-                                   SrcArr s1, int is_diag, int N, int b0, int nb, int n, int m) {
+                                   SrcArr s1, int is_diag, int N, int b0, int nb, int n, int m, int cdiag = 0) {
   int len, base;
   switch (seg) {
     case MSEG_Z: len = 192; base = MF_OFF_Z; break;
     case MSEG_F: len = 12; base = MF_OFF_F; break;
-    case MSEG_Q: len = MF_TRI; base = MF_OFF_Q; break;
-    case MSEG_HR: len = 64; base = MF_OFF_HR; break;
-    case MSEG_QR: len = 16; base = MF_OFF_QR; break;
+    case MSEG_Q: len = cdiag ? MF_N : MF_TRI; base = cdiag ? MF_CDIAG_H : MF_OFF_Q; break;
+    case MSEG_HR: len = cdiag ? MF_M : 64; base = cdiag ? MF_CDIAG_H + MF_N : MF_OFF_HR; break;
+    case MSEG_QR: len = 16; base = cdiag ? MF_CDIAG_QR : MF_OFF_QR; break;
     case MSEG_TERM_Q: len = 144; base = 0; break;
     default: len = 12; base = 144; break;
   }
@@ -78,7 +78,7 @@
         }
       } break;
       case MSEG_F: v = (p0 && e < n) ? p0[e] : 0.0; break;
-      case MSEG_Q: {
+      case MSEG_Q: if (cdiag) { v = e < n ? p0[e] : 0.0; break; } {
         int row = 0, rem = e;
         while (rem >= 12 - row) { rem -= 12 - row; ++row; }
         const int jj = row + rem;
@@ -88,7 +88,7 @@
         const int row = e / 12, jj = e % 12;
         if (row < n && jj < n) v = is_diag ? (row == jj ? p0[row] : 0.0) : p0[row + n * jj];
       } break;
-      case MSEG_HR: {
+      case MSEG_HR: if (cdiag) { v = e < m ? p1[e] : 1.0; break; } {
         const int g = e / 16, jj = e % 16;
         if (g >= m) v = (jj == 12 + g) ? 1.0 : 0.0;
         else if (jj < 12) v = (is_diag || !p0 || jj >= n) ? 0.0 : p0[g + m * jj];
@@ -100,6 +100,36 @@
     if (terminal) term[(int64_t)(b0 + b) * MF_TERM + base + e] = (S)v;
     else if (seg == MSEG_Z || seg == MSEG_F) in[(int64_t)(b0 + b) * st.in_bs + (int64_t)k * st.in_ks + base + e] = (S)v;
     else cin[(int64_t)(b0 + b) * st.cin_bs + (int64_t)k * st.cin_ks + base + e] = (S)v;
+  }
+}
+
+template <typename S>
+__global__ void mfma16_cost_form_kernel(S* dense, int64_t dense_bs, int64_t dense_ks, S* diag, int64_t diag_bs, int64_t diag_ks,
+                                        int to_diag, int N, int batch) {
+  const int len = to_diag ? MF_CDIAG : MF_COST;
+  const int64_t total = (int64_t)batch * N * len;
+  for (int64_t t = blockIdx.x * (int64_t)blockDim.x + threadIdx.x; t < total; t += (int64_t)gridDim.x * blockDim.x) {
+    const int e = (int)(t % len);
+    const int b = (int)((t / len) % batch);
+    const int k = (int)(t / ((int64_t)len * batch));
+    S* dn = dense + (int64_t)b * dense_bs + (int64_t)k * dense_ks;
+    S* dg = diag + (int64_t)b * diag_bs + (int64_t)k * diag_ks;
+    if (to_diag) {
+      const int r = e - MF_CDIAG_H;
+      dg[e] = e >= MF_CDIAG_QR ? dn[MF_OFF_QR + (e - MF_CDIAG_QR)] : (r < MF_N ? dn[MF_OFF_Q + mf_sym(r, r)] : dn[MF_OFF_HR + (r - MF_N) * 16 + r]);
+    } else {
+      S v = S(0);
+      if (e >= MF_OFF_QR) v = dg[MF_CDIAG_QR + (e - MF_OFF_QR)];
+      else if (e >= MF_OFF_HR) {
+        const int g = (e - MF_OFF_HR) / 16, jj = (e - MF_OFF_HR) % 16;
+        if (jj == MF_N + g) v = dg[MF_CDIAG_H + MF_N + g];
+      } else if (e < MF_TRI) {
+        int row = 0, rem = e;
+        while (rem >= 12 - row) { rem -= 12 - row; ++row; }
+        if (rem == 0) v = dg[MF_CDIAG_H + row];
+      }
+      dn[e] = v;
+    }
   }
 }
 
diff --git a/altro_amd/csrc/kernels/tvlqr_mfma16.hip b/altro_amd/csrc/kernels/tvlqr_mfma16.hip
--- a/altro_amd/csrc/kernels/tvlqr_mfma16.hip
+++ b/altro_amd/csrc/kernels/tvlqr_mfma16.hip
@@ -45,6 +45,8 @@
   const S* in;
   int64_t in_bs, in_ks, out_bs, out_ks, xuy_bs, xuy_ks, cin_bs, cin_ks;
   const S* cin;
+  int cin_diag;
+  int cin_qr;
   const S* term;
   S* out;
   S* outn;
@@ -81,16 +83,23 @@
   return q;
 }
 
-template <bool HAS_F, typename S>
+template <bool HAS_F, typename S, bool CDIAG = false>
 __device__ __forceinline__ void mfma16_load_knot(Mfma16Knot& kn, const S* __restrict__ rec,
                                                  const S* __restrict__ crec, int lane, int j, int g,
                                                  const Mfma16QOff& qo) {
 #pragma unroll
   for (int c = 0; c < 3; ++c) kn.z[c] = ld_stream(&rec[MF_OFF_Z + c * 64 + lane]);
-#pragma unroll
-  for (int r = 0; r < 3; ++r) kn.q[r] = ld_stream(&crec[qo.o[r]]);
-  kn.hr = ld_stream(&crec[MF_OFF_HR + lane]);
-  kn.qr = ld_stream(&crec[MF_OFF_QR + j]);
+  if (CDIAG) {
+    kn.q[0] = ld_stream(&crec[MF_CDIAG_H + (j < 12 ? j : 11)]);
+    kn.q[1] = kn.q[2] = 0.0;
+    kn.hr = ld_stream(&crec[MF_CDIAG_H + 12 + g]);
+    kn.qr = ld_stream(&crec[MF_CDIAG_QR + j]);
+  } else {
+#pragma unroll
+    for (int r = 0; r < 3; ++r) kn.q[r] = ld_stream(&crec[qo.o[r]]);
+    kn.hr = ld_stream(&crec[MF_OFF_HR + lane]);
+    kn.qr = ld_stream(&crec[MF_OFF_QR + j]);
+  }
   if (HAS_F) {
 #pragma unroll
     for (int r = 0; r < 3; ++r) kn.f[r] = ld_stream(&rec[MF_OFF_F + g + 4 * r]);
@@ -106,7 +115,7 @@
   return __builtin_fma(y * e, t, y);
 }
 
-template <bool STORE_Q, bool HAS_F, typename S>
+template <bool STORE_Q, bool HAS_F, typename S, bool CDIAG = false>
 __global__ __launch_bounds__(64, 4) void mfma16_backward_kernel(Mfma16Args<S> a) {
   __shared__ __attribute__((aligned(16))) double lds[64 + 16 + 2];
   __shared__ double ptile[12 * MF_PT_LD];
@@ -131,6 +140,8 @@
   const int jc = col_ok ? j : 12;
   S* __restrict__ trash = a.trash + (size_t)b * MF_OUT;
   const Mfma16QOff qo = mfma16_q_offsets(j, g);
+  const int jq = (j < 12) ? j : 11;
+  const bool on_q0 = (g == jq), on_q1 = (g + 4 == jq), on_q2 = (g + 8 == jq), on_r = (j - 12 == g);
   int p_off[3];
 #pragma unroll
   for (int r = 0; r < 3; ++r) {
@@ -164,13 +175,13 @@
   const double reg = a.reg_pp ? a.reg_pp[b] : a.reg;
 
   Mfma16Knot cur, nxt;
-  mfma16_load_knot<HAS_F, S>(cur, in + (size_t)(N - 1) * a.in_ks, cin + (size_t)(N - 1) * a.cin_ks, lane, j, g, qo);
+  mfma16_load_knot<HAS_F, S, CDIAG>(cur, in + (size_t)(N - 1) * a.in_ks, cin + (size_t)(N - 1) * a.cin_ks, lane, j, g, qo);
   __builtin_amdgcn_s_waitcnt(0x0F70);
 
   for (int k = N - 1; k >= 0; --k) {
     {
       const size_t kp = (k > 0) ? k - 1 : 0;
-      mfma16_load_knot<HAS_F, S>(nxt, in + kp * a.in_ks, cin + kp * a.cin_ks, lane, j, g, qo);
+      mfma16_load_knot<HAS_F, S, CDIAG>(nxt, in + kp * a.in_ks, cin + kp * a.cin_ks, lane, j, g, qo);
     }
 
     f64x4 D1 = {0.0, 0.0, 0.0, 0.0};
@@ -178,6 +189,7 @@
     for (int c = 0; c < 3; ++c) D1 = mfma_f64_16x16x4(Pt[c], cur.z[c], D1);
 
     f64x4 G = {cur.q[0], cur.q[1], cur.q[2], cur.hr};
+    if (CDIAG) G = f64x4{on_q0 ? cur.q[0] : 0.0, on_q1 ? cur.q[0] : 0.0, on_q2 ? cur.q[0] : 0.0, on_r ? cur.hr : 0.0};
 #pragma unroll
     for (int c = 0; c < 3; ++c) G = mfma_f64_16x16x4(cur.z[c], D1[c], G);
 
diff --git a/include/altro_hip/altro_hip.h b/include/altro_hip/altro_hip.h
--- a/include/altro_hip/altro_hip.h
+++ b/include/altro_hip/altro_hip.h
@@ -160,8 +160,10 @@
 #define ALTRO_HIP_FORM_FUSED_CLOCK 0x4000u
 #define ALTRO_HIP_FORM_NO_COMPACTION 0x10000u
 #define ALTRO_HIP_FORM_GENERIC_MERIT_LDS 0x20000u
+#define ALTRO_HIP_FORM_COST_RECORD_DENSE 0x40000u
 int altro_hip_set_forms(altro_hip_batch* h, unsigned forms);
 unsigned altro_hip_get_forms(const altro_hip_batch* h);
+int altro_hip_cost_record_form(altro_hip_batch* h);
 typedef struct altro_hip_solve_result {
   int status;
   int iterations;
```

After: 2.696 million, median of 5. No clear change (+0.1%).
